# nh273/caro-ai

Measured on AMD Instinct MI355X. Metric: self-play MCTS node-expansions/sec/GPU (Connect4, 200 sims/move); 1->8 GPU scaling, higher is better.
Workload: dtype f32

## Files before the change

caro_ai_amd/_lib.py:

```python
import ctypes as C
import os

_HERE = os.path.dirname(os.path.abspath(__file__))
LIB_PATH = os.path.join(_HERE, "libcaro_hip.so")
if os.environ.get("CARO_HIP_LIB"):
    LIB_PATH = os.environ["CARO_HIP_LIB"]

GAME_CONNECT4, GAME_MNK, GAME_CARO = 0, 1, 2
RESIGNED = -2


class CaroError(RuntimeError):
    pass


class CaroConfig(C.Structure):
    _fields_ = [
        ("game_kind", C.c_int32), ("n", C.c_int32), ("k", C.c_int32), ("n_games", C.c_int32),
        ("n_stores", C.c_int32), ("n_nets", C.c_int32), ("max_batch", C.c_int32), ("node_cap", C.c_int32),
        ("steps_before_tau_0", C.c_int32), ("first_player_mode", C.c_int32),
        ("c_puct", C.c_float), ("alpha", C.c_double), ("explore", C.c_double),
        ("seed", C.c_uint64), ("uid_base", C.c_uint64), ("uid_stride", C.c_uint64),
        ("device_id", C.c_int32), ("evict", C.c_int32), ("stagger", C.c_int32), ("stagger_recycle", C.c_int32),
        ("games_limit", C.c_int64),
    ]


_P = C.c_void_p


class CaroDrainExtra(C.Structure):
    _fields_ = [("size", C.c_uint32), ("root_q_dev", _P), ("full_dev", _P), ("minibatches_dev", _P)]

    def __init__(self, root_q=None, full=None, minibatches=None):
        super().__init__(C.sizeof(CaroDrainExtra), root_q, full, minibatches)


class CaroDrainExtraOpen(CaroDrainExtra):
    _fields_ = [("open_dev", _P)]

    def __init__(self, root_q=None, full=None, minibatches=None, open=None):
        C.Structure.__init__(self, C.sizeof(CaroDrainExtraOpen), root_q, full, minibatches, open)


_SIGNATURES = {
    "caro_last_error": (C.c_char_p, []),
    "caro_version": (C.c_int, []),
    "caro_key_words": (C.c_int, [C.c_int, C.c_int]),
    "caro_action_space": (C.c_int, [C.c_int, C.c_int]),
    "caro_obs_cells": (C.c_int, [C.c_int, C.c_int]),
    "caro_host_initial": (C.c_int, [C.c_int, C.c_int, C.c_int, _P]),
    "caro_host_move": (C.c_int, [C.c_int, C.c_int, C.c_int, _P, C.c_int, C.c_int, _P]),
    "caro_host_legal": (C.c_int, [C.c_int, C.c_int, C.c_int, _P, _P]),
    "caro_host_encode": (C.c_int, [C.c_int, C.c_int, C.c_int, _P, C.c_int, _P]),
    "caro_host_noise_row": (C.c_int, [C.c_uint64, C.c_uint64, C.c_uint32, C.c_uint32, C.c_int, C.c_double, _P]),
    "caro_host_move_uniform": (C.c_double, [C.c_uint64, C.c_uint64, C.c_uint32]),
    "caro_host_resign_uniform": (C.c_double, [C.c_uint64, C.c_uint64]),
    "caro_host_cap_uniform": (C.c_double, [C.c_uint64, C.c_uint64, C.c_uint32]),
    "caro_host_open_uniform": (C.c_double, [C.c_uint64, C.c_uint64, C.c_uint32]),
    "caro_host_opening": (C.c_int, [C.c_int, C.c_int, C.c_int, C.c_uint64, C.c_uint64, C.c_int, C.c_int, _P, _P, _P]),
    "caro_openings_batch": (C.c_int, [C.c_int, C.c_int, C.c_int, C.c_uint64, C.c_int, C.c_int64] + [_P] * 6),
    "caro_rules_move_batch": (C.c_int, [C.c_int, C.c_int, C.c_int, C.c_int64, _P, _P, _P, _P, _P, _P]),
    "caro_rules_legal_batch": (C.c_int, [C.c_int, C.c_int, C.c_int, C.c_int64, _P, _P, _P]),
    "caro_rules_encode_batch": (C.c_int, [C.c_int, C.c_int, C.c_int, C.c_int64, _P, _P, _P, _P]),
    "caro_noise_batch": (C.c_int, [C.c_uint64, C.c_int64, C.c_int, C.c_double, _P, _P, _P, _P, _P]),
    "caro_engine_create": (C.c_int, [C.POINTER(CaroConfig), C.POINTER(_P)]),
    "caro_engine_destroy": (None, [_P]),
    "caro_engine_restart": (C.c_int, [_P, C.POINTER(CaroConfig), _P]),
    "caro_reset_games": (C.c_int, [_P, _P, _P]),
    "caro_set_roots": (C.c_int, [_P, _P, _P, _P]),
    "caro_select": (C.c_int, [_P, C.c_int, C.c_int, _P, _P, _P, _P]),
    "caro_leaf_counts": (C.c_int, [_P, _P, _P]),
    "caro_leaf_counts_dev": (C.c_int, [_P, _P]),
    "caro_net_packed_size": (C.c_int64, [C.c_int, C.c_int, C.c_int]),
    "caro_net_create": (C.c_int, [C.c_int, C.c_int, C.c_int, C.c_float, _P, C.c_int64, C.c_int, _P]),
    "caro_net_max_depth": (C.c_int, []),
    "caro_net_packed_size_depth": (C.c_int64, [C.c_int, C.c_int, C.c_int, C.c_int]),
    "caro_net_create_depth": (C.c_int, [C.c_int, C.c_int, C.c_int, C.c_int, C.c_float, _P, C.c_int64, C.c_int, _P]),
    "caro_net_depth": (C.c_int, [_P]),
    "caro_net_winograd_size_depth": (C.c_int64, [C.c_int]),
    "caro_net_winograd2d_size_depth": (C.c_int64, [C.c_int]),
    "caro_net_split_bf16_size_depth": (C.c_int64, [C.c_int]),
    "caro_net_destroy": (None, [_P]),
    "caro_net_enable_winograd": (C.c_int, [_P, _P, C.c_int64]),
    "caro_net_winograd2d_size": (C.c_int, []),
    "caro_net_winograd2d_supported": (C.c_int, [C.c_int, C.c_int]),
    "caro_net_enable_winograd2d": (C.c_int, [_P, _P, C.c_int64]),
    "caro_net_split_bf16_size": (C.c_int64, []),
    "caro_net_enable_split_bf16": (C.c_int, [_P, _P, C.c_int64]),
    "caro_net_boards_per_workgroup": (C.c_int, [_P]),
    "caro_net_uses_slot_list": (C.c_int, [_P]),
    "caro_net_stream_evictions": (C.c_int64, [_P]),
    "caro_net_forward": (C.c_int, [_P, _P, _P, C.c_int, C.c_int64, _P, _P, _P]),
    "caro_stream_create_partition": (C.c_int, [C.c_int, C.c_int, C.c_int, _P]),
    "caro_stream_destroy": (C.c_int, [_P]),
    "caro_search_batch": (C.c_int, [_P, _P, _P, C.c_int, C.c_int, _P, _P, _P, _P, _P, _P]),
    "caro_search_move": (C.c_int, [_P, _P, _P, C.c_int, C.c_int] + [_P] * 10),
    "caro_net_forward_pair": (C.c_int, [_P, _P, _P, _P, C.c_int64, _P, _P, _P]),
    "caro_net_forward_pair_at": (C.c_int, [_P, _P, _P, _P, C.c_int64, C.c_int64, _P, _P, _P]),
    "caro_net_forward_slots": (C.c_int, [_P, _P, _P, _P, _P, C.c_int, C.c_int, _P, _P, _P]),
    "caro_net_forward_slot_list": (C.c_int, [_P, _P, _P, _P, _P, _P, C.c_int, C.c_int, _P, _P, _P]),
    "caro_net_create_hash": (C.c_int, [C.c_int, C.c_int, C.c_int, C.c_uint64, C.c_int, _P]),
    "caro_net_forward_stamped": (C.c_int, [_P, _P, _P, C.c_int, C.c_int64, _P, _P, _P, _P]),
    "caro_net_debug_stamps": (C.c_int, [_P, _P]),
    "caro_get_descent": (C.c_int, [_P, C.c_int, C.c_int, _P, _P, _P, _P, _P, _P]),
    "caro_select_cancel": (C.c_int, [_P]),
    "caro_expand_backup": (C.c_int, [_P, _P, _P, _P]),
    "caro_policy": (C.c_int, [_P, _P, _P, _P]),
    "caro_step": (C.c_int, [_P, _P, _P, _P, _P, _P]),
    "caro_drain_tuples": (C.c_int, [_P, C.c_int64, _P, _P, _P, _P, _P, C.c_int, _P, _P, _P]),
    "caro_drain_tuples_begin": (C.c_int, [_P, C.c_int64, _P, _P, _P, _P, _P, C.c_int, _P]),
    "caro_drain_tuples_end": (C.c_int, [_P, _P, _P]),
    "caro_search_staggered": (C.c_int, [_P, _P, _P, C.c_int, C.c_int, _P, _P, _P, _P, _P]),
    "caro_drain_parked_begin": (C.c_int, [_P, C.c_int64, _P, _P, _P, _P, _P, _P]),
    "caro_engine_set_resign": (C.c_int, [_P, C.c_double, C.c_double]),
    "caro_drain_tuples_begin_q": (C.c_int, [_P, C.c_int64, _P, _P, _P, _P, _P, C.c_int, _P, _P]),
    "caro_drain_parked_begin_q": (C.c_int, [_P, C.c_int64, _P, _P, _P, _P, _P, _P, _P]),
    "caro_engine_set_playout_cap": (C.c_int, [_P, C.c_double, C.c_int]),
    "caro_drain_tuples_begin_x": (C.c_int, [_P, C.c_int64, _P, _P, _P, _P, _P, C.c_int, _P, _P, _P]),
    "caro_drain_parked_begin_x": (C.c_int, [_P, C.c_int64, _P, _P, _P, _P, _P, _P, _P, _P]),
    "caro_engine_set_early_stop": (C.c_int, [_P, C.c_int]),
    "caro_engine_set_openings": (C.c_int, [_P, C.c_int]),
    "caro_engine_set_forced_playouts": (C.c_int, [_P, C.c_double]),
    "caro_forced_stats": (C.c_int, [_P, _P, _P]),
    "caro_engine_set_kernel_form": (C.c_int, [_P, C.c_int]),
    "caro_engine_kernel_form": (C.c_int, [_P]),
    "caro_engine_set_fpu": (C.c_int, [_P, C.c_double, C.c_double]),
    "caro_host_fpu_level": (C.c_int, [C.c_int, C.c_int, _P, _P, _P, _P, _P, _P, _P, C.c_float, C.c_double, C.c_float,
                                      C.c_double, _P]),
    "caro_engine_set_virtual_loss": (C.c_int, [_P, C.c_int]),
    "caro_host_vl_level": (C.c_int, [C.c_int, C.c_int, _P, _P, _P, _P, _P, _P, _P, C.c_float, C.c_double, _P, C.c_int, _P]),
    "caro_engine_set_temperature": (C.c_int, [_P, C.c_double, C.c_double, C.c_int]),
    "caro_host_temperature": (C.c_int, [C.c_int, _P, C.c_double, _P]),
    "caro_host_forced_root": (C.c_int, [C.c_int, _P, _P, _P, _P, C.c_double, C.c_double, _P]),
    "caro_host_forced_prune": (C.c_int, [C.c_int, _P, _P, _P, C.c_float, C.c_double, _P]),
    "caro_drain_tuples_begin_ex": (C.c_int, [_P, C.c_int64, _P, _P, _P, _P, _P, C.c_int, C.POINTER(CaroDrainExtra), _P]),
    "caro_drain_parked_begin_ex": (C.c_int, [_P, C.c_int64, _P, _P, _P, _P, _P, C.POINTER(CaroDrainExtra), _P]),
    "caro_pool_open": (C.c_int, [_P, C.c_int64, _P, _P, _P, _P]),
    "caro_pool_set": (C.c_int, [_P, C.c_int64, _P, _P, _P, _P, _P]),
    "caro_pool_select": (C.c_int, [_P, C.c_int64, _P, _P]),
    "caro_pool_hold": (C.c_int, [_P, _P]),
    "caro_pool_level": (C.c_int, [_P, C.c_int64, _P, _P, _P, _P]),
    "caro_pool_select_budget": (C.c_int, [_P, C.c_int64, _P, _P, _P]),
    "caro_principal_lines": (C.c_int, [_P, C.c_int64, _P, C.c_int, C.c_int, C.c_int] + [_P] * 11),
    "caro_host_line_heads": (C.c_int, [C.c_int, _P, C.c_int, _P]),
    "caro_counters": (C.c_int, [_P, _P, _P]),
    "caro_live_games": (C.c_int, [_P, _P, _P]),
    "caro_pending_leaves": (C.c_int, [_P, _P, _P]),
    "caro_debug_stamps": (C.c_int, [_P, C.c_int]),
    "caro_debug_read": (C.c_int, [_P, _P, C.c_int64, _P]),
    "caro_debug_sqrt_check": (C.c_int, [C.c_uint32, _P]),
    "caro_profile_enable": (C.c_int, [_P, C.c_int]),
    "caro_profile_read": (C.c_int, [_P, _P, _P, C.c_int]),
    "caro_profile_begin": (C.c_int, [_P, C.c_int, _P]),
    "caro_profile_end": (None, [_P, C.c_int, _P]),
    "caro_tree_sizes": (C.c_int, [_P, _P, _P]),
    "caro_tree_live": (C.c_int, [_P, _P, _P]),
    "caro_lookup_nodes": (C.c_int, [_P, C.c_int64] + [_P] * 10),
    "caro_get_roots": (C.c_int, [_P] * 6),
    "caro_poke_nodes": (C.c_int, [_P, C.c_int64] + [_P] * 9),
    "caro_backup_path": (C.c_int, [_P, C.c_int, C.c_int, C.c_float, C.c_int, C.c_int, _P, _P, _P]),
    "caro_dump_tree": (C.c_int, [_P, C.c_int, C.c_int, C.c_int64] + [_P] * 8),
}
EXPORTS = sorted(_SIGNATURES)

_lib = None


def load():
    global _lib
    if _lib is not None:
        return _lib
    if not os.path.exists(LIB_PATH):
        raise CaroError("%s is missing: build it with `python -m caro_ai_amd.build` "
                        "(hipcc --offload-arch=gfx950); there is no CPU fallback" % LIB_PATH)
    try:
        lib = C.CDLL(LIB_PATH)
    except OSError as e:
        raise CaroError("cannot load %s: %s" % (LIB_PATH, e))
    for name, (res, args) in _SIGNATURES.items():
        fn = getattr(lib, name)
        fn.restype = res
        fn.argtypes = args
    _lib = lib
    return lib


def check(rc):
    if rc != 0:
        msg = load().caro_last_error()
        raise CaroError("libcaro_hip error %d: %s" % (rc, msg.decode() if msg else "?"))
```

caro_ai_amd/csrc/caro_net.hip:

```cpp
#include <hip/hip_runtime.h>

#include <algorithm>
#include <cstdlib>
#include <cstring>
#include <string>
#include <vector>

#include "../../include/caro_hip.h"
#include "../../include/caro_noise.h"

namespace cnet {

typedef float f32x16 __attribute__((ext_vector_type(16)));

constexpr int NF = 64;
constexpr int ZROW = 255;
constexpr int ACT = 256 * NF;
constexpr int WCHUNK = 64 * 64;
constexpr int NRES = 5;
constexpr int MAX_NRES = 40;
constexpr int TPC = 3;
constexpr int NTAPS = NRES * 9;
constexpr int LDS_FLOATS = ACT + 2 * TPC * WCHUNK;

struct NetParams {
  int H, W, HW, A, TB;
  float slope;
  const float* w_in;
  const float* b_in;
  const float* w_res;
  const float* b_res;
  const float* w_head;
  const float* b_head;
  const float* w_v1;
  const float* b_v1;
  const float* w_v2;
  const float* b_v2;
  const float* w_p;
  const float* b_p;
  const float* w_pT;
  const float* ww;
  const uint32_t* wtab;
  const float* ww2;
  const uint16_t* wx3;
  int ncu, TB2, TB4;
  int nres;
};

__device__ __forceinline__ int aoff(int row, int c) {
  return row * NF + ((((c >> 2) ^ (row & 15)) << 2) | (c & 3));
}
__device__ __forceinline__ float leaky(float x, float slope) { return x > 0.f ? x : x * slope; }

template <bool K2D>
__device__ __forceinline__ int akey(int r, int W) {
  if constexpr (!K2D) return r & 15;
  const int y = r / W, x = r - y * W;
  return (((x + 1) >> 1) & 7) | ((((y + 1) >> 1) & 1) << 3);
}

constexpr int NT = 512;

__device__ __forceinline__ void conv_in_f32(const NetParams& p, const float* __restrict__ planes, const int* smap,
                                            float* act, const float* win, int R, int tid) {
  const int HW = p.HW;
  const float slope = p.slope;
  const int r = tid & 255;
  const int chalf = tid >> 8;
  if (r < R) {
    const int bi = r / HW, cell = r - bi * HW;
    const int y = cell / p.W, x = cell - y * p.W;
    const float* pl = planes + (size_t)smap[bi] * 2 * HW;
    float in0[9], in1[9];
#pragma unroll
    for (int t = 0; t < 9; ++t) {
      const int ny = y + t / 3 - 1, nx = x + t % 3 - 1;
      const bool ok = ny >= 0 && ny < p.H && nx >= 0 && nx < p.W;
      in0[t] = ok ? pl[ny * p.W + nx] : 0.f;
      in1[t] = ok ? pl[HW + ny * p.W + nx] : 0.f;
    }
#pragma unroll
    for (int cc = 0; cc < 8; ++cc) {
      const int c4 = chalf * 8 + cc;
      float o[4];
#pragma unroll
      for (int u = 0; u < 4; ++u) o[u] = p.b_in[c4 * 4 + u];
#pragma unroll
      for (int t = 0; t < 9; ++t) {
        const float i0 = in0[t], i1 = in1[t];
        const float4 w0 = *reinterpret_cast<const float4*>(win + (2 * t) * NF + c4 * 4);
        const float4 w1 = *reinterpret_cast<const float4*>(win + (2 * t + 1) * NF + c4 * 4);
        o[0] = fmaf(i0, w0.x, o[0]); o[1] = fmaf(i0, w0.y, o[1]); o[2] = fmaf(i0, w0.z, o[2]); o[3] = fmaf(i0, w0.w, o[3]);
        o[0] = fmaf(i1, w1.x, o[0]); o[1] = fmaf(i1, w1.y, o[1]); o[2] = fmaf(i1, w1.z, o[2]); o[3] = fmaf(i1, w1.w, o[3]);
      }
      float4 out = make_float4(leaky(o[0], slope), leaky(o[1], slope), leaky(o[2], slope), leaky(o[3], slope));
      *reinterpret_cast<float4*>(act + r * NF + ((c4 ^ (r & 15)) << 2)) = out;
    }
  }
}

template <bool K2D = false, int NTH = NT>
__device__ __forceinline__ void conv_in_mfma(const NetParams& p, const float* __restrict__ planes, const int* smap,
                                             float* act, const float* win, int R, int tid) {
  const int HW = p.HW;
  const float slope = p.slope;
  const int wave = tid >> 6, lane = tid & 63;
  const int i = lane & 31, h = lane >> 5;
  const int ct = wave & 1;
  float wa[9];
#pragma unroll
  for (int t = 0; t < 9; ++t) wa[t] = win[(2 * t + h) * NF + ct * 32 + i];
  float4 bias[4];
#pragma unroll
  for (int q = 0; q < 4; ++q) bias[q] = *reinterpret_cast<const float4*>(p.b_in + ct * 32 + 8 * q + 4 * h);
  constexpr int RTS = NTH / 128;
#pragma unroll
  for (int half = 0; half < 8 / RTS; ++half) {
    const int rt = (wave >> 1) + RTS * half;
    if (rt * 32 >= R) continue;
    const int r = rt * 32 + i;
    const bool rv = r < R;
    const int bi = rv ? r / HW : 0, cell = rv ? r - bi * HW : 0;
    const int y = cell / p.W, x = cell - y * p.W;
    const float* pl = planes + (size_t)smap[bi] * 2 * HW + h * HW;
    float in[9];
#pragma unroll
    for (int t = 0; t < 9; ++t) {
      const int ny = y + t / 3 - 1, nx = x + t % 3 - 1;
      const bool ok = rv && ny >= 0 && ny < p.H && nx >= 0 && nx < p.W;
      in[t] = ok ? pl[ny * p.W + nx] : 0.f;
    }
    f32x16 acc;
#pragma unroll
    for (int q = 0; q < 4; ++q) {
      acc[4 * q] = bias[q].x; acc[4 * q + 1] = bias[q].y; acc[4 * q + 2] = bias[q].z; acc[4 * q + 3] = bias[q].w;
    }
#pragma unroll
    for (int t = 0; t < 9; ++t) acc = __builtin_amdgcn_mfma_f32_32x32x2f32(wa[t], in[t], acc, 0, 0, 0);
    if (rv) {
#pragma unroll
      for (int q = 0; q < 4; ++q) {
        const int c4 = ct * 8 + 2 * q + h;
        const float4 out = make_float4(leaky(acc[4 * q], slope), leaky(acc[4 * q + 1], slope),
                                       leaky(acc[4 * q + 2], slope), leaky(acc[4 * q + 3], slope));
        *reinterpret_cast<float4*>(act + r * NF + ((c4 ^ akey<K2D>(r, p.W)) << 2)) = out;
      }
    }
  }
}

constexpr int HEAD_STAGE_AT = 4096;
constexpr int HEAD_STAGE_MAX = 4096;
__device__ __forceinline__ int head_span(int HW, int A) { return 3 * NF + 3 + 20 * HW + 20 + 20 + 1 + A * 2 * HW + A; }
static inline int head_span_host(int HW, int A) { return 3 * NF + 3 + 20 * HW + 20 + 20 + 1 + A * 2 * HW + A; }

template <bool STAGED, bool K2D = false, int NTH = NT>
__device__ __forceinline__ void heads_f32(const NetParams& p, const float* act, float* scratch,
                                          float* __restrict__ probs, float* __restrict__ values, int slot_v, int nb,
                                          int R, int tid, float* __restrict__ featbuf = nullptr,
                                          int32_t* __restrict__ rowlist = nullptr, int dense0 = 0) {
  const int HW = p.HW, A = p.A;
  const float slope = p.slope;
  constexpr int NSM = (3 * NF + 3 + 20 * 225 + 20 + 20 + 1 + NTH - 1) / NTH;
  const int nsmall = 3 * NF + 3 + 20 * HW + 20 + 20 + 1;
  if (!STAGED && !featbuf) {
    float tmp[NSM];
#pragma unroll
    for (int u = 0; u < NSM; ++u) tmp[u] = tid + u * NTH < nsmall ? p.w_head[tid + u * NTH] : 0.f;
#pragma unroll
    for (int u = 0; u < NSM; ++u)
      if (tid + u * NTH < nsmall) scratch[HEAD_STAGE_AT + tid + u * NTH] = tmp[u];
    __syncthreads();
  }
  const float* hp = featbuf ? p.w_head : scratch + HEAD_STAGE_AT;
  const float* w_head = hp;
  const float* b_head = w_head + 3 * NF;
  const float* w_v1 = b_head + 3;
  const float* b_v1 = w_v1 + 20 * HW;
  const float* w_v2 = b_v1 + 20;
  const float* b_v2 = w_v2 + 20;
  const float* w_p = STAGED ? b_v2 + 1 : p.w_head + nsmall;
  const float* b_p = w_p + (size_t)A * 2 * HW;
  float* feat = scratch;
  float* hid = feat + 768;
  float* logit = feat + 768 + 20 * 32;
  float* stat = logit + 256 * 4;
  int* omap = reinterpret_cast<int*>(stat + 64);
  float* ebuf = stat + 128;
  if (tid < nb) omap[tid] = slot_v;
  for (int q = tid; q < 3 * R; q += NTH) {
    const int o = q / R, r = q - o * R;
    const float* wo = w_head + o * NF;
    float s0 = b_head[o];
    const int rkey = akey<K2D>(r, p.W);
#pragma unroll 8
    for (int g = 0; g < 16; ++g) {
      const float4 v = *reinterpret_cast<const float4*>(act + r * NF + ((g ^ rkey) << 2));
      const float4 w = *reinterpret_cast<const float4*>(wo + g * 4);
      s0 = fmaf(v.x, w.x, s0); s0 = fmaf(v.y, w.y, s0);
      s0 = fmaf(v.z, w.z, s0); s0 = fmaf(v.w, w.w, s0);
    }
    feat[o * 256 + r] = leaky(s0, slope);
  }
  __syncthreads();
  if (featbuf) {
    for (int q = tid; q < 3 * R; q += NTH) {
      const int o = q / R, r = q - o * R;
      const int bi = r / HW, c = r - bi * HW;
      featbuf[((size_t)(dense0 + bi) * 3 + o) * HW + c] = feat[o * 256 + r];
    }
    if (tid < nb) rowlist[dense0 + tid] = slot_v;
    return;
  }
  for (int k = tid; k < nb * 20; k += NTH) {
    const int bi = k / 20, u = k - bi * 20;
    float s = b_v1[u];
    const float* w = w_v1 + u * HW;
    const float* f = feat + bi * HW;
#pragma unroll 8
    for (int c = 0; c < HW; ++c) s = fmaf(f[c], w[c], s);
    hid[k] = leaky(s, slope);
  }
  for (int k = (tid + NTH / 2) % NTH; k < nb * A; k += NTH) {
    const int bi = k / A, a = k - bi * A;
    float s = b_p[a];
    const float* f0 = feat + 256 + bi * HW;
    const float* f1 = feat + 512 + bi * HW;
    if (STAGED || !p.w_pT) {
      const float* w = w_p + (size_t)a * 2 * HW;
#pragma unroll 8
      for (int c = 0; c < HW; ++c) s = fmaf(f0[c], w[c], s);
#pragma unroll 8
      for (int c = 0; c < HW; ++c) s = fmaf(f1[c], w[HW + c], s);
    } else {
      const int nq = HW >> 2, rem = HW & 3;
      const size_t half = ((size_t)HW * A + 3) & ~(size_t)3;
#pragma unroll
      for (int pl = 0; pl < 2; ++pl) {
        const float* f = pl ? f1 : f0;
        const float* wh = p.w_pT + pl * half;
        const float4* wq = reinterpret_cast<const float4*>(wh) + a;
#pragma unroll 8
        for (int q = 0; q < nq; ++q) {
          const float4 w = wq[(size_t)q * A];
          s = fmaf(f[4 * q], w.x, s); s = fmaf(f[4 * q + 1], w.y, s);
          s = fmaf(f[4 * q + 2], w.z, s); s = fmaf(f[4 * q + 3], w.w, s);
        }
        const float* wr = wh + (size_t)nq * A * 4 + a;
        for (int r = 0; r < rem; ++r) s = fmaf(f[4 * nq + r], wr[(size_t)r * A], s);
      }
    }
    logit[k] = s;
  }
  __syncthreads();
  {
    const int vt = tid - (NTH - 64);
    if (vt >= 0 && vt < nb) {
      float s = b_v2[0];
      for (int u = 0; u < 20; ++u) s = fmaf(hid[vt * 20 + u], w_v2[u], s);
      values[omap[vt]] = tanhf(s);
    }
  }
  float* pmax = ebuf + 1024;
  static_assert(768 + 20 * 32 + 256 * 4 + 128 + 1024 + 512 <= HEAD_STAGE_AT, "heads scratch layout");
  const bool wide = A > 32;
  if (wide) {
    for (int idx = tid; idx < nb * 16; idx += NTH) {
      const int bi = idx >> 4, j = idx & 15;
      const float* lg = logit + bi * A;
      float m = -3.4e38f;
      for (int a = j; a < A; a += 16) m = fmaxf(m, lg[a]);
      pmax[idx] = m;
    }
    __syncthreads();
  }
  for (int k = tid; k < nb * A; k += NTH) {
    const int bi = k / A;
    float mx = -3.4e38f;
    if (wide) {
      const float* pm = pmax + bi * 16;
#pragma unroll
      for (int j = 0; j < 16; ++j) mx = fmaxf(mx, pm[j]);
    } else {
      const float* lg = logit + bi * A;
      int a = 0;
      for (; a + 8 <= A; a += 8) {
        const float t0 = lg[a], t1 = lg[a + 1], t2 = lg[a + 2], t3 = lg[a + 3], t4 = lg[a + 4], t5 = lg[a + 5], t6 = lg[a + 6], t7 = lg[a + 7];
        mx = fmaxf(fmaxf(fmaxf(fmaxf(mx, t0), fmaxf(t1, t2)), fmaxf(fmaxf(t3, t4), fmaxf(t5, t6))), t7);
      }
      for (; a < A; ++a) mx = fmaxf(mx, lg[a]);
    }
    ebuf[k] = expf(logit[k] - mx);
  }
  __syncthreads();
  if (wide) {
    for (int idx = tid; idx < nb * 16; idx += NTH) {
      const int bi = idx >> 4, j = idx & 15;
      const float* eb = ebuf + bi * A;
      float part = 0.f;
      for (int a = j; a < A; a += 16) part += eb[a];
      pmax[idx] = part;
    }
    __syncthreads();
    if (tid < nb) {
      float sum = 0.f;
#pragma unroll
      for (int j = 0; j < 16; ++j) sum += pmax[tid * 16 + j];
      stat[2 * tid + 1] = sum;
    }
  } else if (tid < nb) {
    float sum = 0.f;
    const float* eb = ebuf + tid * A;
    int a = 0;
    for (; a + 8 <= A; a += 8) {
      const float t0 = eb[a], t1 = eb[a + 1], t2 = eb[a + 2], t3 = eb[a + 3], t4 = eb[a + 4], t5 = eb[a + 5], t6 = eb[a + 6], t7 = eb[a + 7];
      sum += t0; sum += t1; sum += t2; sum += t3; sum += t4; sum += t5; sum += t6; sum += t7;
    }
    for (; a < A; ++a) sum += eb[a];
    stat[2 * tid + 1] = sum;
  }
  __syncthreads();
  for (int k = tid; k < nb * A; k += NTH) {
    const int bi = k / A;
    probs[(size_t)omap[bi] * A + (k - bi * A)] = ebuf[k] / stat[2 * bi + 1];
  }
}

template <int NTH = NT>
__device__ __forceinline__ void tile_rows(const int32_t* __restrict__ gpack, int G, int B, int cls, int base,
                                          int board0, int nb, int* sc, int* smap, int tid) {
  if (!gpack) {
    if (tid < nb) smap[tid] = base + tid;
    __syncthreads();
    return;
  }
  const int lane = tid & 63, wave = tid >> 6;
  const int cpt = (G + NTH - 1) / NTH;
  const int g_lo = min(G, tid * cpt), g_hi = min(G, g_lo + cpt);
  int mine = 0;
  for (int g = g_lo; g < g_hi; ++g) {
    const int v = gpack[g];
    mine += (v >> 8) == cls ? (v & 0xFF) : 0;
  }
  int inc = mine;
#pragma unroll
  for (int d = 1; d < 64; d <<= 1) {
    const int t = __shfl_up(inc, d, 64);
    if (lane >= d) inc += t;
  }
  if (lane == 63) sc[wave] = inc;
  __syncthreads();
  int ex = inc - mine;
  for (int w = 0; w < wave; ++w) ex += sc[w];
  if (ex < board0 + nb && ex + mine > board0) {
    for (int g = g_lo; g < g_hi; ++g) {
      const int v = gpack[g];
      if ((v >> 8) != cls) continue;
      const int n = v & 0xFF;
      for (int j = 0; j < n; ++j) {
        const int r = ex + j - board0;
        if (r >= 0 && r < nb) smap[r] = g * B + j;
      }
      ex += n;
    }
  }
  __syncthreads();
}


constexpr int GP_PRE = 4;
__device__ __forceinline__ void tile_rows_pre(const int (&gv)[GP_PRE], int cpt, int mine, int B, int cls, int board0,
                                              int nb, int* sc, int* smap, int tid) {
  const int lane = tid & 63, wave = tid >> 6;
  int inc = mine;
#pragma unroll
  for (int d = 1; d < 64; d <<= 1) {
    const int t = __shfl_up(inc, d, 64);
    if (lane >= d) inc += t;
  }
  if (lane == 63) sc[wave] = inc;
  __syncthreads();
  int ex = inc - mine;
  for (int w = 0; w < wave; ++w) ex += sc[w];
  if (ex < board0 + nb && ex + mine > board0) {
#pragma unroll
    for (int u = 0; u < GP_PRE; ++u) {
      const int v = gv[u];
      if (u >= cpt || (v >> 8) != cls) continue;
      const int n = v & 0xFF, g = tid * cpt + u;
      for (int j = 0; j < n; ++j) {
        const int r = ex + j - board0;
        if (r >= 0 && r < nb) smap[r] = g * B + j;
      }
      ex += n;
    }
  }
  __syncthreads();
}

__device__ __forceinline__ unsigned lds_addr(const void* q) {
  return (unsigned)(size_t)(__attribute__((address_space(3))) const void*)q;
}
__device__ __forceinline__ void dma_b128(const void* gsrc, unsigned lds_wave_base) {
  asm volatile("s_mov_b32 m0, %0\n\ts_nop 0\n\tglobal_load_lds_dwordx4 %1, off" ::"s"(lds_wave_base), "v"(gsrc) : "memory");
}
__device__ __forceinline__ void dma_b128_s(const void* sbase, unsigned voff, unsigned lds_wave_base) {
  asm volatile("s_mov_b32 m0, %0\n\ts_nop 0\n\tglobal_load_lds_dwordx4 %1, %2" ::"s"(lds_wave_base), "v"(voff), "s"(sbase) : "memory");
}

#ifndef CARO_X3_TIMERS
#define CARO_X3_TIMERS 0
#endif
typedef __bf16 bf16x8 __attribute__((ext_vector_type(8)));
typedef __bf16 bf16x2 __attribute__((ext_vector_type(2)));
typedef float f32x2 __attribute__((ext_vector_type(2)));
typedef float f32x4v __attribute__((ext_vector_type(4)));
constexpr int X3_H = 3 * 4 * 64;
constexpr int X3_TAP_U4 = 2 * X3_H;
constexpr int X3_PAD_TAPS = 2;
constexpr int X3_RING_H1 = 3 * X3_H;

__device__ __forceinline__ uint32_t pk_bf16(f32x2 v) { return __builtin_bit_cast(uint32_t, __builtin_convertvector(v, bf16x2)); }
__device__ __forceinline__ f32x2 unpk_bf16(uint32_t w) {
  f32x2 r;
  r.x = __builtin_bit_cast(float, w << 16);
  r.y = __builtin_bit_cast(float, w & 0xFFFF0000u);
  return r;
}
__device__ __forceinline__ void split3(f32x2 v, uint32_t& hi, uint32_t& mid, uint32_t& lo) {
  hi = pk_bf16(v);
  const f32x2 r1 = v - unpk_bf16(hi);
  mid = pk_bf16(r1);
  const f32x2 r2 = r1 - unpk_bf16(mid);
  lo = pk_bf16(r2);
}
__device__ __forceinline__ f32x2 join3(uint32_t hi, uint32_t mid, uint32_t lo) {
  return (unpk_bf16(hi) + unpk_bf16(mid)) + unpk_bf16(lo);
}

__global__ __launch_bounds__(NT, 2) void k_net_forward_x3(NetParams p0, NetParams p1, const float* __restrict__ planes,
                                                            const int32_t* __restrict__ counts, int which, int row1,
                                                            float* __restrict__ probs, float* __restrict__ values,
                                                            unsigned long long* __restrict__ stamps,
                                                            const int32_t* __restrict__ gpack, int gG, int gB,
                                                            float* __restrict__ featbuf, int32_t* __restrict__ rowlist) {
  __shared__ __attribute__((aligned(16))) float lds[LDS_FLOATS];
  float* act = lds;
  float* wbuf = lds + ACT;

  int L, row0, board0;
  bool second = false;
  if (which < 2) {
    L = counts[which];
    row0 = which ? counts[0] : 0;
    board0 = blockIdx.x * p0.TB;
  } else {
    const int L0 = counts[0];
    const int t0 = (L0 + p0.TB - 1) / p0.TB;
    second = (int)blockIdx.x >= t0;
    L = second ? counts[1] : L0;
    row0 = second ? (row1 >= 0 ? row1 : L0) : 0;
    board0 = (second ? (int)blockIdx.x - t0 : (int)blockIdx.x) * p0.TB;
  }
  if (board0 >= L) return;
  const NetParams p = second ? p1 : p0;
  const float slope = p.slope;
  unsigned long long t_c0 = 0, t_r0 = 0, t_epi = 0;
  if (stamps) {
    t_c0 = __builtin_amdgcn_s_memtime();
    t_r0 = __builtin_amdgcn_s_memrealtime();
  }
  const int nb = min(p.TB, L - board0);
  const int HW = p.HW;
  const int R = nb * HW;
  const int tid = threadIdx.x;
  const int wave = tid >> 6, lane = tid & 63;

  for (int k = tid; k < ACT / 4; k += NT) reinterpret_cast<float4*>(lds)[k] = make_float4(0.f, 0.f, 0.f, 0.f);
  for (int k = tid; k < 9 * 2 * NF; k += NT) wbuf[k] = p.w_in[k];
  int* smap = reinterpret_cast<int*>(wbuf + 1536);
  tile_rows(gpack, gG, gB, second ? 1 : 0, row0 + board0, board0, nb, smap + 64, smap, tid);
  conv_in_mfma(p, planes, smap, act, wbuf, R, tid);
  const int slot_v0 = tid < nb ? smap[tid] : 0;
  __syncthreads();

  unsigned long long t_trunk0 = 0;
  if (stamps) t_trunk0 = __builtin_amdgcn_s_memtime();
  const int r16 = lane & 15, kg = lane >> 4;
  const int myrow0 = wave * 32 + r16, myrow1 = myrow0 + 16;
  const bool rvalid0 = myrow0 < R, rvalid1 = myrow1 < R;
  f32x2 res[2][4][2];
#pragma unroll
  for (int rb = 0; rb < 2; ++rb)
#pragma unroll
    for (int cb = 0; cb < 4; ++cb) {
      const int row = rb ? myrow1 : myrow0;
      const float4 v = *reinterpret_cast<const float4*>(act + row * NF + (((4 * cb + kg) ^ (row & 15)) << 2));
      res[rb][cb][0] = f32x2{v.x, v.y};
      res[rb][cb][1] = f32x2{v.z, v.w};
    }
  uint4* parts = reinterpret_cast<uint4*>(wbuf);
#pragma unroll
  for (int m = 0; m < 4; ++m) {
    const int k = tid + NT * m, row = k & 255, g = k >> 8;
    const float4 lo4 = *reinterpret_cast<const float4*>(act + row * NF + (((2 * g) ^ (row & 15)) << 2));
    const float4 hi4 = *reinterpret_cast<const float4*>(act + row * NF + (((2 * g + 1) ^ (row & 15)) << 2));
    const f32x2 v[4] = {{lo4.x, lo4.y}, {lo4.z, lo4.w}, {hi4.x, hi4.y}, {hi4.z, hi4.w}};
    uint32_t ph[4], pm[4], pl[4];
#pragma unroll
    for (int e = 0; e < 4; ++e) split3(v[e], ph[e], pm[e], pl[e]);
    parts[(0 * 8 + g) * 256 + row] = make_uint4(ph[0], ph[1], ph[2], ph[3]);
    parts[(1 * 8 + g) * 256 + row] = make_uint4(pm[0], pm[1], pm[2], pm[3]);
    parts[(2 * 8 + g) * 256 + row] = make_uint4(pl[0], pl[1], pl[2], pl[3]);
  }
  __syncthreads();
  uint4* ring = reinterpret_cast<uint4*>(act);
  const uint4* wsrc = reinterpret_cast<const uint4*>(p.wx3);
  const bool stage_h0 = tid >= 256;
  const unsigned ring_lds = lds_addr(ring);
  const unsigned v0off = (unsigned)tid * 16u;
  const unsigned v1off = (unsigned)(stage_h0 ? X3_TAP_U4 + (tid - 256) : X3_H + 512 + tid) * 16u;
  {
    ring[0 * X3_H + tid] = wsrc[tid];
    if (tid < 256) ring[0 * X3_H + 512 + tid] = wsrc[512 + tid];
    ring[1 * X3_H + tid] = wsrc[X3_TAP_U4 + tid];
    if (tid < 256) ring[1 * X3_H + 512 + tid] = wsrc[X3_TAP_U4 + 512 + tid];
    ring[X3_RING_H1 + tid] = wsrc[X3_H + tid];
    if (tid < 256) ring[X3_RING_H1 + 512 + tid] = wsrc[X3_H + 512 + tid];
  }
  static_assert((X3_RING_H1 + 2 * X3_H) * 16 + NRES * NF * 4 + NT * 4 <= ACT * 4, "ring + biases + output rows must fit the 64 KB of the float32 activations");
  float* bias_l = reinterpret_cast<float*>(ring + X3_RING_H1 + 2 * X3_H);
  int* slot_l = reinterpret_cast<int*>(bias_l + NRES * NF);
  if (tid < NRES * NF) bias_l[tid] = p.b_res[tid];
  slot_l[tid] = slot_v0;
  __syncthreads();

  int nrow9[9];
#pragma unroll
  for (int t = 0; t < 9; ++t) nrow9[t] = 0;
#pragma unroll
  for (int rb = 0; rb < 2; ++rb) {
    const int row = rb ? myrow1 : myrow0;
    const bool rv = rb ? rvalid1 : rvalid0;
    const int rbi = row / HW;
    const int rcell = row - rbi * HW;
    const int ry = rcell / p.W, rx = rcell - ry * p.W;
#pragma unroll
    for (int t = 0; t < 9; ++t) {
      const int ny = ry + t / 3 - 1, nx = rx + t % 3 - 1;
      const bool ok = rv && ny >= 0 && ny < p.H && nx >= 0 && nx < p.W;
      nrow9[t] |= (ok ? rbi * HW + ny * p.W + nx : (int)ZROW) << (16 * rb);
    }
  }

  f32x4v acc[2][4];
#pragma unroll
  for (int rb = 0; rb < 2; ++rb)
#pragma unroll
    for (int cb = 0; cb < 4; ++cb) acc[rb][cb] = f32x4v{0.f, 0.f, 0.f, 0.f};
  const uint4* arow = parts + kg * 256;
#define CARO_X3_LOAD_ACT(S_, C_, N0_, N1_)                                  \
  _Pragma("unroll") for (int pt_ = 0; pt_ < 3; ++pt_) {                     \
    S_[pt_ * 2] = arow[(pt_ * 8 + 4 * (C_)) * 256 + (N0_)];                 \
    S_[pt_ * 2 + 1] = arow[(pt_ * 8 + 4 * (C_)) * 256 + (N1_)];             \
  }
#define CARO_X3_LOAD_W(S_, HB_, CP_)                                        \
  _Pragma("unroll") for (int pt_ = 0; pt_ < 3; ++pt_) {                     \
    S_[pt_ * 2] = (HB_)[pt_ * 256 + (CP_) * 32];                            \
    S_[pt_ * 2 + 1] = (HB_)[pt_ * 256 + (CP_) * 32 + 16];                   \
  }
#define CARO_X3_PROD(W_, A_, CP_, WP_, AP_)                                                                     \
  _Pragma("unroll") for (int cbi_ = 0; cbi_ < 2; ++cbi_) _Pragma("unroll") for (int rb_ = 0; rb_ < 2; ++rb_)   \
    acc[rb_][2 * (CP_) + cbi_] = __builtin_amdgcn_mfma_f32_16x16x32_bf16(                                       \
        __builtin_bit_cast(bf16x8, W_[(WP_) * 2 + cbi_]), __builtin_bit_cast(bf16x8, A_[(AP_) * 2 + rb_]),      \
        acc[rb_][2 * (CP_) + cbi_], 0, 0, 0);
#define CARO_X3_SEG(W_, A_, CP_)  \
  CARO_X3_PROD(W_, A_, CP_, 1, 1) \
  CARO_X3_PROD(W_, A_, CP_, 2, 0) \
  CARO_X3_PROD(W_, A_, CP_, 0, 2) \
  CARO_X3_PROD(W_, A_, CP_, 1, 0) \
  CARO_X3_PROD(W_, A_, CP_, 0, 1) \
  CARO_X3_PROD(W_, A_, CP_, 0, 0)
#define CARO_X3_WEAVE(NR_)                                  \
  _Pragma("unroll") for (int q_ = 0; q_ < (NR_); ++q_) {    \
    __builtin_amdgcn_sched_group_barrier(0x008, 2, 0);      \
    __builtin_amdgcn_sched_group_barrier(0x100, 1, 0);      \
  }                                                         \
  __builtin_amdgcn_sched_group_barrier(0x008, 24 - 2 * (NR_), 0);
#if CARO_X3_TIMERS
  unsigned long long tq[8] = {0, 0, 0, 0, 0, 0, 0, 0}, tl = 0;
#define CARO_T0 tl = __builtin_amdgcn_s_memtime();
#define CARO_T(K_) { const unsigned long long t_ = __builtin_amdgcn_s_memtime(); tq[K_] += t_ - tl; tl = t_; }
#else
#define CARO_T0
#define CARO_T(K_)
#endif
  uint4 X[6], Y[6], P[6], Q[6];
  const uint4* wcol = ring + kg * 64 + r16;
  CARO_X3_LOAD_ACT(X, 0, nrow9[0] & 0xFFFF, nrow9[0] >> 16)
  CARO_X3_LOAD_W(P, wcol, 0)
  const char* wnext = reinterpret_cast<const char*>(wsrc + X3_TAP_U4);
  for (int layer = 0; layer < NRES; ++layer) {
#pragma unroll
    for (int tap = 0; tap < 9; ++tap) {
      const int cur = (layer + tap) & 1;
      const int slot0 = tap % 3, slot1 = (tap + 1) % 3, slot2 = (tap + 2) % 3;
      CARO_T0
      {
        const unsigned d1 = ring_lds + (unsigned)(X3_RING_H1 + (cur ^ 1) * X3_H) * 16u;
        const unsigned d0 = ring_lds + (unsigned)(slot2 * X3_H) * 16u;
        const unsigned w1k = (unsigned)wave * 1024u;
        dma_b128_s(wnext + X3_H * 16, v0off, __builtin_amdgcn_readfirstlane(d1 + w1k));
        dma_b128_s(wnext, v1off, __builtin_amdgcn_readfirstlane(stage_h0 ? d0 + w1k - 4096u : d1 + 8192u + w1k));
        dma_b128_s(wnext + (X3_TAP_U4 + 256) * 16, v0off, __builtin_amdgcn_readfirstlane(d0 + 4096u + w1k));
        wnext += X3_TAP_U4 * 16;
      }
      const uint4* hb0 = wcol + slot0 * X3_H;
      const uint4* hb1 = wcol + X3_RING_H1 + cur * X3_H;
      const int n0 = nrow9[tap] & 0xFFFF, n1 = nrow9[tap] >> 16;
      __builtin_amdgcn_sched_barrier(0);
      CARO_T(0)
      CARO_X3_LOAD_W(Q, hb0, 1)
      CARO_X3_SEG(P, X, 0)
      CARO_X3_WEAVE(6)
      __builtin_amdgcn_sched_barrier(0);
      CARO_T(1)
      CARO_X3_LOAD_ACT(Y, 1, n0, n1)
      CARO_X3_LOAD_W(P, hb1, 0)
      CARO_X3_SEG(Q, X, 1)
      CARO_X3_WEAVE(12)
      __builtin_amdgcn_sched_barrier(0);
      CARO_T(2)
      CARO_X3_LOAD_W(Q, hb1, 1)
      CARO_X3_SEG(P, Y, 0)
      CARO_X3_WEAVE(6)
      __builtin_amdgcn_sched_barrier(0);
      CARO_T(3)
      CARO_X3_LOAD_ACT(X, 0, nrow9[tap == 8 ? 0 : tap + 1] & 0xFFFF, nrow9[tap == 8 ? 0 : tap + 1] >> 16)
      CARO_X3_LOAD_W(P, wcol + slot1 * X3_H, 0)
      CARO_X3_SEG(Q, Y, 1)
      CARO_X3_WEAVE(12)
      __builtin_amdgcn_sched_barrier(0);
      CARO_T(4)
      if (tap == 8) {
        unsigned long long t_e0 = 0;
        if (stamps) t_e0 = __builtin_amdgcn_s_memtime();
        __syncthreads();
        const f32x2 slope2 = {slope, slope};
        float4 bq[4];
#pragma unroll
        for (int cb = 0; cb < 4; ++cb) bq[cb] = *reinterpret_cast<const float4*>(bias_l + layer * NF + 16 * cb + 4 * kg);
#pragma unroll
        for (int rb = 0; rb < 2; ++rb) {
          const int row = rb ? myrow1 : myrow0;
          const bool rv = rb ? rvalid1 : rvalid0;
          const f32x2 keep = rv ? f32x2{1.f, 1.f} : f32x2{0.f, 0.f};
          uint2* mine = reinterpret_cast<uint2*>(parts + (kg >> 1) * 256 + row) + (kg & 1);
#pragma unroll
          for (int cb = 0; cb < 4; ++cb) {
            const f32x4v a = acc[rb][cb];
            const f32x2 t01 = f32x2{a[0], a[1]} + f32x2{bq[cb].x, bq[cb].y}, t23 = f32x2{a[2], a[3]} + f32x2{bq[cb].z, bq[cb].w};
            const f32x2 s01 = t01 * slope2, s23 = t23 * slope2;
            const f32x2 l01 = {t01.x > 0.f ? t01.x : s01.x, t01.y > 0.f ? t01.y : s01.y};
            const f32x2 l23 = {t23.x > 0.f ? t23.x : s23.x, t23.y > 0.f ? t23.y : s23.y};
            res[rb][cb][0] = (res[rb][cb][0] + l01) * keep;
            res[rb][cb][1] = (res[rb][cb][1] + l23) * keep;
            uint2 wh, wm, wl;
            split3(res[rb][cb][0], wh.x, wm.x, wl.x);
            split3(res[rb][cb][1], wh.y, wm.y, wl.y);
            mine[(0 * 8 + 2 * cb) * 512] = wh;
            mine[(1 * 8 + 2 * cb) * 512] = wm;
            mine[(2 * 8 + 2 * cb) * 512] = wl;
            acc[rb][cb] = f32x4v{0.f, 0.f, 0.f, 0.f};
          }
        }
        if (stamps) t_epi += __builtin_amdgcn_s_memtime() - t_e0;
      }
      CARO_T0
      asm volatile("s_waitcnt vmcnt(0)" ::: "memory");
      __syncthreads();
      CARO_T(5)
      if (tap == 8 && layer + 1 < NRES) {
        CARO_X3_LOAD_ACT(X, 0, nrow9[0] & 0xFFFF, nrow9[0] >> 16)
      }
    }
  }
#undef CARO_X3_WEAVE
#undef CARO_X3_LOAD_ACT
#undef CARO_X3_LOAD_W
#undef CARO_X3_PROD
#undef CARO_X3_SEG
  const int slot_v = slot_l[tid];
  __syncthreads();
#pragma unroll
  for (int rb = 0; rb < 2; ++rb)
#pragma unroll
    for (int cb = 0; cb < 4; ++cb) {
      const int row = rb ? myrow1 : myrow0;
      *reinterpret_cast<float4*>(act + row * NF + (((4 * cb + kg) ^ (row & 15)) << 2)) =
          make_float4(res[rb][cb][0].x, res[rb][cb][0].y, res[rb][cb][1].x, res[rb][cb][1].y);
    }
  __syncthreads();
  unsigned long long t_trunk1 = 0;
  if (stamps) t_trunk1 = __builtin_amdgcn_s_memtime();
  heads_f32<false>(p, act, wbuf, probs, values, slot_v, nb, R, tid, featbuf, rowlist, row0 + board0);
  if (stamps && tid == 0) {
    stamps[4 * blockIdx.x] = __builtin_amdgcn_s_memtime() - t_c0;
    stamps[4 * blockIdx.x + 1] = ((__builtin_amdgcn_s_memrealtime() - t_r0) & 0xFFFFFull) | (t_epi << 20);
    stamps[4 * blockIdx.x + 2] = t_trunk0 - t_c0;
    stamps[4 * blockIdx.x + 3] = t_trunk1 - t_c0;
#if CARO_X3_TIMERS
    for (int q = 0; q < 8; ++q) stamps[4 * 512 + 8 * blockIdx.x + q] = tq[q];
#endif
  }
}

constexpr int WCH = 4 * 2 * 64 * 16;
constexpr int WNBUF = 3;
constexpr int XROW4 = 63;
constexpr int XROW2 = 127;
static_assert(WNBUF * WCH == 2 * TPC * WCHUNK, "the ring takes the place of the two three-tap buffers");

typedef float f4v __attribute__((ext_vector_type(4)));

__device__ __forceinline__ void fetch_chunk(const float* ww, int c, unsigned wring, int tid) {
  const float4* src = reinterpret_cast<const float4*>(ww + (size_t)c * WCH) + tid;
  const unsigned dst = __builtin_amdgcn_readfirstlane(wring + (unsigned)(c % WNBUF) * (WCH * 4) + (unsigned)(tid >> 6) * 1024u);
#pragma unroll
  for (int m = 0; m < WCH / 4 / NT; ++m) dma_b128(src + m * NT, dst + m * NT * 16);
}

__device__ __forceinline__ void fetch_chunk_s(const float* ww, int c, unsigned wring, int tid) {
  const char* base = reinterpret_cast<const char*>(ww) + (size_t)c * (WCH * 4);
  const unsigned voff = (unsigned)tid * 16u;
  const unsigned dst = __builtin_amdgcn_readfirstlane(wring + (unsigned)(c % WNBUF) * (WCH * 4) + (unsigned)(tid >> 6) * 1024u);
#pragma unroll
  for (int m = 0; m < WCH / 4 / NT; ++m) dma_b128_s(base + m * NT * 16, voff, dst + m * NT * 16);
}

__device__ __forceinline__ void fetch_heads(const float* hp, int hspan, unsigned wring, int tid) {
  const float4* src = reinterpret_cast<const float4*>(hp) + tid;
  const unsigned dst = __builtin_amdgcn_readfirstlane(wring + HEAD_STAGE_AT * 4u + (unsigned)(tid >> 6) * 1024u);
  dma_b128(src, dst);
  if (hspan > NT * 4) dma_b128(src + NT, dst + NT * 16);
}

template <int KS, int NR>
__device__ __forceinline__ void trunk_w(const NetParams& p, float* act, float* wbuf, int nb, int tid, int hspan) {
  const int nres = NR ? NR : p.nres;
  const int wnchunk = nres * 6;
  const float slope = p.slope;
  const int HW = p.HW;
  const int wave = tid >> 6, lane = tid & 63;
  const int i = lane & 31, h = lane >> 5;
  constexpr int NRT = 4 / KS;
  constexpr int NQ = 4 / KS;
  constexpr int NSET = 6 * NQ;
  const int ct = wave & 1, rt = (wave >> 1) % NRT, kq = (wave >> 1) / NRT;
  int tbi, tty, tx;
  bool tvalid;
  if (KS == 1) {
    const uint32_t tent = p.wtab[rt * 32 + i];
    tbi = tent & 0xFF; tty = (tent >> 8) & 0xFF; tx = (tent >> 16) & 0xFF;
    tvalid = (tent >> 24) != 0 && tbi < nb;
  } else {
    const int tpb = ((p.H + 1) >> 1) * p.W;
    const int mt = rt * 32 + i;
    tbi = mt / tpb;
    const int rem = mt - tbi * tpb;
    tty = rem / p.W; tx = rem - tty * p.W;
    tvalid = mt < nb * tpb;
  }
  const int orow0 = tbi * HW + 2 * tty * p.W + tx;
  const bool ovalid0 = tvalid, ovalid1 = tvalid && 2 * tty + 1 < p.H;
  const unsigned abase = lds_addr(act);
  unsigned ra[4][3];
#pragma unroll
  for (int r = 0; r < 4; ++r) {
    const int y = 2 * tty - 1 + r;
    const bool oky = tvalid && y >= 0 && y < p.H;
#pragma unroll
    for (int d = 0; d < 3; ++d) {
      const int nx = tx + d - 1;
      const int v = tbi * HW + y * p.W + nx;
      const int row = oky && nx >= 0 && nx < p.W ? v : ZROW;
      ra[r][d] = abase + (unsigned)(row * NF + (((h * 8 + kq) ^ (v & 15)) << 2)) * 4u;
    }
  }
  const unsigned wlane = lds_addr(wbuf) + (unsigned)((h * 64 + ct * 32 + i) * 16 + ((kq ^ ((i >> 2) & 3)) << 2)) * 4u;
  const unsigned wring = lds_addr(wbuf);

  f4v D0, D1, D2, D3;
  f4v W0, W1, W2, W3, X0, X1, X2, X3;
#define CARO_ALOAD(B0, B1, B2, B3, T)                                                                        \
  {                                                                                                          \
    constexpr int cc_ = (T) / NQ, dx_ = cc_ >> 1, g8_ = (cc_ & 1) * 4 + ((T) % NQ) * KS;                     \
    const unsigned wa_ = (wlane + (unsigned)(cc_ % WNBUF) * (WCH * 4)) ^ ((unsigned)(((T) % NQ) * KS) << 4); \
    asm volatile("ds_read_b128 %0, %1" : "=v"(D0) : "v"(ra[0][dx_] ^ (g8_ << 4)));                           \
    asm volatile("ds_read_b128 %0, %1" : "=v"(D1) : "v"(ra[1][dx_] ^ (g8_ << 4)));                           \
    asm volatile("ds_read_b128 %0, %1" : "=v"(D2) : "v"(ra[2][dx_] ^ (g8_ << 4)));                           \
    asm volatile("ds_read_b128 %0, %1" : "=v"(D3) : "v"(ra[3][dx_] ^ (g8_ << 4)));                           \
    asm volatile("ds_read_b128 %0, %1" : "=v"(B0) : "v"(wa_));                                               \
    asm volatile("ds_read_b128 %0, %1 offset:8192" : "=v"(B1) : "v"(wa_));                                   \
    asm volatile("ds_read_b128 %0, %1 offset:16384" : "=v"(B2) : "v"(wa_));                                  \
    asm volatile("ds_read_b128 %0, %1 offset:24576" : "=v"(B3) : "v"(wa_));                                  \
  }
#define CARO_AWAIT(B0, B1, B2, B3)                                                                           \
  asm volatile("s_waitcnt lgkmcnt(0)" : "+v"(D0), "+v"(D1), "+v"(D2), "+v"(D3), "+v"(B0), "+v"(B1), "+v"(B2), "+v"(B3));
#define CARO_STEP(T, B0, B1, B2, B3, NB0, NB1, NB2, NB3)                                                     \
  CARO_AWAIT(B0, B1, B2, B3)                                                                                 \
  if ((T) % NQ == 0) {                                                                                       \
    if ((T) != 0) {                                                                                          \
      asm volatile("s_waitcnt vmcnt(0)" ::: "memory");                                                       \
       __syncthreads();                                                                    \
    }                                                                                                        \
    if ( c0 + (T) / NQ + 2 < wnchunk) fetch_chunk(p.ww, c0 + (T) / NQ + 2, wring, tid);         \
    else if (c0 + (T) / NQ + 2 == wnchunk && hspan) fetch_heads(p.w_head, hspan, wring, tid);                \
  }                                                                                                          \
  {                                                                                                          \
        \
    const f4v v0 = D0 - D2;                                                                                  \
    __builtin_amdgcn_sched_barrier(0);                                                                       \
    accM0 = __builtin_amdgcn_mfma_f32_32x32x2f32(B0.x, v0.x, accM0, 0, 0, 0);                                \
    const f4v v1 = D1 + D2;                                                                                  \
    __builtin_amdgcn_sched_barrier(0);                                                                       \
    accM1 = __builtin_amdgcn_mfma_f32_32x32x2f32(B1.x, v1.x, accM1, 0, 0, 0);                                \
    const f4v v2 = D2 - D1;                                                                                  \
    __builtin_amdgcn_sched_barrier(0);                                                                       \
    accM2 = __builtin_amdgcn_mfma_f32_32x32x2f32(B2.x, v2.x, accM2, 0, 0, 0);                                \
    const f4v v3 = D1 - D3;                                                                                  \
    __builtin_amdgcn_sched_barrier(0);                                                                       \
    accM3 = __builtin_amdgcn_mfma_f32_32x32x2f32(B3.x, v3.x, accM3, 0, 0, 0);                                \
    __builtin_amdgcn_sched_barrier(0);                                                                       \
    if ((T) + 1 < NSET) CARO_ALOAD(NB0, NB1, NB2, NB3, ((T) + 1) % NSET)                                     \
    __builtin_amdgcn_sched_barrier(0);                                                                       \
    accM0 = __builtin_amdgcn_mfma_f32_32x32x2f32(B0.y, v0.y, accM0, 0, 0, 0);                                \
    accM1 = __builtin_amdgcn_mfma_f32_32x32x2f32(B1.y, v1.y, accM1, 0, 0, 0);                                \
    accM2 = __builtin_amdgcn_mfma_f32_32x32x2f32(B2.y, v2.y, accM2, 0, 0, 0);                                \
    accM3 = __builtin_amdgcn_mfma_f32_32x32x2f32(B3.y, v3.y, accM3, 0, 0, 0);                                \
    accM0 = __builtin_amdgcn_mfma_f32_32x32x2f32(B0.z, v0.z, accM0, 0, 0, 0);                                \
    accM1 = __builtin_amdgcn_mfma_f32_32x32x2f32(B1.z, v1.z, accM1, 0, 0, 0);                                \
    accM2 = __builtin_amdgcn_mfma_f32_32x32x2f32(B2.z, v2.z, accM2, 0, 0, 0);                                \
    accM3 = __builtin_amdgcn_mfma_f32_32x32x2f32(B3.z, v3.z, accM3, 0, 0, 0);                                \
    accM0 = __builtin_amdgcn_mfma_f32_32x32x2f32(B0.w, v0.w, accM0, 0, 0, 0);                                \
    accM1 = __builtin_amdgcn_mfma_f32_32x32x2f32(B1.w, v1.w, accM1, 0, 0, 0);                                \
    accM2 = __builtin_amdgcn_mfma_f32_32x32x2f32(B2.w, v2.w, accM2, 0, 0, 0);                                \
    accM3 = __builtin_amdgcn_mfma_f32_32x32x2f32(B3.w, v3.w, accM3, 0, 0, 0);                                \
    __builtin_amdgcn_sched_barrier(0);                                                                       \
  }

  float4 res0[4], res1[4];
#pragma unroll
  for (int q = 0; q < 4; ++q) res0[q] = res1[q] = make_float4(0.f, 0.f, 0.f, 0.f);
  for (int layer = 0; layer < nres; ++layer) {
    const int c0 = layer * 6;
    f32x16 accM0, accM1, accM2, accM3;
#pragma unroll
    for (int e = 0; e < 16; ++e) {
      accM0[e] = 0.f;
      accM1[e] = 0.f;
      accM2[e] = 0.f;
      accM3[e] = 0.f;
    }
#pragma unroll
    for (int r = 0; r < 4; ++r)
#pragma unroll
      for (int d = 0; d < 3; ++d) asm volatile("" : "+v"(ra[r][d]));
    CARO_ALOAD(W0, W1, W2, W3, 0)
#define CARO_PAIR(T)                                                                                         \
  CARO_STEP(T, W0, W1, W2, W3, X0, X1, X2, X3)                                                               \
  CARO_STEP((T) + 1, X0, X1, X2, X3, W0, W1, W2, W3)
    CARO_PAIR(0) CARO_PAIR(2) CARO_PAIR(4)
    if constexpr (NSET > 6) { CARO_PAIR(6) CARO_PAIR(8) CARO_PAIR(10) }
    if constexpr (NSET > 12) { CARO_PAIR(12) CARO_PAIR(14) CARO_PAIR(16) CARO_PAIR(18) CARO_PAIR(20) CARO_PAIR(22) }
#undef CARO_PAIR
    if constexpr (KS == 2) {
      const bool up = kq != 0;
      const float m0 = up ? 0.f : 1.f, m2 = up ? -1.f : 1.f, m3 = up ? -1.f : 0.f;
      const float s0 = up ? 1.f : 0.f, s2 = up ? 1.f : -1.f, s3 = up ? 0.f : -1.f;
      const float* bias = p.b_res + layer * NF + ct * 32 + 4 * h;
      const int g0 = ct * 8 + h;
      float* rowp = act + (orow0 + (up ? p.W : 0)) * NF;
      const int kk = (orow0 + (up ? p.W : 0)) & 15;
      const bool ov = up ? ovalid1 : ovalid0;
      float4 bq[4], old[4];
#pragma unroll
      for (int q = 0; q < 4; ++q) bq[q] = *reinterpret_cast<const float4*>(bias + 8 * q);
      if (layer == 0) {
#pragma unroll
        for (int q = 0; q < 4; ++q)
          old[q] = ov ? *reinterpret_cast<const float4*>(rowp + (((g0 + 2 * q) ^ kk) << 2)) : make_float4(0.f, 0.f, 0.f, 0.f);
      } else {
#pragma unroll
        for (int q = 0; q < 4; ++q) old[q] = res0[q];
      }
      f32x16 mine, send;
#pragma unroll
      for (int e = 0; e < 16; ++e) {
        float a = fmaf(m0, accM0[e], 0.f), b = fmaf(s0, accM0[e], 0.f);
        a = fmaf(1.f, accM1[e], a); b = fmaf(1.f, accM1[e], b);
        a = fmaf(m2, accM2[e], a); b = fmaf(s2, accM2[e], b);
        a = fmaf(m3, accM3[e], a); b = fmaf(s3, accM3[e], b);
        mine[e] = a;
        send[e] = b;
      }
      float* xw = act + XROW2 * NF + ((rt * 2 + ct) * 2 + kq) * 1024 + lane * 4;
      const float* xr = act + XROW2 * NF + ((rt * 2 + ct) * 2 + (kq ^ 1)) * 1024 + lane * 4;
#pragma unroll
      for (int q = 0; q < 4; ++q)
        *reinterpret_cast<float4*>(xw + q * 256) = make_float4(send[4 * q], send[4 * q + 1], send[4 * q + 2], send[4 * q + 3]);
      asm volatile("s_waitcnt lgkmcnt(0)" ::: "memory");
      __builtin_amdgcn_s_barrier();
      asm volatile("" ::: "memory");
      float4 part[4];
#pragma unroll
      for (int q = 0; q < 4; ++q) part[q] = *reinterpret_cast<const float4*>(xr + q * 256);
#pragma unroll
      for (int q = 0; q < 4; ++q) {
        float4 n;
        n.x = old[q].x + leaky((mine[4 * q] + part[q].x) + bq[q].x, slope);
        n.y = old[q].y + leaky((mine[4 * q + 1] + part[q].y) + bq[q].y, slope);
        n.z = old[q].z + leaky((mine[4 * q + 2] + part[q].z) + bq[q].z, slope);
        n.w = old[q].w + leaky((mine[4 * q + 3] + part[q].w) + bq[q].w, slope);
        if (ov) *reinterpret_cast<float4*>(rowp + (((g0 + 2 * q) ^ kk) << 2)) = n;
        res0[q] = ov ? n : make_float4(0.f, 0.f, 0.f, 0.f);
      }
    } else if constexpr (KS == 4) {
      f32x16 accY0, accY1;
#pragma unroll
      for (int e = 0; e < 16; ++e) {
        float y0 = fmaf(1.f, accM0[e], 0.f), y1 = fmaf(0.f, accM0[e], 0.f);
        y0 = fmaf(1.f, accM1[e], y0); y1 = fmaf(1.f, accM1[e], y1);
        y0 = fmaf(1.f, accM2[e], y0); y1 = fmaf(-1.f, accM2[e], y1);
        y0 = fmaf(0.f, accM3[e], y0); y1 = fmaf(-1.f, accM3[e], y1);
        accY0[e] = y0;
        accY1[e] = y1;
      }
      const int myrow = kq >> 1, qb = (kq & 1) * 2;
      const float* bias = p.b_res + layer * NF + ct * 32 + 4 * h;
      const int g0 = ct * 8 + h;
      float* rowp = act + (orow0 + (myrow ? p.W : 0)) * NF;
      const int kk = (orow0 + (myrow ? p.W : 0)) & 15;
      const bool ov = myrow ? ovalid1 : ovalid0;
      float4 bq[2], old[2];
#pragma unroll
      for (int j = 0; j < 2; ++j) bq[j] = *reinterpret_cast<const float4*>(bias + 8 * (qb + j));
      if (layer == 0) {
#pragma unroll
        for (int j = 0; j < 2; ++j)
          old[j] = ov ? *reinterpret_cast<const float4*>(rowp + (((g0 + 2 * (qb + j)) ^ kk) << 2)) : make_float4(0.f, 0.f, 0.f, 0.f);
      } else {
#pragma unroll
        for (int j = 0; j < 2; ++j) old[j] = res0[j];
      }
#define CARO_QUARTER(D, J)                                                                                              \
  (((D) >> 1) ? make_float4(accY1[4 * (2 * ((D) & 1) + (J))], accY1[4 * (2 * ((D) & 1) + (J)) + 1],                      \
                            accY1[4 * (2 * ((D) & 1) + (J)) + 2], accY1[4 * (2 * ((D) & 1) + (J)) + 3])                  \
              : make_float4(accY0[4 * (2 * ((D) & 1) + (J))], accY0[4 * (2 * ((D) & 1) + (J)) + 1],                      \
                            accY0[4 * (2 * ((D) & 1) + (J)) + 2], accY0[4 * (2 * ((D) & 1) + (J)) + 3]))
      float* xa = act + XROW4 * NF + lane * 4;
      float4 mine[2] = {make_float4(0.f, 0.f, 0.f, 0.f), make_float4(0.f, 0.f, 0.f, 0.f)};
#pragma unroll
      for (int d = 0; d < 4; ++d) {
        if (d == kq) {
          mine[0] = CARO_QUARTER(d, 0);
          mine[1] = CARO_QUARTER(d, 1);
        } else {
          const int sp = kq < d ? kq : kq - 1;
          float* dst = xa + (((ct * 4 + d) * 3 + sp) * 2) * 256;
          *reinterpret_cast<float4*>(dst) = CARO_QUARTER(d, 0);
          *reinterpret_cast<float4*>(dst + 256) = CARO_QUARTER(d, 1);
        }
      }
#undef CARO_QUARTER
      asm volatile("s_waitcnt lgkmcnt(0)" ::: "memory");
      __builtin_amdgcn_s_barrier();
      asm volatile("" ::: "memory");
      float4 part[4][2];
#pragma unroll
      for (int k = 0; k < 4; ++k) {
        part[k][0] = part[k][1] = make_float4(0.f, 0.f, 0.f, 0.f);
        if (k != kq) {
          const int sp = k < kq ? k : k - 1;
          const float* src = xa + (((ct * 4 + kq) * 3 + sp) * 2) * 256;
          part[k][0] = *reinterpret_cast<const float4*>(src);
          part[k][1] = *reinterpret_cast<const float4*>(src + 256);
        }
      }
#pragma unroll
      for (int j = 0; j < 2; ++j) {
        float4 v = kq == 0 ? mine[j] : part[0][j];
#pragma unroll
        for (int k = 1; k < 4; ++k) {
          const float4 t = k == kq ? mine[j] : part[k][j];
          v.x += t.x; v.y += t.y; v.z += t.z; v.w += t.w;
        }
        float4 n;
        n.x = old[j].x + leaky(v.x + bq[j].x, slope);
        n.y = old[j].y + leaky(v.y + bq[j].y, slope);
        n.z = old[j].z + leaky(v.z + bq[j].z, slope);
        n.w = old[j].w + leaky(v.w + bq[j].w, slope);
        if (ov) *reinterpret_cast<float4*>(rowp + (((g0 + 2 * (qb + j)) ^ kk) << 2)) = n;
        res0[j] = ov ? n : make_float4(0.f, 0.f, 0.f, 0.f);
      }
    } else {
    f32x16 accY0, accY1;
#pragma unroll
    for (int e = 0; e < 16; ++e) {
      float y0 = fmaf(1.f, accM0[e], 0.f), y1 = fmaf(0.f, accM0[e], 0.f);
      y0 = fmaf(1.f, accM1[e], y0); y1 = fmaf(1.f, accM1[e], y1);
      y0 = fmaf(1.f, accM2[e], y0); y1 = fmaf(-1.f, accM2[e], y1);
      y0 = fmaf(0.f, accM3[e], y0); y1 = fmaf(-1.f, accM3[e], y1);
      accY0[e] = y0;
      accY1[e] = y1;
    }
    const float* bias = p.b_res + layer * NF + ct * 32 + 4 * h;
    const int g0 = ct * 8 + h;
    float* row0p = act + orow0 * NF;
    float* row1p = row0p + p.W * NF;
    const int k0 = orow0 & 15, k1 = (orow0 + p.W) & 15;
    float4 bq[4], old0[4], old1[4];
#pragma unroll
    for (int q = 0; q < 4; ++q) bq[q] = *reinterpret_cast<const float4*>(bias + 8 * q);
    if (layer == 0) {
#pragma unroll
      for (int q = 0; q < 4; ++q) {
        old0[q] = ovalid0 ? *reinterpret_cast<const float4*>(row0p + (((g0 + 2 * q) ^ k0) << 2)) : make_float4(0.f, 0.f, 0.f, 0.f);
        old1[q] = ovalid1 ? *reinterpret_cast<const float4*>(row1p + (((g0 + 2 * q) ^ k1) << 2)) : make_float4(0.f, 0.f, 0.f, 0.f);
      }
    } else {
#pragma unroll
      for (int q = 0; q < 4; ++q) {
        old0[q] = res0[q];
        old1[q] = res1[q];
      }
    }
    asm volatile("" ::: "memory");
    __builtin_amdgcn_s_barrier();
    asm volatile("" ::: "memory");
    const bool writer = true;
#pragma unroll
    for (int q = 0; q < 4; ++q) {
      float4 n0, n1;
      n0.x = old0[q].x + leaky(accY0[4 * q] + bq[q].x, slope);
      n0.y = old0[q].y + leaky(accY0[4 * q + 1] + bq[q].y, slope);
      n0.z = old0[q].z + leaky(accY0[4 * q + 2] + bq[q].z, slope);
      n0.w = old0[q].w + leaky(accY0[4 * q + 3] + bq[q].w, slope);
      n1.x = old1[q].x + leaky(accY1[4 * q] + bq[q].x, slope);
      n1.y = old1[q].y + leaky(accY1[4 * q + 1] + bq[q].y, slope);
      n1.z = old1[q].z + leaky(accY1[4 * q + 2] + bq[q].z, slope);
      n1.w = old1[q].w + leaky(accY1[4 * q + 3] + bq[q].w, slope);
      if (ovalid0 && writer) *reinterpret_cast<float4*>(row0p + (((g0 + 2 * q) ^ k0) << 2)) = n0;
      if (ovalid1 && writer) *reinterpret_cast<float4*>(row1p + (((g0 + 2 * q) ^ k1) << 2)) = n1;
      res0[q] = ovalid0 ? n0 : make_float4(0.f, 0.f, 0.f, 0.f);
      res1[q] = ovalid1 ? n1 : make_float4(0.f, 0.f, 0.f, 0.f);
    }
    }
    asm volatile("s_waitcnt vmcnt(0)" ::: "memory");
    __syncthreads();
  }
#undef CARO_STEP
#undef CARO_AWAIT
#undef CARO_ALOAD
}


constexpr int W2NCHUNK = NRES * 8;
constexpr int W2SETS = 16;

template <int NR>
__device__ __forceinline__ void trunk_w2d(const NetParams& p, float* act, float* wbuf, int tid) {
  const int nres = NR ? NR : p.nres;
  const int w2nchunk = nres * 8;
  const float slope = p.slope;
  const int H = p.H, W = p.W;
  const int wave = tid >> 6, lane = tid & 63;
  const int i = lane & 31, h = lane >> 5;
  const int ct = wave & 1, rt = (wave >> 1) & 1, bh = wave >> 2;
  const int quad = i >> 2, grp = (0x96 >> quad) & 1, qq = ((quad >> 1) << 2) | (i & 3);
  const int tx = qq & 7, ty = rt * 4 + grp * 2 + (qq >> 3);
  const bool tvalid = ty < ((H + 1) >> 1) && tx < ((W + 1) >> 1);
  const unsigned abase = lds_addr(act);
  const unsigned wring = lds_addr(wbuf);
  auto caddr = [&](int r, int j) -> unsigned {
    const int y = 2 * ty - 1 + r, x = 2 * tx - 1 + j;
    const bool ok = tvalid && y >= 0 && y < H && x >= 0 && x < W;
    const int row = ok ? y * W + x : ZROW;
    const int key = ((tx + (j >> 1)) & 7) | (((ty + (r >> 1)) & 1) << 3);
    return abase + (unsigned)(row * NF + (((h * 8) ^ key) << 2)) * 4u;
  };
  const int jA0 = bh ? 2 : 1, jB0 = bh ? 1 : 2, jA1 = bh ? 1 : 0, jB1 = bh ? 3 : 2;
  const float sg0 = bh ? -1.f : 1.f, sg1 = -1.f;
  unsigned ra[2][4], rb[2][4];
#pragma unroll
  for (int r = 0; r < 4; ++r) {
    ra[0][r] = caddr(r, jA0); rb[0][r] = caddr(r, jB0);
    ra[1][r] = caddr(r, jA1); rb[1][r] = caddr(r, jB1);
  }
  const unsigned wlane = wring + (unsigned)(bh * 16384 + (h * 64 + ct * 32 + i) * 32 + (((i >> 3) & 1) << 4));
  const int xo = 2 * tx + bh, xp = 2 * tx + 1 - bh;
  const int g0 = ct * 8 + h;
  int oidx[2], pidx[2];
  bool ovalid[2], pvalid[2];
#pragma unroll
  for (int u = 0; u < 2; ++u) {
    const int y = 2 * ty + u;
    ovalid[u] = tvalid && y < H && xo < W;
    pvalid[u] = tvalid && y < H && xp < W;
    const int okey = (((xo + 1) >> 1) & 7) | ((((y + 1) >> 1) & 1) << 3);
    const int pkey = (((xp + 1) >> 1) & 7) | ((((y + 1) >> 1) & 1) << 3);
    oidx[u] = (y * W + xo) * NF + ((g0 ^ okey) << 2);
    pidx[u] = (y * W + xp) * NF + ((g0 ^ pkey) << 2);
  }

  f4v CA0, CA1, CA2, CA3, CB0, CB1, CB2, CB3;
  f4v W0, W1, W2, W3, X0, X1, X2, X3;
#define W2_ALOAD(B0, B1, B2, B3, T)                                                                          \
  {                                                                                                          \
    constexpr int ph_ = (T) >> 3, G_ = (T) & 7, cq_ = (T) >> 1;                                              \
    const unsigned wa_ = (wlane + rbuf[cq_ % WNBUF]) ^ ((unsigned)(G_ & 1) << 4);                            \
    asm volatile("ds_read_b128 %0, %1" : "=v"(CA0) : "v"(ra[ph_][0] ^ (G_ << 4)));                           \
    asm volatile("ds_read_b128 %0, %1" : "=v"(CB0) : "v"(rb[ph_][0] ^ (G_ << 4)));                           \
    asm volatile("ds_read_b128 %0, %1" : "=v"(CA1) : "v"(ra[ph_][1] ^ (G_ << 4)));                           \
    asm volatile("ds_read_b128 %0, %1" : "=v"(CB1) : "v"(rb[ph_][1] ^ (G_ << 4)));                           \
    asm volatile("ds_read_b128 %0, %1" : "=v"(CA2) : "v"(ra[ph_][2] ^ (G_ << 4)));                           \
    asm volatile("ds_read_b128 %0, %1" : "=v"(CB2) : "v"(rb[ph_][2] ^ (G_ << 4)));                           \
    asm volatile("ds_read_b128 %0, %1" : "=v"(CA3) : "v"(ra[ph_][3] ^ (G_ << 4)));                           \
    asm volatile("ds_read_b128 %0, %1" : "=v"(CB3) : "v"(rb[ph_][3] ^ (G_ << 4)));                           \
    asm volatile("ds_read_b128 %0, %1" : "=v"(B0) : "v"(wa_));                                               \
    asm volatile("ds_read_b128 %0, %1 offset:4096" : "=v"(B1) : "v"(wa_));                                   \
    asm volatile("ds_read_b128 %0, %1 offset:8192" : "=v"(B2) : "v"(wa_));                                   \
    asm volatile("ds_read_b128 %0, %1 offset:12288" : "=v"(B3) : "v"(wa_));                                  \
  }
#define W2_AWAIT(B0, B1, B2, B3)                                                                             \
  asm volatile("s_waitcnt lgkmcnt(0)"                                                                        \
               : "+v"(CA0), "+v"(CA1), "+v"(CA2), "+v"(CA3), "+v"(CB0), "+v"(CB1), "+v"(CB2), "+v"(CB3),     \
                 "+v"(B0), "+v"(B1), "+v"(B2), "+v"(B3));
#define W2_STEP(T, B0, B1, B2, B3, NB0, NB1, NB2, NB3)                                                       \
  W2_AWAIT(B0, B1, B2, B3)                                                                                   \
  if ((T) % 2 == 0) {                                                                                        \
    if ((T) != 0) {                                                                                          \
      asm volatile("s_waitcnt vmcnt(0)" ::: "memory");                                                       \
       __syncthreads();                                                                    \
    }                                                                                                        \
    if ( c0 + (T) / 2 + 2 < w2nchunk) fetch_chunk_s(p.ww2, c0 + (T) / 2 + 2, wring, tid);       \
  }                                                                                                          \
  {                                                                                                          \
    const float sg_ = ((T) >> 3) ? sg1 : sg0;                                                                \
    const f4v c0_ = CA0 + sg_ * CB0, c1_ = CA1 + sg_ * CB1, c2_ = CA2 + sg_ * CB2, c3_ = CA3 + sg_ * CB3;    \
    const f4v v0 = c0_ - c2_;                                                                                \
    __builtin_amdgcn_sched_barrier(0);                                                                       \
                        \
    accM0 = __builtin_amdgcn_mfma_f32_32x32x2f32(B0.x, v0.x, (T) % 8 == 0 ? zero16 : accM0, 0, 0, 0);        \
    const f4v v1 = c1_ + c2_;                                                                                \
    __builtin_amdgcn_sched_barrier(0);                                                                       \
    accM1 = __builtin_amdgcn_mfma_f32_32x32x2f32(B1.x, v1.x, (T) % 8 == 0 ? zero16 : accM1, 0, 0, 0);        \
    const f4v v2 = c2_ - c1_;                                                                                \
    __builtin_amdgcn_sched_barrier(0);                                                                       \
    accM2 = __builtin_amdgcn_mfma_f32_32x32x2f32(B2.x, v2.x, (T) % 8 == 0 ? zero16 : accM2, 0, 0, 0);        \
    const f4v v3 = c1_ - c3_;                                                                                \
    __builtin_amdgcn_sched_barrier(0);                                                                       \
    accM3 = __builtin_amdgcn_mfma_f32_32x32x2f32(B3.x, v3.x, (T) % 8 == 0 ? zero16 : accM3, 0, 0, 0);        \
    __builtin_amdgcn_sched_barrier(0);                                                                       \
    if ((T) + 1 < W2SETS) W2_ALOAD(NB0, NB1, NB2, NB3, ((T) + 1) % W2SETS)                                   \
    __builtin_amdgcn_sched_barrier(0);                                                                       \
    accM0 = __builtin_amdgcn_mfma_f32_32x32x2f32(B0.y, v0.y, accM0, 0, 0, 0);                                \
    accM1 = __builtin_amdgcn_mfma_f32_32x32x2f32(B1.y, v1.y, accM1, 0, 0, 0);                                \
    accM2 = __builtin_amdgcn_mfma_f32_32x32x2f32(B2.y, v2.y, accM2, 0, 0, 0);                                \
    accM3 = __builtin_amdgcn_mfma_f32_32x32x2f32(B3.y, v3.y, accM3, 0, 0, 0);                                \
    accM0 = __builtin_amdgcn_mfma_f32_32x32x2f32(B0.z, v0.z, accM0, 0, 0, 0);                                \
    accM1 = __builtin_amdgcn_mfma_f32_32x32x2f32(B1.z, v1.z, accM1, 0, 0, 0);                                \
    accM2 = __builtin_amdgcn_mfma_f32_32x32x2f32(B2.z, v2.z, accM2, 0, 0, 0);                                \
    accM3 = __builtin_amdgcn_mfma_f32_32x32x2f32(B3.z, v3.z, accM3, 0, 0, 0);                                \
    accM0 = __builtin_amdgcn_mfma_f32_32x32x2f32(B0.w, v0.w, accM0, 0, 0, 0);                                \
    accM1 = __builtin_amdgcn_mfma_f32_32x32x2f32(B1.w, v1.w, accM1, 0, 0, 0);                                \
    accM2 = __builtin_amdgcn_mfma_f32_32x32x2f32(B2.w, v2.w, accM2, 0, 0, 0);                                \
    accM3 = __builtin_amdgcn_mfma_f32_32x32x2f32(B3.w, v3.w, accM3, 0, 0, 0);                                \
    __builtin_amdgcn_sched_barrier(0);                                                                       \
  }
#define W2_PAIR(T)                                                                                           \
  W2_STEP(T, W0, W1, W2, W3, X0, X1, X2, X3)                                                                 \
  W2_STEP((T) + 1, X0, X1, X2, X3, W0, W1, W2, W3)
#define W2_FOLD(Z0_, Z1_)                                                                                    \
  _Pragma("unroll") for (int e = 0; e < 16; ++e) {                                                           \
    Z0_[e] = (accM0[e] + accM1[e]) + accM2[e];                                                               \
    Z1_[e] = (accM1[e] - accM2[e]) - accM3[e];                                                               \
  }

  for (int layer = 0; layer < nres; ++layer) {
    const int c0 = layer * 8;
    unsigned rbuf[WNBUF];
#pragma unroll
    for (int k = 0; k < WNBUF; ++k) rbuf[k] = (unsigned)((c0 + k) % WNBUF) * (WCH * 4);
    const f32x16 zero16 = {};
    f32x16 accM0, accM1, accM2, accM3, Zs0, Zs1, Zt0, Zt1;
#pragma unroll
    for (int r = 0; r < 4; ++r) asm volatile("" : "+v"(ra[0][r]), "+v"(rb[0][r]), "+v"(ra[1][r]), "+v"(rb[1][r]));
    W2_ALOAD(W0, W1, W2, W3, 0)
    W2_PAIR(0) W2_PAIR(2) W2_PAIR(4)
    const float* bias = p.b_res + layer * NF + ct * 32 + 4 * h;
    float4 bq[4];
#pragma unroll
    for (int q = 0; q < 4; ++q) bq[q] = *reinterpret_cast<const float4*>(bias + 8 * q);
    W2_PAIR(6)
    W2_FOLD(Zs0, Zs1)
    if (bh == 0) {
#pragma unroll
      for (int q = 0; q < 4; ++q) {
        Zs0[4 * q] += bq[q].x; Zs0[4 * q + 1] += bq[q].y; Zs0[4 * q + 2] += bq[q].z; Zs0[4 * q + 3] += bq[q].w;
        Zs1[4 * q] += bq[q].x; Zs1[4 * q + 1] += bq[q].y; Zs1[4 * q + 2] += bq[q].z; Zs1[4 * q + 3] += bq[q].w;
      }
    }
    W2_PAIR(8) W2_PAIR(10) W2_PAIR(12) W2_PAIR(14)
    W2_FOLD(Zt0, Zt1)
    float4 old0[4], old1[4];
    asm volatile("" : "+v"(oidx[0]), "+v"(oidx[1]), "+v"(pidx[0]), "+v"(pidx[1]));
#pragma unroll
    for (int q = 0; q < 4; ++q) {
      old0[q] = ovalid[0] ? *reinterpret_cast<const float4*>(act + (oidx[0] ^ (8 * q))) : make_float4(0.f, 0.f, 0.f, 0.f);
      old1[q] = ovalid[1] ? *reinterpret_cast<const float4*>(act + (oidx[1] ^ (8 * q))) : make_float4(0.f, 0.f, 0.f, 0.f);
    }
    f32x16 S0, S1;
#pragma unroll
    for (int e = 0; e < 16; ++e) {
      S0[e] = Zt0[e] + Zs0[e];
      S1[e] = Zt1[e] + Zs1[e];
    }
    asm volatile("s_waitcnt lgkmcnt(0)" ::: "memory");
    __builtin_amdgcn_s_barrier();
    asm volatile("" ::: "memory");
    {
#pragma unroll
      for (int q = 0; q < 4; ++q) {
        if (pvalid[0])
          *reinterpret_cast<float4*>(act + (pidx[0] ^ (8 * q))) = make_float4(Zs0[4 * q], Zs0[4 * q + 1], Zs0[4 * q + 2], Zs0[4 * q + 3]);
        if (pvalid[1])
          *reinterpret_cast<float4*>(act + (pidx[1] ^ (8 * q))) = make_float4(Zs1[4 * q], Zs1[4 * q + 1], Zs1[4 * q + 2], Zs1[4 * q + 3]);
      }
    }
    asm volatile("s_waitcnt lgkmcnt(0)" ::: "memory");
    __builtin_amdgcn_s_barrier();
    asm volatile("" ::: "memory");
    const float sgn = bh ? -1.f : 1.f;
#pragma unroll
    for (int q = 0; q < 4; ++q) {
      const float4 r0 = ovalid[0] ? *reinterpret_cast<const float4*>(act + (oidx[0] ^ (8 * q))) : make_float4(0.f, 0.f, 0.f, 0.f);
      const float4 r1 = ovalid[1] ? *reinterpret_cast<const float4*>(act + (oidx[1] ^ (8 * q))) : make_float4(0.f, 0.f, 0.f, 0.f);
      float4 n0, n1;
      n0.x = old0[q].x + leaky(fmaf(sgn, S0[4 * q], r0.x), slope);
      n0.y = old0[q].y + leaky(fmaf(sgn, S0[4 * q + 1], r0.y), slope);
      n0.z = old0[q].z + leaky(fmaf(sgn, S0[4 * q + 2], r0.z), slope);
      n0.w = old0[q].w + leaky(fmaf(sgn, S0[4 * q + 3], r0.w), slope);
      n1.x = old1[q].x + leaky(fmaf(sgn, S1[4 * q], r1.x), slope);
      n1.y = old1[q].y + leaky(fmaf(sgn, S1[4 * q + 1], r1.y), slope);
      n1.z = old1[q].z + leaky(fmaf(sgn, S1[4 * q + 2], r1.z), slope);
      n1.w = old1[q].w + leaky(fmaf(sgn, S1[4 * q + 3], r1.w), slope);
      if (ovalid[0]) *reinterpret_cast<float4*>(act + (oidx[0] ^ (8 * q))) = n0;
      if (ovalid[1]) *reinterpret_cast<float4*>(act + (oidx[1] ^ (8 * q))) = n1;
    }
    asm volatile("s_waitcnt vmcnt(0)" ::: "memory");
    __syncthreads();
  }
#undef W2_FOLD
#undef W2_PAIR
#undef W2_STEP
#undef W2_AWAIT
#undef W2_ALOAD
}

#define CARO_NR NRES
#define CARO_KN(name) name
#include "caro_net_kernels.inc"
#undef CARO_NR
#undef CARO_KN
#define CARO_NR 0
#define CARO_KN(name) name##_any
#include "caro_net_kernels.inc"
#undef CARO_NR
#undef CARO_KN

constexpr int HB = 32;
constexpr int HEADS_MAX_CELLS = 225;
constexpr int HPL = 228;
static_assert(HPL >= HEADS_MAX_CELLS && HPL % 4 == 0, "a staged feature plane holds every cell of the largest board");
constexpr int HFS = 3 * HPL + 8;
constexpr int HLG = 256;
__global__ __launch_bounds__(NT, 1) void k_net_heads(NetParams p0, NetParams p1, const int32_t* __restrict__ counts,
                                                       int which, int row1, const float* __restrict__ featbuf,
                                                       const int32_t* __restrict__ rowlist, float* __restrict__ probs,
                                                       float* __restrict__ values) {
  __shared__ __attribute__((aligned(16))) float F[HB * HFS];
  __shared__ __attribute__((aligned(16))) float logit[HB * HLG];
  __shared__ float wv1[20 * HEADS_MAX_CELLS];
  __shared__ float hid[HB * 20];
  __shared__ float part[HB * 16];
  __shared__ float rsum[HB];
  __shared__ int orow[HB];
  int L, base, blk;
  bool second = false;
  if (which < 2) {
    L = counts[which];
    base = which ? counts[0] : 0;
    blk = blockIdx.x;
  } else {
    const int L0 = counts[0], nb0 = (L0 + HB - 1) / HB;
    second = (int)blockIdx.x >= nb0;
    L = second ? counts[1] : L0;
    base = second ? (row1 >= 0 ? row1 : L0) : 0;
    blk = second ? (int)blockIdx.x - nb0 : (int)blockIdx.x;
  }
  const int i0 = blk * HB;
  if (i0 >= L) return;
  const int nbrd = L - i0 < HB ? L - i0 : HB;
  const NetParams p = second ? p1 : p0;
  const int HW = p.HW, A = p.A, tid = threadIdx.x;
  const float slope = p.slope;
  {
    const float* src = featbuf + (size_t)(base + i0) * 3 * HW;
    const int total = nbrd * 3 * HW;
    for (int j0 = tid; j0 < total; j0 += 8 * NT) {
      float t[8];
#pragma unroll
      for (int u = 0; u < 8; ++u) t[u] = j0 + u * NT < total ? src[j0 + u * NT] : 0.f;
#pragma unroll
      for (int u = 0; u < 8; ++u) {
        const int j = j0 + u * NT;
        if (j < total) {
          const int i = j / (3 * HW), r = j - i * 3 * HW, o = (r >= HW) + (r >= 2 * HW);
          F[i * HFS + o * HPL + (r - o * HW)] = t[u];
        }
      }
    }
    static_assert(9 * NT >= 20 * HEADS_MAX_CELLS, "nine rounds of the block cover the value head's first matrix");
    float tw[9];
#pragma unroll
    for (int u = 0; u < 9; ++u) tw[u] = tid + u * NT < 20 * HW ? p.w_v1[tid + u * NT] : 0.f;
#pragma unroll
    for (int u = 0; u < 9; ++u)
      if (tid + u * NT < 20 * HW) wv1[tid + u * NT] = tw[u];
  }
  if (tid < HB) orow[tid] = tid < nbrd ? rowlist[base + i0 + tid] : 0;
  __syncthreads();
  const int wave = tid >> 6, lane = tid & 63;
  if (wave * 32 < A) {
    const int i = lane & 31, h = lane >> 5, a = wave * 32 + i;
    const bool av = a < A;
    const int nq = HW >> 2, rem = HW & 3;
    const int npair = (nq + 1) / 2;
    const size_t half = ((size_t)HW * A + 3) & ~(size_t)3;
    constexpr int U = 4;
    f32x16 acc;
#pragma unroll
    for (int r = 0; r < 16; ++r) acc[r] = 0.f;
    for (int pl = 0; pl < 2; ++pl) {
      const float* frow = F + i * HFS + (1 + pl) * HPL;
      const float* wh = p.w_pT + pl * half;
      const float4* wq = reinterpret_cast<const float4*>(wh) + (av ? a : 0);
      float4 bw[U], fa[U], bn[U], fn[U];
      auto fetch = [&](int g, float4* b_, float4* f_) {
#pragma unroll
        for (int u = 0; u < U; ++u) {
          const int q = 2 * (g * U + u) + h;
          const bool qv = q < nq && g * U + u < npair;
          b_[u] = (qv && av) ? wq[(size_t)q * A] : make_float4(0.f, 0.f, 0.f, 0.f);
          f_[u] = qv ? *reinterpret_cast<const float4*>(frow + 4 * q) : make_float4(0.f, 0.f, 0.f, 0.f);
        }
      };
      const int ngrp = (npair + U - 1) / U;
      fetch(0, bn, fn);
      for (int g = 0; g < ngrp; ++g) {
#pragma unroll
        for (int u = 0; u < U; ++u) { bw[u] = bn[u]; fa[u] = fn[u]; }
        if (g + 1 < ngrp) fetch(g + 1, bn, fn);
#pragma unroll
        for (int u = 0; u < U; ++u) {
          acc = __builtin_amdgcn_mfma_f32_32x32x2f32(fa[u].x, bw[u].x, acc, 0, 0, 0);
          acc = __builtin_amdgcn_mfma_f32_32x32x2f32(fa[u].y, bw[u].y, acc, 0, 0, 0);
          acc = __builtin_amdgcn_mfma_f32_32x32x2f32(fa[u].z, bw[u].z, acc, 0, 0, 0);
          acc = __builtin_amdgcn_mfma_f32_32x32x2f32(fa[u].w, bw[u].w, acc, 0, 0, 0);
        }
      }
      const float* wr = wh + (size_t)nq * A * 4;
      for (int r = 0; r < rem; ++r) {
        const float fr = h == 0 ? frow[4 * nq + r] : 0.f;
        const float br = (h == 0 && av) ? wr[(size_t)r * A + a] : 0.f;
        acc = __builtin_amdgcn_mfma_f32_32x32x2f32(fr, br, acc, 0, 0, 0);
      }
    }
    if (av) {
      const float bias = p.b_p[a];
#pragma unroll
      for (int r = 0; r < 16; ++r) logit[(8 * (r >> 2) + 4 * h + (r & 3)) * HLG + a] = acc[r] + bias;
    }
  }
  for (int k = tid; k < nbrd * 20; k += NT) {
    const int bi = k / 20, u = k - bi * 20;
    float s = p.b_v1[u];
    const float* w = wv1 + u * HW;
    const float* f = F + bi * HFS;
#pragma unroll 8
    for (int c = 0; c < HW; ++c) s = fmaf(f[c], w[c], s);
    hid[k] = leaky(s, slope);
  }
  __syncthreads();
  if (tid < nbrd) {
    float s = p.b_v2[0];
    for (int u = 0; u < 20; ++u) s = fmaf(hid[tid * 20 + u], p.w_v2[u], s);
    values[orow[tid]] = tanhf(s);
  }
  const int bi = tid >> 4, j = tid & 15;
  float* lg = logit + bi * HLG;
  float mx = -3.4e38f;
  for (int a = j; a < A; a += 16) mx = fmaxf(mx, lg[a]);
#pragma unroll
  for (int m = 1; m < 16; m <<= 1) mx = fmaxf(mx, __shfl_xor(mx, m, 16));
  float ps = 0.f;
  for (int a = j; a < A; a += 16) {
    const float e = expf(lg[a] - mx);
    lg[a] = e;
    ps += e;
  }
  part[tid] = ps;
  __syncthreads();
  if (j == 0) {
    float sum = 0.f;
#pragma unroll
    for (int q = 0; q < 16; ++q) sum += part[bi * 16 + q];
    rsum[bi] = sum;
  }
  __syncthreads();
  if (bi < nbrd) {
    const float sum = rsum[bi];
    float* out = probs + (size_t)orow[bi] * A;
    for (int a = j; a < A; a += 16) out[a] = lg[a] / sum;
  }
}


__global__ __launch_bounds__(256) void k_net_hash(int HW2, int A, unsigned long long salt0, unsigned long long salt1,
                                                  const float* __restrict__ planes,
                                                  const int32_t* __restrict__ counts, int which, int row1,
                                                  float* __restrict__ probs, float* __restrict__ values,
                                                  const int32_t* __restrict__ gpack, int gG, int gB) {
  const int lane = threadIdx.x & 63;
  const long long w = (long long)blockIdx.x * 4 + (threadIdx.x >> 6);
  long long row;
  int cls = 0;
  if (gpack) {
    const int g = (int)(w / gB), j = (int)(w - (long long)g * gB);
    if (g >= gG) return;
    const int v = gpack[g];
    if (j >= (v & 0xFF)) return;
    cls = v >> 8;
    row = w;
  } else if (which < 2) {
    if (w >= counts[which]) return;
    row = w + (which ? counts[0] : 0);
    cls = 0;
  } else {
    const int L0 = counts[0], L1 = counts[1];
    if (w < L0) { row = w; cls = 0; }
    else if (w < L0 + L1) { row = (row1 >= 0 ? row1 : L0) + (w - L0); cls = 1; }
    else return;
  }
  const float* pl = planes + (size_t)row * HW2;
  unsigned long long h = 0;
  for (int j = lane; j < HW2; j += 64)
    if (pl[j] != 0.0f) h += caro_mix64(0x5851f42d4c957f2dULL + (unsigned long long)j) | 1ULL;
#pragma unroll
  for (int m = 1; m < 64; m <<= 1) h += __shfl_xor(h, m, 64);
  h += cls ? salt1 : salt0;
  for (int a = lane; a < A; a += 64) {
    const unsigned long long ha = caro_mix64(h + 0x9E3779B97F4A7C15ULL * (unsigned long long)(a + 1));
    probs[(size_t)row * A + a] = (float)(((ha >> 20) & 1023ULL) + 1ULL) / 8192.0f;
  }
  if (lane == 0) {
    const unsigned long long hv = caro_mix64(h ^ 0xA5A5A5A5A5A5A5A5ULL);
    values[row] = (float)((long long)((hv >> 20) % 2001ULL) - 1000LL) / 1024.0f;
  }
}

}

extern "C" void caro__set_error(const char* msg);

struct caro_net {
  int kind;
  uint64_t salt;
  cnet::NetParams p;
  float* dev;
  float* ww_dev;
  uint32_t* wtab_dev;
  float* ww2_dev;
  float* wpT_dev;
  uint16_t* wx3_dev;
  struct HeadRows { void* stream; float* feat; int32_t* rowl; int64_t rows; uint64_t used; } hrows[8];
  int n_hrows;
  uint64_t hrows_clock;
  int64_t hrows_evictions;
  int device;
  unsigned long long* dbg_stamps;
};

static int nfail(int code, const std::string& m) {
  caro__set_error(m.c_str());
  return code;
}

static unsigned net_grid(const caro_net* n, int64_t max_rows) {
  int64_t grid = (max_rows + n->p.TB - 1) / n->p.TB;
  if (n->p.ww && n->p.ncu > 0) {
    const int64_t ncu = n->p.ncu, full = ncu * n->p.TB;
    const int tbs[2] = {n->p.TB4, n->p.TB2};
    for (int tb : tbs) {
      if (tb <= 0) continue;
      int64_t small = (max_rows + tb - 1) / tb;
      if (small > ncu) small = ncu;
      if (small > grid) grid = small;
      if (max_rows > full) {
        int64_t split = ncu + (max_rows - full + tb - 1) / tb;
        if (split > 2 * ncu) split = 2 * ncu;
        if (split > grid) grid = split;
      }
    }
  }
  return (unsigned)grid;
}

extern "C" {

static bool depth_ok(int depth) { return depth >= 1 && depth <= cnet::MAX_NRES; }
static int bad_depth(int depth) {
  return nfail(CARO_E_INVAL, "unsupported net depth " + std::to_string(depth) + ": the kernels run 1 .. " +
                                 std::to_string(cnet::MAX_NRES) + " residual blocks");
}

int64_t caro_net_packed_size_depth(int H, int W, int A, int depth) {
  if (!depth_ok(depth)) return bad_depth(depth);
  const int64_t HW = (int64_t)H * W;
  return 9 * 2 * 64 + 64 + (int64_t)depth * 9 * cnet::WCHUNK + depth * 64 + 3 * 64 + 3 +
         20 * HW + 20 + 20 + 1 + (int64_t)A * 2 * HW + A;
}
int64_t caro_net_packed_size(int H, int W, int A) { return caro_net_packed_size_depth(H, W, A, cnet::NRES); }
int caro_net_max_depth(void) { return cnet::MAX_NRES; }
int caro_net_depth(const caro_net* n) { return n && n->kind == 0 ? n->p.nres : 0; }

int caro_net_create(int H, int W, int A, float negative_slope, const float* packed_host, int64_t n_floats,
                    int device_id, caro_net** out) {
  return caro_net_create_depth(H, W, A, cnet::NRES, negative_slope, packed_host, n_floats, device_id, out);
}

int caro_net_create_depth(int H, int W, int A, int depth, float negative_slope, const float* packed_host,
                          int64_t n_floats, int device_id, caro_net** out) {
  if (!packed_host || !out) return nfail(CARO_E_INVAL, "null argument");
  if (H < 2 || W < 2 || H > 15 || W > 15 || A < 1 || A > 255) return nfail(CARO_E_INVAL, "unsupported board / action count");
  if (!depth_ok(depth)) return bad_depth(depth);
  if (n_floats != caro_net_packed_size_depth(H, W, A, depth))
    return nfail(CARO_E_INVAL, depth == cnet::NRES ? "packed weight buffer has the wrong size"
                                                   : "packed weight buffer has the wrong size for a net of " +
                                                         std::to_string(depth) + " residual blocks");
  int ndev = 0;
  if (hipGetDeviceCount(&ndev) != hipSuccess || ndev <= 0)
    return nfail(CARO_E_NODEV, "no HIP device: libcaro_hip needs a GPU (there is no CPU fallback)");
  if (device_id < 0 || device_id >= ndev) return nfail(CARO_E_INVAL, "device_id out of range");
  if (hipSetDevice(device_id) != hipSuccess) return nfail(CARO_E_HIP, "hipSetDevice failed");
  caro_net* n = new caro_net();
  n->kind = 0;
  n->salt = 0;
  n->device = device_id;
  n->ww_dev = nullptr;
  n->wtab_dev = nullptr;
  n->ww2_dev = nullptr;
  n->wpT_dev = nullptr;
  n->wx3_dev = nullptr;
  n->n_hrows = 0;
  n->hrows_clock = 0;
  n->hrows_evictions = 0;
  const size_t pad = (size_t)cnet::TPC * cnet::WCHUNK;
  if (hipMalloc((void**)&n->dev, (n_floats + pad) * sizeof(float)) != hipSuccess) {
    delete n;
    return nfail(CARO_E_NOMEM, "hipMalloc failed");
  }
  if (hipMemset(n->dev + n_floats, 0, pad * sizeof(float)) != hipSuccess ||
      hipMemcpy(n->dev, packed_host, n_floats * sizeof(float), hipMemcpyHostToDevice) != hipSuccess) {
    (void)hipFree(n->dev);
    delete n;
    return nfail(CARO_E_HIP, "hipMemcpy failed");
  }
  cnet::NetParams& p = n->p;
  const int HW = H * W;
  p.H = H; p.W = W; p.HW = HW; p.A = A; p.TB = 255 / HW; p.slope = negative_slope;
  if (p.TB * A > 1024 || p.TB > 32) p.TB = p.TB > 32 ? 32 : p.TB;
  const float* q = n->dev;
  p.w_in = q;   q += 9 * 2 * 64;
  p.b_in = q;   q += 64;
  p.nres = depth;
  p.w_res = q;  q += (size_t)depth * 9 * cnet::WCHUNK;
  p.b_res = q;  q += depth * 64;
  p.w_head = q; q += 3 * 64;
  p.b_head = q; q += 3;
  p.w_v1 = q;   q += 20 * HW;
  p.b_v1 = q;   q += 20;
  p.w_v2 = q;   q += 20;
  p.b_v2 = q;   q += 1;
  p.w_p = q;    q += (size_t)A * 2 * HW;
  p.b_p = q;    q += A;
  p.ww = nullptr;
  p.wtab = nullptr;
  p.ww2 = nullptr;
  p.w_pT = nullptr;
  p.wx3 = nullptr;
  p.ncu = 0; p.TB2 = 0; p.TB4 = 0;
  if (cnet::head_span_host(HW, A) > cnet::HEAD_STAGE_MAX) {
    const size_t half = ((size_t)HW * A + 3) & ~(size_t)3, np = 2 * half;
    const float* wp_host = packed_host + (p.w_p - n->dev);
    std::vector<float> t(np, 0.f);
    const int nq = HW / 4;
    for (int a = 0; a < A; ++a)
      for (int pl = 0; pl < 2; ++pl)
        for (int c = 0; c < HW; ++c) {
          const float w = wp_host[(size_t)a * 2 * HW + pl * HW + c];
          const size_t at = c < 4 * nq ? ((size_t)(c >> 2) * A + a) * 4 + (c & 3) : (size_t)nq * A * 4 + (size_t)(c - 4 * nq) * A + a;
          t[pl * half + at] = w;
        }
    if (hipMalloc((void**)&n->wpT_dev, np * sizeof(float)) != hipSuccess ||
        hipMemcpy(n->wpT_dev, t.data(), np * sizeof(float), hipMemcpyHostToDevice) != hipSuccess) {
      if (n->wpT_dev) (void)hipFree(n->wpT_dev);
      (void)hipFree(n->dev);
      delete n;
      return nfail(CARO_E_NOMEM, "hipMalloc / hipMemcpy failed");
    }
    p.w_pT = n->wpT_dev;
  }
  *out = n;
  return 0;
}

static int wrong_image(const caro_net* n, const char* what) {
  return nfail(CARO_E_INVAL, std::string(what) + " has the wrong size for this net's " + std::to_string(n->p.nres) +
                                 " residual blocks");
}
int64_t caro_net_winograd_size_depth(int depth) {
  return depth_ok(depth) ? (int64_t)depth * 12 * cnet::WCHUNK : bad_depth(depth);
}
int caro_net_enable_winograd(caro_net* n, const float* ww_host, int64_t n_floats) {
  if (!n || !ww_host) return nfail(CARO_E_INVAL, "null argument");
  if (n->kind != 0) return nfail(CARO_E_STATE, "not a conv net");
  if (n->p.ww2 || n->p.wx3) return nfail(CARO_E_STATE, "net is already in another arithmetic mode");
  const int64_t want = caro_net_winograd_size_depth(n->p.nres);
  if (n_floats != want) return wrong_image(n, "transformed weight image");
  if (hipSetDevice(n->device) != hipSuccess) return nfail(CARO_E_HIP, "hipSetDevice failed");
  if (!n->ww_dev && hipMalloc((void**)&n->ww_dev, want * sizeof(float)) != hipSuccess)
    return nfail(CARO_E_NOMEM, "hipMalloc failed");
  {
    std::vector<float> img((size_t)want);
    for (int layer = 0; layer < n->p.nres; ++layer)
      for (int dx = 0; dx < 3; ++dx)
        for (int hq = 0; hq < 2; ++hq)
          for (int pp = 0; pp < 4; ++pp)
            for (int h = 0; h < 2; ++h)
              for (int co = 0; co < 64; ++co)
                for (int g = 0; g < 4; ++g) {
                  const float* src = ww_host + ((size_t)(layer * 4 + pp) * 3 + dx) * cnet::WCHUNK + (h * 64 + co) * 32 +
                                     (((hq * 4 + g) ^ ((co >> 1) & 7)) << 2);
                  float* dst = img.data() + ((size_t)(layer * 3 + dx) * 2 + hq) * cnet::WCH +
                               ((pp * 2 + h) * 64 + co) * 16 + ((g ^ ((co >> 2) & 3)) << 2);
                  for (int j = 0; j < 4; ++j) dst[j] = src[j];
                }
    if (hipMemcpy(n->ww_dev, img.data(), want * sizeof(float), hipMemcpyHostToDevice) != hipSuccess)
      return nfail(CARO_E_HIP, "hipMemcpy failed");
  }
  const int H = n->p.H, W = n->p.W, HW = n->p.HW;
  const int tpb = ((H + 1) / 2) * W;
  if (tpb > 128) return nfail(CARO_E_INVAL, "board too large for the 128-tile workgroup");
  const int tbw = 128 / tpb;
  if (tbw < n->p.TB) n->p.TB = tbw;
  static const int kLanes[2][16] = {{0, 1, 2, 3, 12, 13, 14, 15, 20, 21, 22, 23, 24, 25, 26, 27},
                                    {4, 5, 6, 7, 8, 9, 10, 11, 16, 17, 18, 19, 28, 29, 30, 31}};
  std::vector<uint32_t> by_res[16], group[8], left;
  bool has[8][16] = {};
  for (int bi = 0; bi < n->p.TB; ++bi)
    for (int ty = 0; ty < (H + 1) / 2; ++ty)
      for (int x = 0; x < W; ++x)
        by_res[(bi * HW + 2 * ty * W + x) & 15].push_back((uint32_t)bi | (uint32_t)ty << 8 | (uint32_t)x << 16 | 1u << 24);
  int order[16];
  for (int r = 0; r < 16; ++r) order[r] = r;
  std::sort(order, order + 16, [&](int a, int b) { return by_res[a].size() > by_res[b].size(); });
  for (int oi = 0; oi < 16; ++oi) {
    const int r = order[oi];
    for (uint32_t t : by_res[r]) {
      int best = -1;
      for (int g = 0; g < 8; ++g)
        if (!has[g][r] && group[g].size() < 16 && (best < 0 || group[g].size() < group[best].size())) best = g;
      if (best < 0) {
        left.push_back(t);
      } else {
        has[best][r] = true;
        group[best].push_back(t);
      }
    }
  }
  for (uint32_t t : left) {
    int best = 0;
    for (int g = 1; g < 8; ++g)
      if (group[g].size() < group[best].size()) best = g;
    group[best].push_back(t);
  }
  uint32_t tab[128] = {};
  for (int g = 0; g < 8; ++g)
    for (size_t k = 0; k < group[g].size(); ++k) tab[(g >> 1) * 32 + kLanes[g & 1][k]] = group[g][k];
  if (!n->wtab_dev && hipMalloc((void**)&n->wtab_dev, sizeof(tab)) != hipSuccess) return nfail(CARO_E_NOMEM, "hipMalloc failed");
  if (hipMemcpy(n->wtab_dev, tab, sizeof(tab), hipMemcpyHostToDevice) != hipSuccess) return nfail(CARO_E_HIP, "hipMemcpy failed");
  n->p.wtab = n->wtab_dev;
  n->p.ww = n->ww_dev;
  int ncu = 0;
  if (hipDeviceGetAttribute(&ncu, hipDeviceAttributeMultiprocessorCount, n->device) != hipSuccess) ncu = 0;
  const char* off = getenv("CARO_NO_SPLIT_TILES");
  if (off && off[0] == '1') ncu = 0;
  n->p.ncu = ncu;
  n->p.TB2 = 64 / tpb < n->p.TB ? 64 / tpb : 0;
  if (n->p.TB2 * H * W > cnet::XROW2) n->p.TB2 = 0;
  n->p.TB4 = 32 / tpb < n->p.TB ? 32 / tpb : 0;
  if (n->p.TB4 * H * W > cnet::XROW4) n->p.TB4 = 0;
  return 0;
}

int caro_net_winograd2d_size(void) { return cnet::W2NCHUNK * cnet::WCH; }
int64_t caro_net_winograd2d_size_depth(int depth) {
  return depth_ok(depth) ? (int64_t)depth * 8 * cnet::WCH : bad_depth(depth);
}
int caro_net_winograd2d_supported(int H, int W) {
  return (H * W >= 128 && H * W <= cnet::HEADS_MAX_CELLS && ((H + 1) / 2) <= 8 && ((W + 1) / 2) <= 8) ? 1 : 0;
}
int caro_net_enable_winograd2d(caro_net* n, const float* ww2_host, int64_t n_floats) {
  if (!n || !ww2_host) return nfail(CARO_E_INVAL, "null argument");
  if (n->kind != 0) return nfail(CARO_E_STATE, "not a conv net");
  if (n->p.ww || n->p.wx3) return nfail(CARO_E_STATE, "net is already in another arithmetic mode");
  if (!caro_net_winograd2d_supported(n->p.H, n->p.W))
    return nfail(CARO_E_INVAL, "2-D Winograd form: boards of one per workgroup with at most 8 x 8 tiles (12x12 .. 15x15)");
  const int64_t want = caro_net_winograd2d_size_depth(n->p.nres);
  if (n_floats != want) return wrong_image(n, "transformed weight image");
  if (!n->p.w_pT) return nfail(CARO_E_STATE, "2-D Winograd form: the batched heads need the transposed policy matrix");
  if (hipSetDevice(n->device) != hipSuccess) return nfail(CARO_E_HIP, "hipSetDevice failed");
  if (!n->ww2_dev && hipMalloc((void**)&n->ww2_dev, want * sizeof(float)) != hipSuccess)
    return nfail(CARO_E_NOMEM, "hipMalloc failed");
  if (hipMemcpy(n->ww2_dev, ww2_host, want * sizeof(float), hipMemcpyHostToDevice) != hipSuccess)
    return nfail(CARO_E_HIP, "hipMemcpy failed");
  n->p.TB = 1;
  n->p.ww2 = n->ww2_dev;
  return 0;
}

int64_t caro_net_split_bf16_size(void) { return (int64_t)cnet::NTAPS * cnet::X3_TAP_U4 * 8; }
int64_t caro_net_split_bf16_size_depth(int depth) {
  return depth_ok(depth) ? (int64_t)depth * 9 * cnet::X3_TAP_U4 * 8 : bad_depth(depth);
}
int caro_net_enable_split_bf16(caro_net* n, const uint16_t* parts_host, int64_t n_u16) {
  if (!n || !parts_host) return nfail(CARO_E_INVAL, "null argument");
  if (n->kind != 0) return nfail(CARO_E_STATE, "not a conv net");
  if (n->p.ww || n->p.ww2) return nfail(CARO_E_STATE, "net is already in another arithmetic mode");
  if (n->p.nres != cnet::NRES)
    return nfail(CARO_E_INVAL, "bf16x3 form: built for nets of " + std::to_string(cnet::NRES) + " residual blocks only, this net has " +
                                   std::to_string(n->p.nres) + " (use a float32 mode)");
  const int64_t want = caro_net_split_bf16_size();
  if (n_u16 != want) return wrong_image(n, "split weight image");
  if (hipSetDevice(n->device) != hipSuccess) return nfail(CARO_E_HIP, "hipSetDevice failed");
  const size_t pad = (size_t)cnet::X3_PAD_TAPS * cnet::X3_TAP_U4 * 8;
  if (!n->wx3_dev) {
    if (hipMalloc((void**)&n->wx3_dev, (want + pad) * sizeof(uint16_t)) != hipSuccess) return nfail(CARO_E_NOMEM, "hipMalloc failed");
    if (hipMemset(n->wx3_dev + want, 0, pad * sizeof(uint16_t)) != hipSuccess) return nfail(CARO_E_HIP, "hipMemset failed");
  }
  if (hipMemcpy(n->wx3_dev, parts_host, want * sizeof(uint16_t), hipMemcpyHostToDevice) != hipSuccess)
    return nfail(CARO_E_HIP, "hipMemcpy failed");
  n->p.wx3 = n->wx3_dev;
  return 0;
}

int64_t caro_net_stream_evictions(const caro_net* n) { return n ? n->hrows_evictions : 0; }

void caro_net_destroy(caro_net* n) {
  if (!n) return;
  if (n->ww_dev) (void)hipFree(n->ww_dev);
  if (n->wtab_dev) (void)hipFree(n->wtab_dev);
  if (n->ww2_dev) (void)hipFree(n->ww2_dev);
  if (n->wpT_dev) (void)hipFree(n->wpT_dev);
  if (n->wx3_dev) (void)hipFree(n->wx3_dev);
  for (int k = 0; k < n->n_hrows; ++k) {
    if (n->hrows[k].feat) (void)hipFree(n->hrows[k].feat);
    if (n->hrows[k].rowl) (void)hipFree(n->hrows[k].rowl);
  }
  if (n->dev) (void)hipFree(n->dev);
  delete n;
}

int caro_net_create_hash(int H, int W, int A, uint64_t salt, int device_id, caro_net** out) {
  if (!out) return nfail(CARO_E_INVAL, "null argument");
  if (H < 2 || W < 2 || H > 15 || W > 15 || A < 1 || A > 255) return nfail(CARO_E_INVAL, "unsupported board / action count");
  int ndev = 0;
  if (hipGetDeviceCount(&ndev) != hipSuccess || ndev <= 0)
    return nfail(CARO_E_NODEV, "no HIP device: libcaro_hip needs a GPU (there is no CPU fallback)");
  if (device_id < 0 || device_id >= ndev) return nfail(CARO_E_INVAL, "device_id out of range");
  caro_net* n = new caro_net();
  memset(&n->p, 0, sizeof n->p);
  n->kind = 1;
  n->salt = salt;
  n->device = device_id;
  n->dev = nullptr;
  n->ww_dev = nullptr;
  n->wtab_dev = nullptr;
  n->ww2_dev = nullptr;
  n->wpT_dev = nullptr;
  n->wx3_dev = nullptr;
  n->n_hrows = 0;
  n->hrows_clock = 0;
  n->hrows_evictions = 0;
  n->p.H = H; n->p.W = W; n->p.HW = H * W; n->p.A = A; n->p.TB = 4;
  *out = n;
  return 0;
}

static int head_rows_for(caro_net* n0, void* stream, int64_t need, caro_net::HeadRows** out) {
  caro_net::HeadRows* hr = nullptr;
  for (int k = 0; k < n0->n_hrows; ++k)
    if (n0->hrows[k].stream == stream) hr = &n0->hrows[k];
  if (!hr) {
    if (n0->n_hrows == 8) {
      hr = &n0->hrows[0];
      for (int k = 1; k < 8; ++k)
        if (n0->hrows[k].used < hr->used) hr = &n0->hrows[k];
      if (hipDeviceSynchronize() != hipSuccess) return nfail(CARO_E_HIP, "hipDeviceSynchronize failed");
      n0->hrows_evictions += 1;
      hr->stream = stream;
    } else {
      hr = &n0->hrows[n0->n_hrows++];
      hr->stream = stream; hr->feat = nullptr; hr->rowl = nullptr; hr->rows = 0;
    }
  }
  hr->used = ++n0->hrows_clock;
  if (hr->rows < need) {
    if (hr->feat) (void)hipFree(hr->feat);
    if (hr->rowl) (void)hipFree(hr->rowl);
    hr->feat = nullptr; hr->rowl = nullptr; hr->rows = 0;
    if (hipMalloc((void**)&hr->feat, (size_t)need * 3 * n0->p.HW * sizeof(float)) != hipSuccess ||
        hipMalloc((void**)&hr->rowl, (size_t)need * sizeof(int32_t)) != hipSuccess)
      return nfail(CARO_E_NOMEM, "hipMalloc of the head feature rows failed");
    hr->rows = need;
  }
  *out = hr;
  return 0;
}

static int net_launch(caro_net* n0, caro_net* n1, const float* planes_dev, const int32_t* counts_dev, int which,
                      int row1, int64_t max_rows, float* probs_dev, float* values_dev, const int32_t* gpack, int G,
                      int B, unsigned long long* stamps, void* stream, const int32_t* slist = nullptr) {
  hipStream_t st = (hipStream_t)stream;
  if (n0->kind == 1) {
    const int64_t waves = gpack ? (int64_t)G * B : max_rows;
    const unsigned grid = (unsigned)((waves + 3) / 4);
    hipLaunchKernelGGL(cnet::k_net_hash, dim3(grid), dim3(256), 0, st, 2 * n0->p.HW, n0->p.A,
                       (unsigned long long)n0->salt, (unsigned long long)n1->salt, planes_dev, counts_dev, which, row1,
                       probs_dev, values_dev, gpack, G, B);
  } else {
    const unsigned grid = net_grid(n0, max_rows) + (which == 2 ? 1u : 0u);
    const bool d5 = n0->p.nres == cnet::NRES && n1->p.nres == cnet::NRES;
    if (n0->p.ww2) {
      caro_net::HeadRows* hr = nullptr;
      if (int rc = head_rows_for(n0, stream, max_rows + (row1 > 0 ? row1 : 0) + 64, &hr)) return rc;
      hipLaunchKernelGGL(d5 ? cnet::k_net_forward_w2 : cnet::k_net_forward_w2_any, dim3(grid), dim3(cnet::NT), 0, st,
                         n0->p, n1->p, planes_dev, counts_dev, which, row1, probs_dev, values_dev,
                         stamps ? stamps : n0->dbg_stamps, gpack, G, B, hr->feat, hr->rowl, slist);
      if (hipGetLastError() != hipSuccess) return nfail(CARO_E_HIP, "net kernel launch failed");
      const unsigned hgrid = (unsigned)((max_rows + cnet::HB - 1) / cnet::HB) + (which == 2 ? 1u : 0u);
      hipLaunchKernelGGL(cnet::k_net_heads, dim3(hgrid), dim3(cnet::NT), 0, st, n0->p, n1->p, counts_dev, which, row1,
                         hr->feat, hr->rowl, probs_dev, values_dev);
    }
    else if (n0->p.ww)
      hipLaunchKernelGGL(d5 ? cnet::k_net_forward_w : cnet::k_net_forward_w_any, dim3(grid), dim3(cnet::NT), 0, st,
                         n0->p, n1->p, planes_dev, counts_dev, which, row1, probs_dev, values_dev,
                         stamps ? stamps : n0->dbg_stamps, gpack, G, B);
    else if (n0->p.wx3) {
      const bool batched = n0->p.TB == 1 && n0->p.w_pT && n0->p.HW <= cnet::HEADS_MAX_CELLS;
      caro_net::HeadRows* hr = nullptr;
      if (batched)
        if (int rc = head_rows_for(n0, stream, max_rows + (row1 > 0 ? row1 : 0) + 64, &hr)) return rc;
      hipLaunchKernelGGL(cnet::k_net_forward_x3, dim3(grid), dim3(cnet::NT), 0, st, n0->p, n1->p, planes_dev,
                         counts_dev, which, row1, probs_dev, values_dev, stamps, gpack, G, B, hr ? hr->feat : nullptr,
                         hr ? hr->rowl : nullptr);
      if (hr) {
        if (hipGetLastError() != hipSuccess) return nfail(CARO_E_HIP, "net kernel launch failed");
        const unsigned hgrid = (unsigned)((max_rows + cnet::HB - 1) / cnet::HB) + (which == 2 ? 1u : 0u);
        hipLaunchKernelGGL(cnet::k_net_heads, dim3(hgrid), dim3(cnet::NT), 0, st, n0->p, n1->p, counts_dev, which, row1,
                           hr->feat, hr->rowl, probs_dev, values_dev);
      }
    }
    else
      hipLaunchKernelGGL(d5 ? cnet::k_net_forward : cnet::k_net_forward_any, dim3(grid), dim3(cnet::NT), 0, st, n0->p,
                         n1->p, planes_dev, counts_dev, which, row1, probs_dev, values_dev, stamps, gpack, G, B);
  }
  if (hipGetLastError() != hipSuccess) return nfail(CARO_E_HIP, "net kernel launch failed");
  return 0;
}
static int pair_ok(const caro_net* n0, const caro_net* n1) {
  if (n0->p.H != n1->p.H || n0->p.W != n1->p.W || n0->p.A != n1->p.A) return nfail(CARO_E_INVAL, "nets differ in shape");
  if (n0->kind != n1->kind || 
      (n0->p.ww == nullptr) != (n1->p.ww == nullptr) || (n0->p.ww2 == nullptr) != (n1->p.ww2 == nullptr) ||
      (n0->p.wx3 == nullptr) != (n1->p.wx3 == nullptr))
    return nfail(CARO_E_INVAL, "nets differ in kind / arithmetic mode");
  return 0;
}

int caro_net_boards_per_workgroup(const caro_net* n) { return n ? n->p.TB : 0; }
int caro_net_uses_slot_list(const caro_net* n) { return n && n->p.ww2 ? 1 : 0; }

int caro_net_forward(caro_net* n, const float* planes_dev, const int32_t* counts_dev, int which, int64_t max_rows,
                     float* probs_dev, float* values_dev, void* stream) {
  if (!n || !planes_dev || !counts_dev || !probs_dev || !values_dev) return nfail(CARO_E_INVAL, "null argument");
  if (which != 0 && which != 1) return nfail(CARO_E_INVAL, "which must be 0 or 1");
  if (max_rows <= 0) return 0;
  return net_launch(n, n, planes_dev, counts_dev, which, -1, max_rows, probs_dev, values_dev, nullptr, 0, 0, nullptr,
                    stream);
}

int caro_net_forward_pair_at(caro_net* n0, caro_net* n1, const float* planes_dev, const int32_t* counts_dev,
                             int64_t row1_base, int64_t max_rows, float* probs_dev, float* values_dev, void* stream) {
  if (!n0 || !n1 || !planes_dev || !counts_dev || !probs_dev || !values_dev) return nfail(CARO_E_INVAL, "null argument");
  if (int rc = pair_ok(n0, n1)) return rc;
  if (max_rows <= 0) return 0;
  return net_launch(n0, n1, planes_dev, counts_dev, 2, (int)row1_base, max_rows, probs_dev, values_dev, nullptr, 0, 0,
                    nullptr, stream);
}

int caro_net_forward_pair(caro_net* n0, caro_net* n1, const float* planes_dev, const int32_t* counts_dev,
                          int64_t max_rows, float* probs_dev, float* values_dev, void* stream) {
  return caro_net_forward_pair_at(n0, n1, planes_dev, counts_dev, -1, max_rows, probs_dev, values_dev, stream);
}

int caro_net_forward_slots(caro_net* n0, caro_net* n1, const float* planes_dev, const int32_t* counts_dev,
                           const int32_t* gpack_dev, int n_games, int batch, float* probs_dev, float* values_dev,
                           void* stream) {
  if (!n0 || !planes_dev || !counts_dev || !gpack_dev || !probs_dev || !values_dev)
    return nfail(CARO_E_INVAL, "null argument");
  if (n_games < 1 || batch < 1 || batch > 255) return nfail(CARO_E_INVAL, "bad slot geometry");
  if (n1)
    if (int rc = pair_ok(n0, n1)) return rc;
  return net_launch(n0, n1 ? n1 : n0, planes_dev, counts_dev, n1 ? 2 : 0, -1, (int64_t)n_games * batch, probs_dev,
                    values_dev, gpack_dev, n_games, batch, nullptr, stream);
}

int caro_net_forward_slot_list(caro_net* n0, caro_net* n1, const float* planes_dev, const int32_t* counts_dev,
                               const int32_t* gpack_dev, const int32_t* slot_list_dev, int n_games, int batch,
                               float* probs_dev, float* values_dev, void* stream) {
  if (!n0 || !planes_dev || !counts_dev || !gpack_dev || !probs_dev || !values_dev)
    return nfail(CARO_E_INVAL, "null argument");
  if (n_games < 1 || batch < 1 || batch > 255) return nfail(CARO_E_INVAL, "bad slot geometry");
  if (n1)
    if (int rc = pair_ok(n0, n1)) return rc;
  return net_launch(n0, n1 ? n1 : n0, planes_dev, counts_dev, n1 ? 2 : 0, -1, (int64_t)n_games * batch, probs_dev,
                    values_dev, gpack_dev, n_games, batch, nullptr, stream, n0->p.ww2 ? slot_list_dev : nullptr);
}

int caro_net_forward_stamped(caro_net* n, const float* planes_dev, const int32_t* counts_dev, int which,
                             int64_t max_rows, float* probs_dev, float* values_dev, uint64_t* stamps_dev,
                             void* stream) {
  if (!n || !stamps_dev) return nfail(CARO_E_INVAL, "null argument");
  if (n->kind != 0) return nfail(CARO_E_STATE, "stamps: conv kernels only");
  return net_launch(n, n, planes_dev, counts_dev, which, -1, max_rows, probs_dev, values_dev, nullptr, 0, 0,
                    (unsigned long long*)stamps_dev, stream);
}

int caro_net_debug_stamps(caro_net* n, uint64_t* stamps_dev) {
  if (!n) return nfail(CARO_E_INVAL, "null argument");
  n->dbg_stamps = (unsigned long long*)stamps_dev;
  return 0;
}

}
```

caro_ai_amd/csrc/caro_net_kernels.inc:

```

__global__ __launch_bounds__(NT, 2) void CARO_KN(k_net_forward)(NetParams p0, NetParams p1, const float* __restrict__ planes,
                                                         const int32_t* __restrict__ counts, int which, int row1,
                                                         float* __restrict__ probs, float* __restrict__ values,
                                                         unsigned long long* __restrict__ stamps,
                                                         const int32_t* __restrict__ gpack, int gG, int gB) {
  __shared__ __attribute__((aligned(16))) float lds[LDS_FLOATS];
  float* act = lds;
  float* wbuf = lds + ACT;

  int L, row0, board0;
  bool second = false;
  if (which < 2) {
    L = counts[which];
    row0 = which ? counts[0] : 0;
    board0 = blockIdx.x * p0.TB;
  } else {
    const int L0 = counts[0];
    const int t0 = (L0 + p0.TB - 1) / p0.TB;
    second = (int)blockIdx.x >= t0;
    L = second ? counts[1] : L0;
    row0 = second ? (row1 >= 0 ? row1 : L0) : 0;
    board0 = (second ? (int)blockIdx.x - t0 : (int)blockIdx.x) * p0.TB;
  }
  if (board0 >= L) return;
  const NetParams p = second ? p1 : p0;
  const float slope = p.slope;
  unsigned long long t_c0 = 0, t_r0 = 0;
  if (stamps) {
    t_c0 = __builtin_amdgcn_s_memtime();
    t_r0 = __builtin_amdgcn_s_memrealtime();
  }
  const int nb = min(p.TB, L - board0);
  const int HW = p.HW;
  const int R = nb * HW;
  const int tid = threadIdx.x;
  const int wave = tid >> 6, lane = tid & 63;
  const int i = lane & 31, h = lane >> 5;

  for (int k = tid; k < ACT / 4; k += NT) reinterpret_cast<float4*>(lds)[k] = make_float4(0.f, 0.f, 0.f, 0.f);
  for (int k = tid; k < 9 * 2 * NF; k += NT) wbuf[k] = p.w_in[k];
  int* smap = reinterpret_cast<int*>(wbuf + 1536);
  tile_rows(gpack, gG, gB, second ? 1 : 0, row0 + board0, board0, nb, smap + 64, smap, tid);

  conv_in_f32(p, planes, smap, act, wbuf, R, tid);
  const int slot_v = tid < nb ? smap[tid] : 0;
  __syncthreads();

  unsigned long long t_trunk0 = 0;
  if (stamps) t_trunk0 = __builtin_amdgcn_s_memtime();
  {
    const float4* src = reinterpret_cast<const float4*>(p.w_res);
#pragma unroll
    for (int m = 0; m < 2 * TPC; ++m) reinterpret_cast<float4*>(wbuf)[tid + NT * m] = src[tid + NT * m];
  }
  __syncthreads();

  const int myrow = wave * 32 + i;
  const bool rvalid = myrow < R;
  const int rbi = myrow / HW;
  const int rcell = myrow - rbi * HW;
  const int ry = rcell / p.W, rx = rcell - ry * p.W;
  const int bswz = (i >> 1) & 7;

  f32x16 acc0, acc1;
#pragma unroll
  for (int e = 0; e < 16; ++e) {
    acc0[e] = 0.f;
    acc1[e] = 0.f;
  }
  static_assert(TPC == 3, "the staging registers below are written out for three taps per chunk");
  float4 wn0, wn1, wn2, wn3, wn4, wn5;
  wn0 = wn1 = wn2 = wn3 = wn4 = wn5 = make_float4(0.f, 0.f, 0.f, 0.f);
  const int ntaps = (CARO_NR ? CARO_NR : p.nres) * 9, nchunk = (ntaps + TPC - 1) / TPC;
  for (int ft = 0; ft < ntaps; ++ft) {
    const int c = ft / TPC, within = ft % TPC, cur = c & 1;
    const int layer = ft / 9, tap = ft % 9;
    const bool last_in_chunk = within == TPC - 1 || ft == ntaps - 1;
    const bool has_next = c + 1 < nchunk;
    if (within == 0 && has_next) {
      const float4* src = reinterpret_cast<const float4*>(p.w_res + (size_t)(c + 1) * TPC * WCHUNK);
      wn0 = src[tid];
      wn1 = src[tid + NT];
      wn2 = src[tid + 2 * NT];
      wn3 = src[tid + 3 * NT];
      wn4 = src[tid + 4 * NT];
      wn5 = src[tid + 5 * NT];
    }
    const float* wcur = wbuf + cur * TPC * WCHUNK + within * WCHUNK;
    const int ny = ry + tap / 3 - 1, nx = rx + tap % 3 - 1;
    const bool ok = rvalid && ny >= 0 && ny < p.H && nx >= 0 && nx < p.W;
    const int nrow = ok ? rbi * HW + ny * p.W + nx : ZROW;
    const float* abase = act + nrow * NF;
    const int aswz = nrow & 15;
    const float* bbase0 = wcur + (h * 64 + i) * 32;
    const float* bbase1 = wcur + (h * 64 + 32 + i) * 32;
#define CARO_LOAD_SET(A_, B0_, B1_, Q_)                                                             \
  A_ = *reinterpret_cast<const float4*>(abase + (((h * 8 + (Q_)) ^ aswz) << 2));                    \
  B0_ = *reinterpret_cast<const float4*>(bbase0 + (((Q_) ^ bswz) << 2));                            \
  B1_ = *reinterpret_cast<const float4*>(bbase1 + (((Q_) ^ bswz) << 2));
#define CARO_MFMA_SET(A_, B0_, B1_)                                                \
  acc0 = __builtin_amdgcn_mfma_f32_32x32x2f32(A_.x, B0_.x, acc0, 0, 0, 0);        \
  acc1 = __builtin_amdgcn_mfma_f32_32x32x2f32(A_.x, B1_.x, acc1, 0, 0, 0);        \
  acc0 = __builtin_amdgcn_mfma_f32_32x32x2f32(A_.y, B0_.y, acc0, 0, 0, 0);        \
  acc1 = __builtin_amdgcn_mfma_f32_32x32x2f32(A_.y, B1_.y, acc1, 0, 0, 0);        \
  acc0 = __builtin_amdgcn_mfma_f32_32x32x2f32(A_.z, B0_.z, acc0, 0, 0, 0);        \
  acc1 = __builtin_amdgcn_mfma_f32_32x32x2f32(A_.z, B1_.z, acc1, 0, 0, 0);        \
  acc0 = __builtin_amdgcn_mfma_f32_32x32x2f32(A_.w, B0_.w, acc0, 0, 0, 0);        \
  acc1 = __builtin_amdgcn_mfma_f32_32x32x2f32(A_.w, B1_.w, acc1, 0, 0, 0);
    float4 xa, xb0, xb1, ya, yb0, yb1;
    CARO_LOAD_SET(xa, xb0, xb1, 0)
#pragma unroll
    for (int q = 0; q < 8; q += 2) {
      CARO_LOAD_SET(ya, yb0, yb1, q + 1)
      __builtin_amdgcn_sched_barrier(0);
      CARO_MFMA_SET(xa, xb0, xb1)
      __builtin_amdgcn_sched_barrier(0);
      if (q + 2 < 8) {
        CARO_LOAD_SET(xa, xb0, xb1, q + 2)
      }
      __builtin_amdgcn_sched_barrier(0);
      CARO_MFMA_SET(ya, yb0, yb1)
      __builtin_amdgcn_sched_barrier(0);
    }
#undef CARO_LOAD_SET
#undef CARO_MFMA_SET
    if (last_in_chunk && has_next) {
      float4* dst = reinterpret_cast<float4*>(wbuf + (cur ^ 1) * TPC * WCHUNK);
      dst[tid] = wn0;
      dst[tid + NT] = wn1;
      dst[tid + 2 * NT] = wn2;
      dst[tid + 3 * NT] = wn3;
      dst[tid + 4 * NT] = wn4;
      dst[tid + 5 * NT] = wn5;
    }
    if (tap == 8) {
      __syncthreads();
      const float* bias = p.b_res + layer * NF;
      const float bc0 = bias[i], bc1 = bias[32 + i];
      float old0[16], old1[16];
#pragma unroll
      for (int e = 0; e < 16; ++e) {
        const int row = wave * 32 + (e & 3) + 8 * (e >> 2) + 4 * h;
        old0[e] = act[aoff(row, i)];
        old1[e] = act[aoff(row, 32 + i)];
      }
#pragma unroll
      for (int e = 0; e < 16; ++e) {
        const int row = wave * 32 + (e & 3) + 8 * (e >> 2) + 4 * h;
        const bool real = row < R;
        const float n0 = old0[e] + leaky(acc0[e] + bc0, slope);
        const float n1 = old1[e] + leaky(acc1[e] + bc1, slope);
        act[aoff(row, i)] = real ? n0 : 0.f;
        act[aoff(row, 32 + i)] = real ? n1 : 0.f;
        acc0[e] = 0.f;
        acc1[e] = 0.f;
      }
    }
    if (last_in_chunk || tap == 8) __syncthreads();
  }
  unsigned long long t_trunk1 = 0;
  if (stamps) t_trunk1 = __builtin_amdgcn_s_memtime();
  heads_f32<false>(p, act, wbuf, probs, values, slot_v, nb, R, tid);
  if (stamps && tid == 0) {
    stamps[4 * blockIdx.x] = __builtin_amdgcn_s_memtime() - t_c0;
    stamps[4 * blockIdx.x + 1] = __builtin_amdgcn_s_memrealtime() - t_r0;
    stamps[4 * blockIdx.x + 2] = t_trunk0 - t_c0;
    stamps[4 * blockIdx.x + 3] = t_trunk1 - t_c0;
  }
}

__global__ __launch_bounds__(NT, 2) void CARO_KN(k_net_forward_w)(NetParams p0, NetParams p1,
                                                           const float* __restrict__ planes,
                                                           const int32_t* __restrict__ counts, int which, int row1,
                                                           float* __restrict__ probs, float* __restrict__ values,
                                                           unsigned long long* __restrict__ stamps,
                                                           const int32_t* __restrict__ gpack, int gG, int gB) {
  __shared__ __attribute__((aligned(256))) float lds[LDS_FLOATS];
  float* act = lds;
  float* wbuf = lds + ACT;

  const unsigned long long t_abs0 = stamps ? __builtin_amdgcn_s_memrealtime() : 0;
  const int gcpt = gpack ? (gG + NT - 1) / NT : 0;
  const bool gpre = gpack && gcpt <= GP_PRE;
  int gv[GP_PRE];
#pragma unroll
  for (int u = 0; u < GP_PRE; ++u) {
    const int g = (int)threadIdx.x * gcpt + u;
    gv[u] = gpre && u < gcpt && g < gG ? gpack[g] : 0;
  }
  int L, row0, board0, nb, nb_cap = p0.TB;
  int ks = 1;
  bool second = false;
  if (which < 2) {
    L = counts[which];
    row0 = which ? counts[0] : 0;
    board0 = blockIdx.x * p0.TB;
    const int full = p0.ncu * p0.TB;
    if (p0.ncu > 0) {
      if (p0.TB4 > 0 && L <= p0.ncu * p0.TB4) ks = 4;
      else if (p0.TB2 > 0 && L <= p0.ncu * p0.TB2) ks = 2;
      if (ks > 1) {
        nb_cap = ks == 4 ? p0.TB4 : p0.TB2;
        board0 = (int)blockIdx.x * nb_cap;
      } else if (L > full) {
        const int over = L - full;
        if (p0.TB4 > 0 && over <= p0.ncu * p0.TB4) ks = 4;
        else if (p0.TB2 > 0 && over <= p0.ncu * p0.TB2) ks = 2;
        if (ks > 1) {
          if ((int)blockIdx.x < p0.ncu) {
            ks = 1;
          } else {
            nb_cap = ks == 4 ? p0.TB4 : p0.TB2;
            board0 = full + ((int)blockIdx.x - p0.ncu) * nb_cap;
          }
        }
      }
    }
  } else {
    const int L0 = counts[0], L1 = counts[1];
    if (p0.ncu > 1) {
      if (p0.TB4 > 0 && L0 + L1 <= (p0.ncu - 1) * p0.TB4) ks = 4;
      else if (p0.TB2 > 0 && L0 + L1 <= (p0.ncu - 1) * p0.TB2) ks = 2;
      if (ks > 1) nb_cap = ks == 4 ? p0.TB4 : p0.TB2;
    }
    const int t0 = (L0 + nb_cap - 1) / nb_cap;
    second = (int)blockIdx.x >= t0;
    L = second ? L1 : L0;
    row0 = second ? (row1 >= 0 ? row1 : L0) : 0;
    board0 = (second ? (int)blockIdx.x - t0 : (int)blockIdx.x) * nb_cap;
  }
  if (board0 >= L) return;
  const NetParams p = second ? p1 : p0;
  unsigned long long t_c0 = 0, t_r0 = 0;
  if (stamps) {
    t_c0 = __builtin_amdgcn_s_memtime();
    t_r0 = __builtin_amdgcn_s_memrealtime();
  }
  nb = min(nb_cap, L - board0);
  const int HW = p.HW;
  const int R = nb * HW;
  const int tid = threadIdx.x;

  int gmine = 0;
#pragma unroll
  for (int u = 0; u < GP_PRE; ++u) gmine += (gv[u] >> 8) == (second ? 1 : 0) ? (gv[u] & 0xFF) : 0;
  asm volatile("" : "+v"(gmine));
  float* win = wbuf + 2 * WCH;
  if (tid < 320) dma_b128(reinterpret_cast<const float4*>(p.w_in) + tid,
                          __builtin_amdgcn_readfirstlane(lds_addr(win) + (unsigned)(tid >> 6) * 1024u));
  fetch_chunk(p.ww, 0, lds_addr(wbuf), tid);
  fetch_chunk(p.ww, 1, lds_addr(wbuf), tid);
  for (int k = tid + (R * NF) / 4; k < ACT / 4; k += NT) reinterpret_cast<float4*>(lds)[k] = make_float4(0.f, 0.f, 0.f, 0.f);
  static_assert(2 * (WCH / 4 / NT) == 8, "s_waitcnt vmcnt(8) below counts 2 chunks x WCH / 4 / NT transfers per thread");
  static_assert(320 * 4 >= 9 * 2 * NF, "the 320-lane transfer must cover w_in [9][2][64]");
  asm volatile("s_waitcnt vmcnt(8)" ::: "memory");
  int* smap = reinterpret_cast<int*>(win + 1536);
  if (gpre) tile_rows_pre(gv, gcpt, gmine, gB, second ? 1 : 0, board0, nb, smap + 64, smap, tid);
  else tile_rows(gpack, gG, gB, second ? 1 : 0, row0 + board0, board0, nb, smap + 64, smap, tid);
  conv_in_mfma(p, planes, smap, act, win, R, tid);
  const int slot_v = tid < nb ? smap[tid] : 0;
  unsigned long long t_trunk0 = 0;
  if (stamps) t_trunk0 = __builtin_amdgcn_s_memtime();
  asm volatile("s_waitcnt vmcnt(0)" ::: "memory");
  __syncthreads();
  const int hspan = head_span(HW, p.A) <= HEAD_STAGE_MAX ? head_span(HW, p.A) : 0;
  if (ks == 1) trunk_w<1, CARO_NR>(p, act, wbuf, nb, tid, hspan);
  else if (ks == 2) trunk_w<2, CARO_NR>(p, act, wbuf, nb, tid, hspan);
  else trunk_w<4, CARO_NR>(p, act, wbuf, nb, tid, hspan);
  unsigned long long t_trunk1 = 0;
  if (stamps) t_trunk1 = __builtin_amdgcn_s_memtime();
  if (hspan) heads_f32<true>(p, act, wbuf, probs, values, slot_v, nb, R, tid);
  else heads_f32<false>(p, act, wbuf, probs, values, slot_v, nb, R, tid);
  if (stamps && tid == 0) {
    stamps[4 * blockIdx.x] = __builtin_amdgcn_s_memtime() - t_c0;
    stamps[4 * blockIdx.x + 1] = gpack ? ((__builtin_amdgcn_s_memrealtime() - t_abs0) & 0xFFFFFull) | (t_abs0 << 20)
                                       : __builtin_amdgcn_s_memrealtime() - t_r0;
    stamps[4 * blockIdx.x + 2] = t_trunk0 - t_c0;
    stamps[4 * blockIdx.x + 3] = t_trunk1 - t_c0;
  }
}

__global__ __launch_bounds__(NT, 2) void CARO_KN(k_net_forward_w2)(NetParams p0, NetParams p1,
                                                            const float* __restrict__ planes,
                                                            const int32_t* __restrict__ counts, int which, int row1,
                                                            float* __restrict__ probs, float* __restrict__ values,
                                                            unsigned long long* __restrict__ stamps,
                                                            const int32_t* __restrict__ gpack, int gG, int gB,
                                                            float* __restrict__ featbuf, int32_t* __restrict__ rowlist,
                                                            const int32_t* __restrict__ slist) {
  __shared__ __attribute__((aligned(256))) float lds[LDS_FLOATS];
  float* act = lds;
  float* wbuf = lds + ACT;
  const int gcpt = gpack && !slist ? (gG + NT - 1) / NT : 0;
  const bool gpre = gpack && !slist && gcpt <= GP_PRE;
  int gv[GP_PRE];
#pragma unroll
  for (int u = 0; u < GP_PRE; ++u) {
    const int g = (int)threadIdx.x * gcpt + u;
    gv[u] = gpre && u < gcpt && g < gG ? gpack[g] : 0;
  }
  int L, row0, board0;
  bool second = false;
  if (which < 2) {
    L = counts[which];
    row0 = which ? counts[0] : 0;
    board0 = blockIdx.x;
  } else {
    const int L0 = counts[0];
    second = (int)blockIdx.x >= L0;
    L = second ? counts[1] : L0;
    row0 = second ? (row1 >= 0 ? row1 : L0) : 0;
    board0 = second ? (int)blockIdx.x - L0 : (int)blockIdx.x;
  }
  if (board0 >= L) return;
  const int listed = slist ? slist[(second ? gG * gB : 0) + board0] : 0;
  const NetParams p = second ? p1 : p0;
  unsigned long long t_c0 = 0, t_r0 = 0;
  if (stamps) {
    t_c0 = __builtin_amdgcn_s_memtime();
    t_r0 = __builtin_amdgcn_s_memrealtime();
  }
  const int nb = 1;
  const int HW = p.HW;
  const int R = HW;
  const int tid = threadIdx.x;
  int gmine = 0;
#pragma unroll
  for (int u = 0; u < GP_PRE; ++u) gmine += (gv[u] >> 8) == (second ? 1 : 0) ? (gv[u] & 0xFF) : 0;
  asm volatile("" : "+v"(gmine));
  float* win = wbuf + 2 * WCH;
  if (tid < 320) dma_b128(reinterpret_cast<const float4*>(p.w_in) + tid,
                          __builtin_amdgcn_readfirstlane(lds_addr(win) + (unsigned)(tid >> 6) * 1024u));
  fetch_chunk_s(p.ww2, 0, lds_addr(wbuf), tid);
  fetch_chunk_s(p.ww2, 1, lds_addr(wbuf), tid);
  for (int k = tid + (R * NF) / 4; k < ACT / 4; k += NT) reinterpret_cast<float4*>(lds)[k] = make_float4(0.f, 0.f, 0.f, 0.f);
  static_assert(2 * (WCH / 4 / NT) == 8, "s_waitcnt vmcnt(8) below counts 2 chunks x WCH / 4 / NT transfers per thread");
  asm volatile("s_waitcnt vmcnt(8)" ::: "memory");
  int* smap = reinterpret_cast<int*>(win + 1536);
  if (slist) {
    if (tid == 0) smap[0] = listed;
    __syncthreads();
  } else if (gpre) tile_rows_pre(gv, gcpt, gmine, gB, second ? 1 : 0, board0, nb, smap + 64, smap, tid);
  else tile_rows(gpack, gG, gB, second ? 1 : 0, row0 + board0, board0, nb, smap + 64, smap, tid);
  conv_in_mfma<true>(p, planes, smap, act, win, R, tid);
  const int slot_v = tid < nb ? smap[tid] : 0;
  unsigned long long t_trunk0 = 0;
  if (stamps) t_trunk0 = __builtin_amdgcn_s_memtime();
  asm volatile("s_waitcnt vmcnt(0)" ::: "memory");
  __syncthreads();
  trunk_w2d<CARO_NR>(p, act, wbuf, tid);
  unsigned long long t_trunk1 = 0;
  if (stamps) t_trunk1 = __builtin_amdgcn_s_memtime();
  heads_f32<false, true>(p, act, wbuf, probs, values, slot_v, nb, R, tid, featbuf, rowlist, row0 + board0);
  if (stamps && tid == 0) {
    stamps[4 * blockIdx.x] = __builtin_amdgcn_s_memtime() - t_c0;
    stamps[4 * blockIdx.x + 1] = __builtin_amdgcn_s_memrealtime() - t_r0;
    stamps[4 * blockIdx.x + 2] = t_trunk0 - t_c0;
    stamps[4 * blockIdx.x + 3] = t_trunk1 - t_c0;
  }
}
```

caro_ai_amd/net_hip.py:

```python
import ctypes as C

import numpy as np
import torch

from caro_ai_amd import _lib
from caro_ai_amd.lib.model import Net, _fold


def pack_net(net: Net) -> np.ndarray:
    net = net.eval()
    H, W = net.input_shape[1], net.input_shape[2]
    parts = []
    w0, b0 = _fold(net.conv_in)
    parts += [w0.permute(2, 3, 1, 0).reshape(9, 2, 64), b0]
    co = np.arange(64)[None, :, None]
    h = np.arange(2)[:, None, None]
    j = np.arange(32)[None, None, :]
    idx = ((h * 64 + co) * 32 + ((((j >> 2) ^ ((co >> 1) & 7)) << 2) | (j & 3))).reshape(-1)
    ci = np.broadcast_to(h * 32 + j, (2, 64, 32)).reshape(-1)
    cc = np.broadcast_to(co, (2, 64, 32)).reshape(-1)
    res_w, res_b = [], []
    for blk in net.residual_blocks():
        w, b = _fold(blk)
        w = w.cpu().numpy()
        chunks = np.zeros((9, 4096), np.float32)
        for tap in range(9):
            chunks[tap, idx] = w[cc, ci, tap // 3, tap % 3]
        res_w.append(chunks)
        res_b.append(b.cpu().numpy())
    parts += [np.stack(res_w), np.stack(res_b)]
    wv, bv = _fold(net.conv_val)
    wp, bp = _fold(net.conv_policy)
    parts += [torch.cat([wv, wp]).reshape(3, 64), torch.cat([bv, bp])]
    parts += [net.value[0].weight, net.value[0].bias, net.value[2].weight.reshape(-1), net.value[2].bias]
    parts += [net.policy[0].weight, net.policy[0].bias]
    flat = [np.ascontiguousarray(p.detach().cpu().numpy() if torch.is_tensor(p) else p, dtype=np.float32).reshape(-1)
            for p in parts]
    out = np.concatenate(flat)
    assert out.size == _lib.load().caro_net_packed_size_depth(H, W, net.actions_n, net.n_residual), out.size
    return out


def _lds_image_index():
    co = np.arange(64)[None, :, None]
    h = np.arange(2)[:, None, None]
    j = np.arange(32)[None, None, :]
    idx = ((h * 64 + co) * 32 + ((((j >> 2) ^ ((co >> 1) & 7)) << 2) | (j & 3))).reshape(-1)
    ci = np.broadcast_to(h * 32 + j, (2, 64, 32)).reshape(-1)
    cc = np.broadcast_to(co, (2, 64, 32)).reshape(-1)
    return idx, cc, ci


_WINO_G = np.array([[1.0, 0.0, 0.0], [0.5, 0.5, 0.5], [0.5, -0.5, 0.5], [0.0, 0.0, 1.0]])


def pack_net_w(net: Net) -> np.ndarray:
    net = net.eval()
    idx, cc, ci = _lds_image_index()
    out = np.zeros((net.n_residual, 4, 3, 4096), np.float32)
    for li, blk in enumerate(net.residual_blocks()):
        w, _ = _fold(blk)
        w = w.cpu().numpy().astype(np.float64)
        u = np.einsum("pk,oikx->pxoi", _WINO_G, w)
        for pp in range(4):
            for dx in range(3):
                out[li, pp, dx, idx] = u[pp, dx][cc, ci].astype(np.float32)
    assert out.size == _lib.load().caro_net_winograd_size_depth(net.n_residual), out.size
    return out.reshape(-1)


W2_PHASE_B = ((1, 2), (0, 3))


def wino2d_weights(w: np.ndarray) -> np.ndarray:
    return np.einsum("ak,bl,oikl->aboi", _WINO_G, _WINO_G, w.astype(np.float64))


def pack_net_w2(net: Net) -> np.ndarray:
    net = net.eval()
    out = np.zeros((net.n_residual, 8, 2, 4, 2, 64, 8), np.float32)
    co = np.arange(64)
    for li, blk in enumerate(net.residual_blocks()):
        w, _ = _fold(blk)
        u = wino2d_weights(w.cpu().numpy())
        for phase in range(2):
            for bh in range(2):
                b = W2_PHASE_B[phase][bh]
                for cq in range(4):
                    for gi in range(2):
                        G = 2 * cq + gi
                        for h in range(2):
                            ch = 32 * h + 4 * G
                            blk4 = u[:, b, :, ch:ch + 4].astype(np.float32)
                            slot = gi ^ ((co >> 3) & 1)
                            for a in range(4):
                                for sl in range(2):
                                    m = slot == sl
                                    out[li, phase * 4 + cq, bh, a, h, m, sl * 4:sl * 4 + 4] = blk4[a, m]
    assert out.size == _lib.load().caro_net_winograd2d_size_depth(net.n_residual), out.size
    return out.reshape(-1)


def bf16_round(x: np.ndarray) -> np.ndarray:
    u = np.ascontiguousarray(x, np.float32).view(np.uint32).astype(np.uint64)
    return ((u + 0x7FFF + ((u >> 16) & 1)) >> 16).astype(np.uint16)


def bf16_value(b: np.ndarray) -> np.ndarray:
    return (b.astype(np.uint32) << 16).view(np.float32)


def split_bf16x3(x: np.ndarray):
    x = np.ascontiguousarray(x, np.float32)
    hi = bf16_round(x)
    r1 = x - bf16_value(hi)
    mid = bf16_round(r1)
    r2 = r1 - bf16_value(mid)
    lo = bf16_round(r2)
    return hi, mid, lo


def pack_net_x3(net: Net) -> np.ndarray:
    net = net.eval()
    out = np.zeros((net.n_residual, 9, 2, 3, 4, 64, 8), np.uint16)
    for li, blk in enumerate(net.residual_blocks()):
        w, _ = _fold(blk)
        w = w.detach().cpu().numpy().astype(np.float32)
        for tap in range(9):
            wt = w[:, :, tap // 3, tap % 3].reshape(64, 2, 4, 8).transpose(1, 2, 0, 3)
            for part, bits in enumerate(split_bf16x3(wt)):
                out[li, tap, :, part] = bits
    assert out.size == _lib.load().caro_net_split_bf16_size_depth(net.n_residual), out.size
    return out.reshape(-1)


def wino2d_pays(H: int, W: int) -> bool:
    L = _lib.load()
    if not L.caro_net_winograd2d_supported(H, W):
        return False
    rows = -(-(((H + 1) // 2) * W) // 32) * 32
    return 64 * 16 <= 0.75 * rows * 12


class HipNet:

    device_counts = True

    def __init__(self, net: Net, device="cuda:0", negative_slope=0.01, mode="f32w", split_tiles=True):
        self.L = _lib.load()
        self.device = torch.device(device)
        self.H, self.W = net.input_shape[1], net.input_shape[2]
        self.A = net.actions_n
        self.depth = net.n_residual
        size = self.L.caro_net_packed_size_depth(self.H, self.W, self.A, self.depth)
        if size < 0:
            _lib.check(size)
        if mode == "bf16x3" and self.depth != 5:
            raise _lib.CaroError("net mode bf16x3 is built for nets of 5 residual blocks only, this net has %d: "
                                 "use a float32 mode (f32w, f32)" % self.depth)
        packed = pack_net(net)
        h = C.c_void_p()
        torch.cuda.set_device(self.device)
        _lib.check(self.L.caro_net_create_depth(self.H, self.W, self.A, self.depth, negative_slope, packed.ctypes.data,
                                                packed.size, self.device.index or 0, C.byref(h)))
        self.h = h
        assert self.L.caro_net_depth(self.h) == self.depth
        if mode == "f32w":
            mode = "f32w2" if wino2d_pays(self.H, self.W) else "f32w1"
        self.mode = mode
        if mode == "f32w2":
            w2 = pack_net_w2(net)
            _lib.check(self.L.caro_net_enable_winograd2d(self.h, w2.ctypes.data, w2.size))
        elif mode == "f32w1":
            ww = pack_net_w(net)
            import os
            old = os.environ.get("CARO_NO_SPLIT_TILES")
            if not split_tiles:
                os.environ["CARO_NO_SPLIT_TILES"] = "1"
            try:
                _lib.check(self.L.caro_net_enable_winograd(self.h, ww.ctypes.data, ww.size))
            finally:
                if not split_tiles:
                    if old is None:
                        del os.environ["CARO_NO_SPLIT_TILES"]
                    else:
                        os.environ["CARO_NO_SPLIT_TILES"] = old
        elif mode == "bf16x3":
            wx = pack_net_x3(net)
            _lib.check(self.L.caro_net_enable_split_bf16(self.h, wx.ctypes.data, wx.size))
        else:
            assert mode == "f32", mode

    def close(self):
        if getattr(self, "h", None):
            self.L.caro_net_destroy(self.h)
            self.h = None

    def __del__(self):
        try:
            self.close()
        except Exception:
            pass

    def workgroup_mfma_flops(self):
        K = self.depth
        if self.mode == "f32w2":
            return K * 16 * 4 * 32 * 4096.0
        if self.mode == "bf16x3":
            return 9 * K * 96 * 8 * 16384.0
        taps = {"f32w1": 12 * K, "f32": 9 * K}.get(self.mode)
        return None if taps is None else taps * 32 * 8 * 4096.0

    def forward_dev(self, planes, counts_dev_ptr, which, max_rows, probs, values, stream):
        _lib.check(self.L.caro_net_forward(self.h, planes.data_ptr(), counts_dev_ptr, which, max_rows,
                                           probs.data_ptr(), values.data_ptr(), stream))

    def __call__(self, planes):
        L = planes.shape[0]
        counts = torch.tensor([L, 0], dtype=torch.int32, device=planes.device)
        probs = torch.empty((L, self.A), dtype=torch.float32, device=planes.device)
        values = torch.empty(L, dtype=torch.float32, device=planes.device)
        st = C.c_void_p(torch.cuda.current_stream(planes.device).cuda_stream)
        self.forward_dev(planes.contiguous(), counts.data_ptr(), 0, L, probs, values, st)
        return probs, values


def weights_version(net):
    return tuple((t._version, t.data_ptr()) for t in net.state_dict(keep_vars=True).values())


_HIPNETS = {}
HIPNET_CACHE = 4


def hipnet_for(net: Net, device="cuda:0", mode="f32w", split_tiles=True) -> HipNet:
    key = (id(net), str(torch.device(device)), mode, bool(split_tiles))
    ver = weights_version(net)
    hit = _HIPNETS.pop(key, None)
    if hit is None or hit[0] != ver:
        hit = (ver, HipNet(net, device, mode=mode, split_tiles=split_tiles))
    _HIPNETS[key] = hit
    while len(_HIPNETS) > HIPNET_CACHE:
        _HIPNETS.pop(next(iter(_HIPNETS)))
    return hit[1]


def release_hipnets():
    _HIPNETS.clear()


class HashNet:

    device_counts = True

    def __init__(self, game_or_shape, actions_n=None, device="cuda:0", salt=0):
        shape = getattr(game_or_shape, "obs_shape", game_or_shape)
        self.H, self.W = int(shape[1]), int(shape[2])
        self.A = int(actions_n if actions_n is not None else game_or_shape.action_space)
        self.L = _lib.load()
        self.device = torch.device(device)
        self.salt = int(salt)
        h = C.c_void_p()
        torch.cuda.set_device(self.device)
        _lib.check(self.L.caro_net_create_hash(self.H, self.W, self.A, self.salt, self.device.index or 0, C.byref(h)))
        self.h = h

    close = HipNet.close
    __del__ = HipNet.__del__
    forward_dev = HipNet.forward_dev
    __call__ = HipNet.__call__
```

include/caro_hip.h:

```cpp
#ifndef CARO_HIP_H
#define CARO_HIP_H

#include <stdint.h>

#ifdef __cplusplus
extern "C" {
#endif

#define CARO_GAME_CONNECT4 0
#define CARO_GAME_MNK 1
#define CARO_GAME_CARO 2

#define CARO_E_INVAL (-22)
#define CARO_E_NOMEM (-12)
#define CARO_E_HIP (-5)
#define CARO_E_NODEV (-19)
#define CARO_E_STATE (-71)

#define CARO_RESIGNED (-2)

typedef struct caro_engine caro_engine;

typedef struct caro_config {
  int32_t game_kind;
  int32_t n, k;
  int32_t n_games;
  int32_t n_stores;
  int32_t n_nets;
  int32_t max_batch;
  int32_t node_cap;
  int32_t steps_before_tau_0;
  int32_t first_player_mode;
  float c_puct;
  double alpha, explore;
  uint64_t seed;
  uint64_t uid_base;
  uint64_t uid_stride;
  int32_t device_id;
  int32_t evict;
  int32_t stagger;
  int32_t stagger_recycle;
  int64_t games_limit;
} caro_config;

const char* caro_last_error(void);
int caro_version(void);

int caro_key_words(int game_kind, int n);
int caro_action_space(int game_kind, int n);
int caro_obs_cells(int game_kind, int n);

int caro_host_initial(int game_kind, int n, int k, uint64_t* key);
int caro_host_move(int game_kind, int n, int k, uint64_t* key, int move, int player, int* won);
int caro_host_legal(int game_kind, int n, int k, const uint64_t* key, uint8_t* legal);
int caro_host_encode(int game_kind, int n, int k, const uint64_t* key, int who_move, float* planes);
int caro_host_noise_row(uint64_t seed, uint64_t uid, uint32_t ply, uint32_t sim, int A, double alpha, double* out);
double caro_host_move_uniform(uint64_t seed, uint64_t uid, uint32_t ply);
double caro_host_resign_uniform(uint64_t seed, uint64_t uid);
double caro_host_cap_uniform(uint64_t seed, uint64_t uid, uint32_t ply);
double caro_host_open_uniform(uint64_t seed, uint64_t uid, uint32_t i);
int caro_host_opening(int game_kind, int n, int k, uint64_t seed, uint64_t uid, int first, int max_plies,
                      uint64_t* key_out, int* player_out, int* made_out);

int caro_host_forced_root(int A, const int32_t* N, const float* P, const double* noise, const uint8_t* legal,
                          double explore, double k, uint8_t* forced_out);
int caro_host_forced_prune(int A, const int32_t* N, const double* Q, const float* P, float c_puct, double k,
                           int32_t* N_out);

int caro_host_fpu_level(int A, int root, const int32_t* N, const float* W, const float* Q, const float* P,
                        const int32_t* strong, const uint8_t* legal, const double* noise, float c_puct, double explore,
                        float q_up, double reduction, double* scores_out);

int caro_host_vl_level(int A, int root, const int32_t* N, const float* W, const float* Q, const float* P,
                       const int32_t* strong, const uint8_t* legal, const double* noise, float c_puct, double explore,
                       const int32_t* c, int n_vl, double* scores_out);

int caro_host_temperature(int A, const int32_t* N, double tau, double* pi_out);

int caro_rules_move_batch(int game_kind, int n, int k, int64_t M, uint64_t* keys_dev, const int32_t* moves_dev,
                          const int32_t* players_dev, int32_t* won_dev, int32_t* full_dev, void* stream);
int caro_rules_legal_batch(int game_kind, int n, int k, int64_t M, const uint64_t* keys_dev, uint8_t* legal_dev,
                           void* stream);
int caro_rules_encode_batch(int game_kind, int n, int k, int64_t M, const uint64_t* keys_dev,
                            const int32_t* who_dev, float* planes_dev, void* stream);
int caro_noise_batch(uint64_t seed, int64_t M, int A, double alpha, const uint64_t* uid_dev, const uint32_t* ply_dev,
                     const uint32_t* sim_dev, double* out_dev, void* stream);

int caro_openings_batch(int game_kind, int n, int k, uint64_t seed, int max_plies, int64_t M, const uint64_t* uid_dev,
                        const int32_t* first_dev, uint64_t* keys_dev, int32_t* players_dev, int32_t* made_dev,
                        void* stream);

int caro_engine_create(const caro_config* cfg, caro_engine** out);
void caro_engine_destroy(caro_engine* h);
int caro_engine_restart(caro_engine* h, const caro_config* cfg, void* stream);
int caro_reset_games(caro_engine* h, const int32_t* first_player_dev, void* stream);
int caro_set_roots(caro_engine* h, const uint64_t* keys_dev, const int32_t* players_dev, void* stream);

int caro_select(caro_engine* h, int batch, int mb_index, const double* noise_dev, float* planes_dev,
                uint64_t* leaf_keys_dev, void* stream);
int caro_get_descent(caro_engine* h, int game, int b, int32_t* info_dev, float* value_dev, uint64_t* leaf_key_dev,
                     uint64_t* path_keys_dev, int32_t* path_actions_dev, void* stream);
int caro_select_cancel(caro_engine* h);
int caro_leaf_counts(caro_engine* h, int32_t counts[2], void* stream);
int caro_leaf_counts_dev(caro_engine* h, const int32_t** counts_dev);
int caro_expand_backup(caro_engine* h, const float* probs_dev, const float* values_dev, void* stream);

int caro_policy(caro_engine* h, double* pi_dev, int32_t* counts_dev, void* stream);
int caro_step(caro_engine* h, const double* uniforms_dev, int32_t* actions_dev, int32_t* done_dev,
              int32_t* result_dev, void* stream);
int caro_drain_tuples(caro_engine* h, int64_t cap, uint64_t* states_dev, int32_t* players_dev, double* pi_dev,
                      int32_t* z_dev, int64_t* games_dev, int recycle, int64_t* n_tuples, int64_t* n_games,
                      void* stream);
int caro_drain_tuples_begin(caro_engine* h, int64_t cap, uint64_t* states_dev, int32_t* players_dev, double* pi_dev,
                            int32_t* z_dev, int64_t* games_dev, int recycle, void* stream);
int caro_drain_tuples_end(caro_engine* h, int64_t* n_tuples, int64_t* n_games);

int caro_engine_set_resign(caro_engine* h, double threshold, double playthrough);
int caro_drain_tuples_begin_q(caro_engine* h, int64_t cap, uint64_t* states_dev, int32_t* players_dev, double* pi_dev,
                              int32_t* z_dev, int64_t* games_dev, int recycle, double* root_q_dev, void* stream);
int caro_drain_parked_begin_q(caro_engine* h, int64_t cap, uint64_t* states_dev, int32_t* players_dev, double* pi_dev,
                              int32_t* z_dev, int64_t* games_dev, double* root_q_dev, void* stream);

int caro_engine_set_playout_cap(caro_engine* h, double p_full, int fast);
int caro_drain_tuples_begin_x(caro_engine* h, int64_t cap, uint64_t* states_dev, int32_t* players_dev, double* pi_dev,
                              int32_t* z_dev, int64_t* games_dev, int recycle, double* root_q_dev, uint8_t* full_dev,
                              void* stream);
int caro_drain_parked_begin_x(caro_engine* h, int64_t cap, uint64_t* states_dev, int32_t* players_dev, double* pi_dev,
                              int32_t* z_dev, int64_t* games_dev, double* root_q_dev, uint8_t* full_dev, void* stream);

int caro_engine_set_early_stop(caro_engine* h, int min_minibatches);

int caro_engine_set_openings(caro_engine* h, int max_plies);

int caro_engine_set_forced_playouts(caro_engine* h, double k);
int caro_forced_stats(caro_engine* h, int64_t out[4], void* stream);

int caro_engine_set_fpu(caro_engine* h, double reduction, double root_reduction);

int caro_engine_set_virtual_loss(caro_engine* h, int n_vl);

int caro_engine_set_temperature(caro_engine* h, double tau_early, double tau_late, int visit_targets);

int caro_pool_open(caro_engine* h, int64_t M, const int32_t* games_dev, const uint64_t* uid_dev,
                   const int32_t* first_player_dev, void* stream);
int caro_pool_set(caro_engine* h, int64_t M, const int32_t* games_dev, const uint64_t* keys_dev,
                  const int32_t* players_dev, const int32_t* ply_dev, void* stream);
int caro_pool_select(caro_engine* h, int64_t M, const int32_t* games_dev, void* stream);
int caro_pool_hold(caro_engine* h, void* stream);
int caro_pool_level(caro_engine* h, int64_t M, const int32_t* games_dev, const int32_t* net_dev, const double* tau_dev,
                    void* stream);
int caro_pool_select_budget(caro_engine* h, int64_t M, const int32_t* games_dev, const int32_t* budget_dev, void* stream);

int caro_principal_lines(caro_engine* h, int64_t M, const int32_t* games_dev, int store, int top, int depth,
                         int32_t* n_lines_dev, int32_t* root_visits_dev, int32_t* len_dev, int32_t* end_dev,
                         int32_t* move_dev, int32_t* N_dev, float* W_dev, float* Q_dev, float* P_dev,
                         int32_t* strong_dev, void* stream);
int caro_host_line_heads(int A, const int32_t* N, int top, int32_t* heads_out);

int caro_engine_set_kernel_form(caro_engine* h, int form);
int caro_engine_kernel_form(const caro_engine* h);

typedef struct caro_drain_extra {
  uint32_t size;
  double* root_q_dev;
  uint8_t* full_dev;
  uint16_t* minibatches_dev;
  int16_t* open_dev;
} caro_drain_extra;
int caro_drain_tuples_begin_ex(caro_engine* h, int64_t cap, uint64_t* states_dev, int32_t* players_dev, double* pi_dev,
                               int32_t* z_dev, int64_t* games_dev, int recycle, const caro_drain_extra* extra,
                               void* stream);
int caro_drain_parked_begin_ex(caro_engine* h, int64_t cap, uint64_t* states_dev, int32_t* players_dev, double* pi_dev,
                               int32_t* z_dev, int64_t* games_dev, const caro_drain_extra* extra, void* stream);

int caro_counters(caro_engine* h, int64_t counters[8], void* stream);
int caro_profile_enable(caro_engine* h, int on);
int caro_profile_begin(caro_engine* h, int kind, void* stream);
void caro_profile_end(caro_engine* h, int slot, void* stream);
int caro_profile_read(caro_engine* h, double ms[8], int64_t launches[8], int reset);
int caro_debug_stamps(caro_engine* h, int on);
int caro_debug_read(caro_engine* h, uint64_t* out_host, int64_t n_u64, void* stream);
int caro_debug_sqrt_check(uint32_t n_max, uint64_t* bad_host);
int caro_live_games(caro_engine* h, int32_t* live, void* stream);
int caro_pending_leaves(caro_engine* h, int32_t* pending, void* stream);

int caro_tree_sizes(caro_engine* h, int32_t* out_dev, void* stream);
int caro_tree_live(caro_engine* h, int32_t* out_dev, void* stream);
int caro_lookup_nodes(caro_engine* h, int64_t M, const int32_t* game_dev, const int32_t* store_dev,
                      const uint64_t* keys_dev, int32_t* found_dev, int32_t* N_dev, float* W_dev, float* Q_dev,
                      float* P_dev, int32_t* strong_dev, void* stream);
int caro_get_roots(caro_engine* h, uint64_t* keys_dev, int32_t* players_dev, int32_t* ply_dev, uint64_t* uid_dev,
                   void* stream);
int caro_poke_nodes(caro_engine* h, int64_t M, const int32_t* game_dev, const int32_t* store_dev,
                    const uint64_t* keys_dev, const int32_t* N_dev, const float* W_dev, const float* Q_dev,
                    const float* P_dev, const int32_t* strong_dev, void* stream);
int caro_backup_path(caro_engine* h, int game, int store, float value, int value_is_f32, int len,
                     const uint64_t* keys_dev, const int32_t* actions_dev, void* stream);
int caro_dump_tree(caro_engine* h, int game, int store, int64_t cap, uint64_t* keys_dev, int32_t* N_dev,
                   float* W_dev, float* Q_dev, float* P_dev, int32_t* strong_dev, int64_t* n_nodes, void* stream);

typedef struct caro_net caro_net;
int64_t caro_net_packed_size(int H, int W, int A);
int caro_net_create(int H, int W, int A, float negative_slope, const float* packed_host, int64_t n_floats,
                    int device_id, caro_net** out);
int caro_net_max_depth(void);
int64_t caro_net_packed_size_depth(int H, int W, int A, int depth);
int caro_net_create_depth(int H, int W, int A, int depth, float negative_slope, const float* packed_host,
                          int64_t n_floats, int device_id, caro_net** out);
int caro_net_depth(const caro_net* n);
int64_t caro_net_winograd_size_depth(int depth);
int caro_net_enable_winograd(caro_net* n, const float* ww_host, int64_t n_floats);
int caro_net_winograd2d_size(void);
int64_t caro_net_winograd2d_size_depth(int depth);
int caro_net_winograd2d_supported(int H, int W);
int caro_net_enable_winograd2d(caro_net* n, const float* ww2_host, int64_t n_floats);
int64_t caro_net_split_bf16_size(void);
int64_t caro_net_split_bf16_size_depth(int depth);
int caro_net_enable_split_bf16(caro_net* n, const uint16_t* parts_host, int64_t n_u16);
int64_t caro_net_stream_evictions(const caro_net* n);
void caro_net_destroy(caro_net* n);
int caro_net_boards_per_workgroup(const caro_net* n);
int caro_net_uses_slot_list(const caro_net* n);
int caro_net_forward(caro_net* n, const float* planes_dev, const int32_t* counts_dev, int which, int64_t max_rows,
                     float* probs_dev, float* values_dev, void* stream);

int caro_net_forward_slots(caro_net* n0, caro_net* n1, const float* planes_dev, const int32_t* counts_dev,
                           const int32_t* gpack_dev, int n_games, int batch, float* probs_dev, float* values_dev,
                           void* stream);

int caro_net_forward_slot_list(caro_net* n0, caro_net* n1, const float* planes_dev, const int32_t* counts_dev,
                               const int32_t* gpack_dev, const int32_t* slot_list_dev, int n_games, int batch,
                               float* probs_dev, float* values_dev, void* stream);

int caro_net_create_hash(int H, int W, int A, uint64_t salt, int device_id, caro_net** out);

int caro_stream_create_partition(int device_id, int part, int nparts, void** stream_out);
int caro_stream_destroy(void* stream);
int caro_net_forward_pair(caro_net* n0, caro_net* n1, const float* planes_dev, const int32_t* counts_dev,
                          int64_t max_rows, float* probs_dev, float* values_dev, void* stream);
int caro_net_forward_pair_at(caro_net* n0, caro_net* n1, const float* planes_dev, const int32_t* counts_dev,
                             int64_t row1_base, int64_t max_rows, float* probs_dev, float* values_dev, void* stream);
int caro_net_forward_stamped(caro_net* n, const float* planes_dev, const int32_t* counts_dev, int which,
                             int64_t max_rows, float* probs_dev, float* values_dev, uint64_t* stamps_dev,
                             void* stream);
int caro_net_debug_stamps(caro_net* n, uint64_t* stamps_dev);
int caro_search_batch(caro_engine* h, caro_net* net0, caro_net* net1, int searches, int batch,
                      const double* noise_dev, float* planes_dev, uint64_t* leaf_keys_dev, float* probs_dev,
                      float* values_dev, void* stream);

int caro_search_move(caro_engine* h, caro_net* net0, caro_net* net1, int searches, int batch, const double* noise_dev,
                     const double* uniforms_dev, float* planes_dev, uint64_t* leaf_keys_dev, float* probs_dev,
                     float* values_dev, int32_t* actions_dev, int32_t* done_dev, int32_t* result_dev, void* stream);

int caro_search_staggered(caro_engine* h, caro_net* net0, caro_net* net1, int launches, int batch, float* planes_dev,
                          uint64_t* leaf_keys_dev, float* probs_dev, float* values_dev, void* stream);
int caro_drain_parked_begin(caro_engine* h, int64_t cap, uint64_t* states_dev, int32_t* players_dev, double* pi_dev,
                            int32_t* z_dev, int64_t* games_dev, void* stream);

#ifdef __cplusplus
}
#endif
#endif
```

Before: 8.488 million.

## Add a Connect4 shape-specialized single-net Winograd forward kernel

Templates the conv-in, trunk and head routines on a shape policy so the board size, action count and tile counts can be compile-time constants. It then instantiates a Connect4 (6x7, 7 actions) single-net variant of the Winograd forward kernel and dispatches to it when the net parameters match, with an environment variable and API call to force the general kernel. The aim is cheaper index math (constant divisions), fewer live registers and less branching per launch. The head loop also switches from division to shift-based indexing. This adds code size and a second kernel path that has to stay consistent with the general one.

```diff
diff --git a/caro_ai_amd/_lib.py b/caro_ai_amd/_lib.py
--- a/caro_ai_amd/_lib.py
+++ b/caro_ai_amd/_lib.py
@@ -90,6 +90,9 @@
     "caro_net_enable_split_bf16": (C.c_int, [_P, _P, C.c_int64]),
     "caro_net_boards_per_workgroup": (C.c_int, [_P]),
     "caro_net_uses_slot_list": (C.c_int, [_P]),
+    "caro_net_set_kernel_form": (C.c_int, [_P, C.c_int]),
+    "caro_net_kernel_form": (C.c_int, [_P]),
+    "caro_net_last_launch_form": (C.c_int, [_P]),
     "caro_net_stream_evictions": (C.c_int64, [_P]),
     "caro_net_forward": (C.c_int, [_P, _P, _P, C.c_int, C.c_int64, _P, _P, _P]),
     "caro_stream_create_partition": (C.c_int, [C.c_int, C.c_int, C.c_int, _P]),
diff --git a/caro_ai_amd/csrc/caro_net.hip b/caro_ai_amd/csrc/caro_net.hip
--- a/caro_ai_amd/csrc/caro_net.hip
+++ b/caro_ai_amd/csrc/caro_net.hip
@@ -52,6 +52,17 @@
 }
 __device__ __forceinline__ float leaky(float x, float slope) { return x > 0.f ? x : x * slope; }
 
+struct ShapeAny {
+  static constexpr bool FIXED = false;
+  static __device__ __forceinline__ int H(int of_block) { return of_block; }
+  static __device__ __forceinline__ int W(int of_block) { return of_block; }
+  static __device__ __forceinline__ int HW(int of_block) { return of_block; }
+  static __device__ __forceinline__ int A(int of_block) { return of_block; }
+  static __device__ __forceinline__ int TB(int of_block) { return of_block; }
+  static __device__ __forceinline__ int TB2(int of_block) { return of_block; }
+  static __device__ __forceinline__ int TB4(int of_block) { return of_block; }
+};
+
 template <bool K2D>
 __device__ __forceinline__ int akey(int r, int W) {
   if constexpr (!K2D) return r & 15;
@@ -99,10 +110,10 @@
   }
 }
 
-template <bool K2D = false, int NTH = NT>
+template <class S, bool K2D = false, int NTH = NT>
 __device__ __forceinline__ void conv_in_mfma(const NetParams& p, const float* __restrict__ planes, const int* smap,
                                              float* act, const float* win, int R, int tid) {
-  const int HW = p.HW;
+  const int HW = S::HW(p.HW), H = S::H(p.H), W = S::W(p.W);
   const float slope = p.slope;
   const int wave = tid >> 6, lane = tid & 63;
   const int i = lane & 31, h = lane >> 5;
@@ -121,14 +132,14 @@
     const int r = rt * 32 + i;
     const bool rv = r < R;
     const int bi = rv ? r / HW : 0, cell = rv ? r - bi * HW : 0;
-    const int y = cell / p.W, x = cell - y * p.W;
+    const int y = cell / W, x = cell - y * W;
     const float* pl = planes + (size_t)smap[bi] * 2 * HW + h * HW;
     float in[9];
 #pragma unroll
     for (int t = 0; t < 9; ++t) {
       const int ny = y + t / 3 - 1, nx = x + t % 3 - 1;
-      const bool ok = rv && ny >= 0 && ny < p.H && nx >= 0 && nx < p.W;
-      in[t] = ok ? pl[ny * p.W + nx] : 0.f;
+      const bool ok = rv && ny >= 0 && ny < H && nx >= 0 && nx < W;
+      in[t] = ok ? pl[ny * W + nx] : 0.f;
     }
     f32x16 acc;
 #pragma unroll
@@ -143,7 +154,7 @@
         const int c4 = ct * 8 + 2 * q + h;
         const float4 out = make_float4(leaky(acc[4 * q], slope), leaky(acc[4 * q + 1], slope),
                                        leaky(acc[4 * q + 2], slope), leaky(acc[4 * q + 3], slope));
-        *reinterpret_cast<float4*>(act + r * NF + ((c4 ^ akey<K2D>(r, p.W)) << 2)) = out;
+        *reinterpret_cast<float4*>(act + r * NF + ((c4 ^ akey<K2D>(r, W)) << 2)) = out;
       }
     }
   }
@@ -151,15 +162,15 @@
 
 constexpr int HEAD_STAGE_AT = 4096;
 constexpr int HEAD_STAGE_MAX = 4096;
-__device__ __forceinline__ int head_span(int HW, int A) { return 3 * NF + 3 + 20 * HW + 20 + 20 + 1 + A * 2 * HW + A; }
-static inline int head_span_host(int HW, int A) { return 3 * NF + 3 + 20 * HW + 20 + 20 + 1 + A * 2 * HW + A; }
-
-template <bool STAGED, bool K2D = false, int NTH = NT>
+__device__ __forceinline__ constexpr int head_span(int HW, int A) { return 3 * NF + 3 + 20 * HW + 20 + 20 + 1 + A * 2 * HW + A; }
+static inline constexpr int head_span_host(int HW, int A) { return 3 * NF + 3 + 20 * HW + 20 + 20 + 1 + A * 2 * HW + A; }
+
+template <class S, bool STAGED, bool K2D = false, int NTH = NT>
 __device__ __forceinline__ void heads_f32(const NetParams& p, const float* act, float* scratch,
                                           float* __restrict__ probs, float* __restrict__ values, int slot_v, int nb,
                                           int R, int tid, float* __restrict__ featbuf = nullptr,
                                           int32_t* __restrict__ rowlist = nullptr, int dense0 = 0) {
-  const int HW = p.HW, A = p.A;
+  const int HW = S::HW(p.HW), A = S::A(p.A);
   const float slope = p.slope;
   constexpr int NSM = (3 * NF + 3 + 20 * 225 + 20 + 20 + 1 + NTH - 1) / NTH;
   const int nsmall = 3 * NF + 3 + 20 * HW + 20 + 20 + 1;
@@ -188,11 +199,13 @@
   int* omap = reinterpret_cast<int*>(stat + 64);
   float* ebuf = stat + 128;
   if (tid < nb) omap[tid] = slot_v;
-  for (int q = tid; q < 3 * R; q += NTH) {
-    const int o = q / R, r = q - o * R;
+  const int rsh = R > 128 ? 8 : R > 64 ? 7 : 6;
+  for (int q = tid; q < (3 << rsh); q += NTH) {
+    const int o = q >> rsh, r = q & ((1 << rsh) - 1);
+    if (r >= R) continue;
     const float* wo = w_head + o * NF;
     float s0 = b_head[o];
-    const int rkey = akey<K2D>(r, p.W);
+    const int rkey = akey<K2D>(r, S::W(p.W));
 #pragma unroll 8
     for (int g = 0; g < 16; ++g) {
       const float4 v = *reinterpret_cast<const float4*>(act + r * NF + ((g ^ rkey) << 2));
@@ -480,7 +493,7 @@
   for (int k = tid; k < 9 * 2 * NF; k += NT) wbuf[k] = p.w_in[k];
   int* smap = reinterpret_cast<int*>(wbuf + 1536);
   tile_rows(gpack, gG, gB, second ? 1 : 0, row0 + board0, board0, nb, smap + 64, smap, tid);
-  conv_in_mfma(p, planes, smap, act, wbuf, R, tid);
+  conv_in_mfma<ShapeAny>(p, planes, smap, act, wbuf, R, tid);
   const int slot_v0 = tid < nb ? smap[tid] : 0;
   __syncthreads();
 
@@ -703,7 +716,7 @@
   __syncthreads();
   unsigned long long t_trunk1 = 0;
   if (stamps) t_trunk1 = __builtin_amdgcn_s_memtime();
-  heads_f32<false>(p, act, wbuf, probs, values, slot_v, nb, R, tid, featbuf, rowlist, row0 + board0);
+  heads_f32<ShapeAny, false>(p, act, wbuf, probs, values, slot_v, nb, R, tid, featbuf, rowlist, row0 + board0);
   if (stamps && tid == 0) {
     stamps[4 * blockIdx.x] = __builtin_amdgcn_s_memtime() - t_c0;
     stamps[4 * blockIdx.x + 1] = ((__builtin_amdgcn_s_memrealtime() - t_r0) & 0xFFFFFull) | (t_epi << 20);
@@ -745,12 +758,12 @@
   if (hspan > NT * 4) dma_b128(src + NT, dst + NT * 16);
 }
 
-template <int KS, int NR>
+template <int KS, int NR, class S>
 __device__ __forceinline__ void trunk_w(const NetParams& p, float* act, float* wbuf, int nb, int tid, int hspan) {
   const int nres = NR ? NR : p.nres;
   const int wnchunk = nres * 6;
   const float slope = p.slope;
-  const int HW = p.HW;
+  const int HW = S::HW(p.HW), H = S::H(p.H), W = S::W(p.W);
   const int wave = tid >> 6, lane = tid & 63;
   const int i = lane & 31, h = lane >> 5;
   constexpr int NRT = 4 / KS;
@@ -764,26 +777,26 @@
     tbi = tent & 0xFF; tty = (tent >> 8) & 0xFF; tx = (tent >> 16) & 0xFF;
     tvalid = (tent >> 24) != 0 && tbi < nb;
   } else {
-    const int tpb = ((p.H + 1) >> 1) * p.W;
+    const int tpb = ((H + 1) >> 1) * W;
     const int mt = rt * 32 + i;
     tbi = mt / tpb;
     const int rem = mt - tbi * tpb;
-    tty = rem / p.W; tx = rem - tty * p.W;
+    tty = rem / W; tx = rem - tty * W;
     tvalid = mt < nb * tpb;
   }
-  const int orow0 = tbi * HW + 2 * tty * p.W + tx;
-  const bool ovalid0 = tvalid, ovalid1 = tvalid && 2 * tty + 1 < p.H;
+  const int orow0 = tbi * HW + 2 * tty * W + tx;
+  const bool ovalid0 = tvalid, ovalid1 = tvalid && 2 * tty + 1 < H;
   const unsigned abase = lds_addr(act);
   unsigned ra[4][3];
 #pragma unroll
   for (int r = 0; r < 4; ++r) {
     const int y = 2 * tty - 1 + r;
-    const bool oky = tvalid && y >= 0 && y < p.H;
+    const bool oky = tvalid && y >= 0 && y < H;
 #pragma unroll
     for (int d = 0; d < 3; ++d) {
       const int nx = tx + d - 1;
-      const int v = tbi * HW + y * p.W + nx;
-      const int row = oky && nx >= 0 && nx < p.W ? v : ZROW;
+      const int v = tbi * HW + y * W + nx;
+      const int row = oky && nx >= 0 && nx < W ? v : ZROW;
       ra[r][d] = abase + (unsigned)(row * NF + (((h * 8 + kq) ^ (v & 15)) << 2)) * 4u;
     }
   }
@@ -880,8 +893,8 @@
       const float s0 = up ? 1.f : 0.f, s2 = up ? 1.f : -1.f, s3 = up ? 0.f : -1.f;
       const float* bias = p.b_res + layer * NF + ct * 32 + 4 * h;
       const int g0 = ct * 8 + h;
-      float* rowp = act + (orow0 + (up ? p.W : 0)) * NF;
-      const int kk = (orow0 + (up ? p.W : 0)) & 15;
+      float* rowp = act + (orow0 + (up ? W : 0)) * NF;
+      const int kk = (orow0 + (up ? W : 0)) & 15;
       const bool ov = up ? ovalid1 : ovalid0;
       float4 bq[4], old[4];
 #pragma unroll
@@ -939,8 +952,8 @@
       const int myrow = kq >> 1, qb = (kq & 1) * 2;
       const float* bias = p.b_res + layer * NF + ct * 32 + 4 * h;
       const int g0 = ct * 8 + h;
-      float* rowp = act + (orow0 + (myrow ? p.W : 0)) * NF;
-      const int kk = (orow0 + (myrow ? p.W : 0)) & 15;
+      float* rowp = act + (orow0 + (myrow ? W : 0)) * NF;
+      const int kk = (orow0 + (myrow ? W : 0)) & 15;
       const bool ov = myrow ? ovalid1 : ovalid0;
       float4 bq[2], old[2];
 #pragma unroll
@@ -1017,8 +1030,8 @@
     const float* bias = p.b_res + layer * NF + ct * 32 + 4 * h;
     const int g0 = ct * 8 + h;
     float* row0p = act + orow0 * NF;
-    float* row1p = row0p + p.W * NF;
-    const int k0 = orow0 & 15, k1 = (orow0 + p.W) & 15;
+    float* row1p = row0p + W * NF;
+    const int k0 = orow0 & 15, k1 = (orow0 + W) & 15;
     float4 bq[4], old0[4], old1[4];
 #pragma unroll
     for (int q = 0; q < 4; ++q) bq[q] = *reinterpret_cast<const float4*>(bias + 8 * q);
@@ -1268,6 +1281,8 @@
 #undef W2_ALOAD
 }
 
+#define CARO_SHAPE ShapeAny
+#define CARO_ONE_NET 0
 #define CARO_NR NRES
 #define CARO_KN(name) name
 #include "caro_net_kernels.inc"
@@ -1278,6 +1293,41 @@
 #include "caro_net_kernels.inc"
 #undef CARO_NR
 #undef CARO_KN
+#undef CARO_SHAPE
+#undef CARO_ONE_NET
+
+template <int H_, int W_, int A_>
+struct ShapeFixed {
+  static constexpr bool FIXED = true;
+  static constexpr int cHW = H_ * W_, cTPB = ((H_ + 1) / 2) * W_;
+  static constexpr int cTB0 = 255 / cHW > 32 ? 32 : 255 / cHW;
+  static constexpr int cTB = 128 / cTPB < cTB0 ? 128 / cTPB : cTB0;
+  static constexpr int cTB2 = 64 / cTPB < cTB && 64 / cTPB * cHW <= XROW2 ? 64 / cTPB : 0;
+  static constexpr int cTB4 = 32 / cTPB < cTB && 32 / cTPB * cHW <= XROW4 ? 32 / cTPB : 0;
+  static_assert(cTPB <= 128 && cTB >= 1 && head_span_host(cHW, A_) <= HEAD_STAGE_MAX, "a board of the staged row-Winograd form");
+  static __device__ __forceinline__ constexpr int H(int) { return H_; }
+  static __device__ __forceinline__ constexpr int W(int) { return W_; }
+  static __device__ __forceinline__ constexpr int HW(int) { return cHW; }
+  static __device__ __forceinline__ constexpr int A(int) { return A_; }
+  static __device__ __forceinline__ constexpr int TB(int) { return cTB; }
+  static __device__ __forceinline__ constexpr int TB2(int) { return cTB2; }
+  static __device__ __forceinline__ constexpr int TB4(int) { return cTB4; }
+  static bool fits(const NetParams& p) {
+    return p.H == H_ && p.W == W_ && p.HW == cHW && p.A == A_ && p.TB == cTB && p.TB2 == cTB2 && p.TB4 == cTB4;
+  }
+};
+using ShapeC4 = ShapeFixed<6, 7, 7>;
+static_assert(ShapeC4::cTB == 6 && ShapeC4::cTB2 == 3 && ShapeC4::cTB4 == 1, "connect four: tiles of 6 / 3 / 1 boards");
+
+#define CARO_SHAPE ShapeC4
+#define CARO_ONE_NET 1
+#define CARO_NR NRES
+#define CARO_KN(name) name##_c4
+#include "caro_net_kernels.inc"
+#undef CARO_NR
+#undef CARO_KN
+#undef CARO_SHAPE
+#undef CARO_ONE_NET
 
 constexpr int HB = 32;
 constexpr int HEADS_MAX_CELLS = 225;
@@ -1500,7 +1550,20 @@
   int64_t hrows_evictions;
   int device;
   unsigned long long* dbg_stamps;
+  int force_generic;
+  int last_form;
 };
+
+static const int g_net_form_env = [] {
+  const char* e = getenv("CARO_NET_KERNEL_FORM");
+  return e && e[0] == '1' && !e[1] ? 1 : 0;
+}();
+
+static int net_form(const caro_net* n0, const caro_net* n1, int which) {
+  if (n0->kind != 0 || !n0->p.ww || n0->force_generic) return 1;
+  if (which >= 2 || n0->p.nres != cnet::NRES || n1->p.nres != cnet::NRES) return 1;
+  return cnet::ShapeC4::fits(n0->p) ? 0 : 1;
+}
 
 static int nfail(int code, const std::string& m) {
   caro__set_error(m.c_str());
@@ -1576,6 +1639,8 @@
   n->n_hrows = 0;
   n->hrows_clock = 0;
   n->hrows_evictions = 0;
+  n->force_generic = g_net_form_env;
+  n->last_form = -1;
   const size_t pad = (size_t)cnet::TPC * cnet::WCHUNK;
   if (hipMalloc((void**)&n->dev, (n_floats + pad) * sizeof(float)) != hipSuccess) {
     delete n;
@@ -1814,6 +1879,8 @@
   n->n_hrows = 0;
   n->hrows_clock = 0;
   n->hrows_evictions = 0;
+  n->force_generic = g_net_form_env;
+  n->last_form = -1;
   n->p.H = H; n->p.W = W; n->p.HW = H * W; n->p.A = A; n->p.TB = 4;
   *out = n;
   return 0;
@@ -1874,10 +1941,16 @@
       hipLaunchKernelGGL(cnet::k_net_heads, dim3(hgrid), dim3(cnet::NT), 0, st, n0->p, n1->p, counts_dev, which, row1,
                          hr->feat, hr->rowl, probs_dev, values_dev);
     }
-    else if (n0->p.ww)
-      hipLaunchKernelGGL(d5 ? cnet::k_net_forward_w : cnet::k_net_forward_w_any, dim3(grid), dim3(cnet::NT), 0, st,
-                         n0->p, n1->p, planes_dev, counts_dev, which, row1, probs_dev, values_dev,
-                         stamps ? stamps : n0->dbg_stamps, gpack, G, B);
+    else if (n0->p.ww) {
+      n0->last_form = net_form(n0, n1, which);
+      if (n0->last_form == 0)
+        hipLaunchKernelGGL(cnet::k_net_forward_w_c4, dim3(grid), dim3(cnet::NT), 0, st, n0->p, planes_dev, counts_dev,
+                           which, probs_dev, values_dev, stamps ? stamps : n0->dbg_stamps, gpack, G, B);
+      else
+        hipLaunchKernelGGL(d5 ? cnet::k_net_forward_w : cnet::k_net_forward_w_any, dim3(grid), dim3(cnet::NT), 0, st,
+                           n0->p, n1->p, planes_dev, counts_dev, which, row1, probs_dev, values_dev,
+                           stamps ? stamps : n0->dbg_stamps, gpack, G, B);
+    }
     else if (n0->p.wx3) {
       const bool batched = n0->p.TB == 1 && n0->p.w_pT && n0->p.HW <= cnet::HEADS_MAX_CELLS;
       caro_net::HeadRows* hr = nullptr;
@@ -1909,6 +1982,21 @@
   return 0;
 }
 
+int caro_net_set_kernel_form(caro_net* n, int form) {
+  if (!n) return nfail(CARO_E_INVAL, "null argument");
+  if (form != 0 && form != 1) return nfail(CARO_E_INVAL, "kernel form must be 0 (automatic) or 1 (always the general form)");
+  n->force_generic = form;
+  return 0;
+}
+int caro_net_kernel_form(const caro_net* n) {
+  if (!n) return nfail(CARO_E_INVAL, "null argument");
+  return net_form(n, n, 0);
+}
+int caro_net_last_launch_form(const caro_net* n) {
+  if (!n) return nfail(CARO_E_INVAL, "null argument");
+  return n->kind == 0 && n->p.ww ? n->last_form : 1;
+}
+
 int caro_net_boards_per_workgroup(const caro_net* n) { return n ? n->p.TB : 0; }
 int caro_net_uses_slot_list(const caro_net* n) { return n && n->p.ww2 ? 1 : 0; }
 
diff --git a/caro_ai_amd/csrc/caro_net_kernels.inc b/caro_ai_amd/csrc/caro_net_kernels.inc
--- a/caro_ai_amd/csrc/caro_net_kernels.inc
+++ b/caro_ai_amd/csrc/caro_net_kernels.inc
@@ -1,4 +1,5 @@
 
+#if !CARO_ONE_NET
 __global__ __launch_bounds__(NT, 2) void CARO_KN(k_net_forward)(NetParams p0, NetParams p1, const float* __restrict__ planes,
                                                          const int32_t* __restrict__ counts, int which, int row1,
                                                          float* __restrict__ probs, float* __restrict__ values,
@@ -160,7 +161,7 @@
   }
   unsigned long long t_trunk1 = 0;
   if (stamps) t_trunk1 = __builtin_amdgcn_s_memtime();
-  heads_f32<false>(p, act, wbuf, probs, values, slot_v, nb, R, tid);
+  heads_f32<ShapeAny, false>(p, act, wbuf, probs, values, slot_v, nb, R, tid);
   if (stamps && tid == 0) {
     stamps[4 * blockIdx.x] = __builtin_amdgcn_s_memtime() - t_c0;
     stamps[4 * blockIdx.x + 1] = __builtin_amdgcn_s_memrealtime() - t_r0;
@@ -168,13 +169,23 @@
     stamps[4 * blockIdx.x + 3] = t_trunk1 - t_c0;
   }
 }
-
+#endif
+
+#if CARO_ONE_NET
+__global__ __launch_bounds__(NT, 2) void CARO_KN(k_net_forward_w)(NetParams p0, const float* __restrict__ planes,
+                                                           const int32_t* __restrict__ counts, int which,
+                                                           float* __restrict__ probs, float* __restrict__ values,
+                                                           unsigned long long* __restrict__ stamps,
+                                                           const int32_t* __restrict__ gpack, int gG, int gB) {
+#else
 __global__ __launch_bounds__(NT, 2) void CARO_KN(k_net_forward_w)(NetParams p0, NetParams p1,
                                                            const float* __restrict__ planes,
                                                            const int32_t* __restrict__ counts, int which, int row1,
                                                            float* __restrict__ probs, float* __restrict__ values,
                                                            unsigned long long* __restrict__ stamps,
                                                            const int32_t* __restrict__ gpack, int gG, int gB) {
+#endif
+  using S = CARO_SHAPE;
   __shared__ __attribute__((aligned(256))) float lds[LDS_FLOATS];
   float* act = lds;
   float* wbuf = lds + ACT;
@@ -188,40 +199,48 @@
     const int g = (int)threadIdx.x * gcpt + u;
     gv[u] = gpre && u < gcpt && g < gG ? gpack[g] : 0;
   }
-  int L, row0, board0, nb, nb_cap = p0.TB;
+  const int TB = S::TB(p0.TB), TB2 = S::TB2(p0.TB2), TB4 = S::TB4(p0.TB4);
+  int L, row0, board0, nb, nb_cap = TB;
   int ks = 1;
+#if CARO_ONE_NET
+  constexpr bool second = false;
+  {
+#else
   bool second = false;
   if (which < 2) {
+#endif
     L = counts[which];
     row0 = which ? counts[0] : 0;
-    board0 = blockIdx.x * p0.TB;
-    const int full = p0.ncu * p0.TB;
+    board0 = blockIdx.x * TB;
+    const int full = p0.ncu * TB;
     if (p0.ncu > 0) {
-      if (p0.TB4 > 0 && L <= p0.ncu * p0.TB4) ks = 4;
-      else if (p0.TB2 > 0 && L <= p0.ncu * p0.TB2) ks = 2;
+      if (TB4 > 0 && L <= p0.ncu * TB4) ks = 4;
+      else if (TB2 > 0 && L <= p0.ncu * TB2) ks = 2;
       if (ks > 1) {
-        nb_cap = ks == 4 ? p0.TB4 : p0.TB2;
+        nb_cap = ks == 4 ? TB4 : TB2;
         board0 = (int)blockIdx.x * nb_cap;
       } else if (L > full) {
         const int over = L - full;
-        if (p0.TB4 > 0 && over <= p0.ncu * p0.TB4) ks = 4;
-        else if (p0.TB2 > 0 && over <= p0.ncu * p0.TB2) ks = 2;
+        if (TB4 > 0 && over <= p0.ncu * TB4) ks = 4;
+        else if (TB2 > 0 && over <= p0.ncu * TB2) ks = 2;
         if (ks > 1) {
           if ((int)blockIdx.x < p0.ncu) {
             ks = 1;
           } else {
-            nb_cap = ks == 4 ? p0.TB4 : p0.TB2;
+            nb_cap = ks == 4 ? TB4 : TB2;
             board0 = full + ((int)blockIdx.x - p0.ncu) * nb_cap;
           }
         }
       }
     }
-  } else {
+  }
+#if !CARO_ONE_NET
+  else {
     const int L0 = counts[0], L1 = counts[1];
     if (p0.ncu > 1) {
-      if (p0.TB4 > 0 && L0 + L1 <= (p0.ncu - 1) * p0.TB4) ks = 4;
-      else if (p0.TB2 > 0 && L0 + L1 <= (p0.ncu - 1) * p0.TB2) ks = 2;
-      if (ks > 1) nb_cap = ks == 4 ? p0.TB4 : p0.TB2;
+      if (TB4 > 0 && L0 + L1 <= (p0.ncu - 1) * TB4) ks = 4;
+      else if (TB2 > 0 && L0 + L1 <= (p0.ncu - 1) * TB2) ks = 2;
+      if (ks > 1) nb_cap = ks == 4 ? TB4 : TB2;
     }
     const int t0 = (L0 + nb_cap - 1) / nb_cap;
     second = (int)blockIdx.x >= t0;
@@ -229,15 +248,20 @@
     row0 = second ? (row1 >= 0 ? row1 : L0) : 0;
     board0 = (second ? (int)blockIdx.x - t0 : (int)blockIdx.x) * nb_cap;
   }
+#endif
   if (board0 >= L) return;
+#if CARO_ONE_NET
+  const NetParams& p = p0;
+#else
   const NetParams p = second ? p1 : p0;
+#endif
   unsigned long long t_c0 = 0, t_r0 = 0;
   if (stamps) {
     t_c0 = __builtin_amdgcn_s_memtime();
     t_r0 = __builtin_amdgcn_s_memrealtime();
   }
   nb = min(nb_cap, L - board0);
-  const int HW = p.HW;
+  const int HW = S::HW(p.HW);
   const int R = nb * HW;
   const int tid = threadIdx.x;
 
@@ -257,20 +281,25 @@
   int* smap = reinterpret_cast<int*>(win + 1536);
   if (gpre) tile_rows_pre(gv, gcpt, gmine, gB, second ? 1 : 0, board0, nb, smap + 64, smap, tid);
   else tile_rows(gpack, gG, gB, second ? 1 : 0, row0 + board0, board0, nb, smap + 64, smap, tid);
-  conv_in_mfma(p, planes, smap, act, win, R, tid);
+  conv_in_mfma<S>(p, planes, smap, act, win, R, tid);
   const int slot_v = tid < nb ? smap[tid] : 0;
   unsigned long long t_trunk0 = 0;
   if (stamps) t_trunk0 = __builtin_amdgcn_s_memtime();
   asm volatile("s_waitcnt vmcnt(0)" ::: "memory");
   __syncthreads();
-  const int hspan = head_span(HW, p.A) <= HEAD_STAGE_MAX ? head_span(HW, p.A) : 0;
-  if (ks == 1) trunk_w<1, CARO_NR>(p, act, wbuf, nb, tid, hspan);
-  else if (ks == 2) trunk_w<2, CARO_NR>(p, act, wbuf, nb, tid, hspan);
-  else trunk_w<4, CARO_NR>(p, act, wbuf, nb, tid, hspan);
+  const int hspan = head_span(HW, S::A(p.A)) <= HEAD_STAGE_MAX ? head_span(HW, S::A(p.A)) : 0;
+  if (ks == 1) trunk_w<1, CARO_NR, S>(p, act, wbuf, nb, tid, hspan);
+  else if (ks == 2) trunk_w<2, CARO_NR, S>(p, act, wbuf, nb, tid, hspan);
+  else trunk_w<4, CARO_NR, S>(p, act, wbuf, nb, tid, hspan);
   unsigned long long t_trunk1 = 0;
   if (stamps) t_trunk1 = __builtin_amdgcn_s_memtime();
-  if (hspan) heads_f32<true>(p, act, wbuf, probs, values, slot_v, nb, R, tid);
-  else heads_f32<false>(p, act, wbuf, probs, values, slot_v, nb, R, tid);
+#if CARO_ONE_NET
+  static_assert(S::FIXED, "the one-net form is built for a fixed shape, whose head block is always staged");
+  heads_f32<S, true>(p, act, wbuf, probs, values, slot_v, nb, R, tid);
+#else
+  if (hspan) heads_f32<S, true>(p, act, wbuf, probs, values, slot_v, nb, R, tid);
+  else heads_f32<S, false>(p, act, wbuf, probs, values, slot_v, nb, R, tid);
+#endif
   if (stamps && tid == 0) {
     stamps[4 * blockIdx.x] = __builtin_amdgcn_s_memtime() - t_c0;
     stamps[4 * blockIdx.x + 1] = gpack ? ((__builtin_amdgcn_s_memrealtime() - t_abs0) & 0xFFFFFull) | (t_abs0 << 20)
@@ -280,6 +309,7 @@
   }
 }
 
+#if !CARO_ONE_NET
 __global__ __launch_bounds__(NT, 2) void CARO_KN(k_net_forward_w2)(NetParams p0, NetParams p1,
                                                             const float* __restrict__ planes,
                                                             const int32_t* __restrict__ counts, int which, int row1,
@@ -342,7 +372,7 @@
     __syncthreads();
   } else if (gpre) tile_rows_pre(gv, gcpt, gmine, gB, second ? 1 : 0, board0, nb, smap + 64, smap, tid);
   else tile_rows(gpack, gG, gB, second ? 1 : 0, row0 + board0, board0, nb, smap + 64, smap, tid);
-  conv_in_mfma<true>(p, planes, smap, act, win, R, tid);
+  conv_in_mfma<ShapeAny, true>(p, planes, smap, act, win, R, tid);
   const int slot_v = tid < nb ? smap[tid] : 0;
   unsigned long long t_trunk0 = 0;
   if (stamps) t_trunk0 = __builtin_amdgcn_s_memtime();
@@ -351,7 +381,7 @@
   trunk_w2d<CARO_NR>(p, act, wbuf, tid);
   unsigned long long t_trunk1 = 0;
   if (stamps) t_trunk1 = __builtin_amdgcn_s_memtime();
-  heads_f32<false, true>(p, act, wbuf, probs, values, slot_v, nb, R, tid, featbuf, rowlist, row0 + board0);
+  heads_f32<ShapeAny, false, true>(p, act, wbuf, probs, values, slot_v, nb, R, tid, featbuf, rowlist, row0 + board0);
   if (stamps && tid == 0) {
     stamps[4 * blockIdx.x] = __builtin_amdgcn_s_memtime() - t_c0;
     stamps[4 * blockIdx.x + 1] = __builtin_amdgcn_s_memrealtime() - t_r0;
@@ -359,3 +389,4 @@
     stamps[4 * blockIdx.x + 3] = t_trunk1 - t_c0;
   }
 }
+#endif
diff --git a/caro_ai_amd/net_hip.py b/caro_ai_amd/net_hip.py
--- a/caro_ai_amd/net_hip.py
+++ b/caro_ai_amd/net_hip.py
@@ -146,7 +146,7 @@
 
     device_counts = True
 
-    def __init__(self, net: Net, device="cuda:0", negative_slope=0.01, mode="f32w", split_tiles=True):
+    def __init__(self, net: Net, device="cuda:0", negative_slope=0.01, mode="f32w", split_tiles=True, kernel_form=None):
         self.L = _lib.load()
         self.device = torch.device(device)
         self.H, self.W = net.input_shape[1], net.input_shape[2]
@@ -190,6 +190,17 @@
             _lib.check(self.L.caro_net_enable_split_bf16(self.h, wx.ctypes.data, wx.size))
         else:
             assert mode == "f32", mode
+        if kernel_form is not None:
+            self.set_kernel_form(kernel_form)
+
+    def set_kernel_form(self, form):
+        _lib.check(self.L.caro_net_set_kernel_form(self.h, int(form)))
+
+    def kernel_form(self):
+        form = self.L.caro_net_kernel_form(self.h)
+        if form < 0:
+            _lib.check(form)
+        return form
 
     def close(self):
         if getattr(self, "h", None):
diff --git a/include/caro_hip.h b/include/caro_hip.h
--- a/include/caro_hip.h
+++ b/include/caro_hip.h
@@ -220,6 +220,9 @@
 int64_t caro_net_stream_evictions(const caro_net* n);
 void caro_net_destroy(caro_net* n);
 int caro_net_boards_per_workgroup(const caro_net* n);
+int caro_net_set_kernel_form(caro_net* n, int form);
+int caro_net_kernel_form(const caro_net* n);
+int caro_net_last_launch_form(const caro_net* n);
 int caro_net_uses_slot_list(const caro_net* n);
 int caro_net_forward(caro_net* n, const float* planes_dev, const int32_t* counts_dev, int which, int64_t max_rows,
                      float* probs_dev, float* values_dev, void* stream);
```

New measurement: 8.586 million (median of 6 runs). 1.01x the previous value.
